# dylandreimerink/gobpfld

Measured on AMD Instinct MI355X. Metric: Mpkt/s device-resident XDP-emulator verdicts, 64B and 1500B batches, higher is better.
Workload: dtype int64

## Files before the change

### gobpfld_amd/_native.py

```python
from __future__ import annotations

import ctypes as C
from pathlib import Path

ROOT = Path(__file__).resolve().parent.parent
PRODUCT_LIB = ROOT / "gobpfld_amd" / "libxdpemu.so"
TUNING_LIB = ROOT / "gobpfld_amd" / "libxdpemu_tuning.so"


def product_path() -> Path:
    import os
    env = os.environ.get("XE_LIB")
    if not env:
        return PRODUCT_LIB
    p = Path(env).resolve()
    if p not in (PRODUCT_LIB.resolve(), TUNING_LIB.resolve()):
        raise RuntimeError(f"XE_LIB={env}: only {PRODUCT_LIB.name} or {TUNING_LIB.name} may serve as the product library")
    return p


class Desc(C.Structure):
    _fields_ = [("addr", C.c_uint64), ("len", C.c_uint32), ("options", C.c_uint32)]


# ... 45 lines not shown
class BatchStats(C.Structure):
    _fields_ = [("packets", C.c_uint64), ("steps", C.c_uint64), ("status_count", C.c_uint64 * 8),
                ("mode_used", C.c_uint32), ("conflict", C.c_uint32), ("kernel_ms", C.c_float),
                ("total_ms", C.c_float), ("engine_used", C.c_uint32), ("grid_blocks", C.c_uint32)]


def np_dtypes():
    import numpy as np
    desc = np.dtype([("addr", "<u8"), ("len", "<u4"), ("options", "<u4")])
    result = np.dtype([("status", "u1"), ("r0_kind", "u1"), ("code", "<u2"), ("pc", "<u4"), ("r0", "<i8")])
    regs = np.dtype([("val", "<i8", (10,)), ("kind", "u1", (10,)), ("region", "u1", (10,)),
                     ("map", "u1", (10,)), ("pad", "u1", (2,)), ("steps", "<u4")], align=True)
    assert desc.itemsize == 16 and result.itemsize == 16 and regs.itemsize == C.sizeof(Regs)
    return desc, result, regs


def np_trace_dtype():
    import numpy as np
    t = np.dtype([("packet", "<u4"), ("step", "<u4"), ("pc", "<i4"), ("pi", "<i4"), ("sf", "<u4"),
                  ("kind", "u1", (11,)), ("pad", "u1"), ("val", "<i8", (11,))], align=True)
    assert t.itemsize == C.sizeof(TraceRec) == 120
    return t


P = C.c_void_p
_SIGS = {
    "default_settings": (C.c_int, [P]),
    "create": (C.c_int, [P, C.POINTER(P)]),
    "destroy": (None, [P]),
    "last_error": (C.c_char_p, [P]),
    "add_raw_program": (C.c_int, [P, P, C.c_uint32, C.POINTER(C.c_int32)]),
    "set_entrypoint": (C.c_int, [P, C.c_int32]),
    "add_map": (C.c_int, [P, P, P, C.c_size_t, C.POINTER(C.c_int32)]),
    "map_lookup": (C.c_int, [P, C.c_int32, P, P]),
    "map_update": (C.c_int, [P, C.c_int32, P, P]),
    "map_delete": (C.c_int, [P, C.c_int32, P]),
    "map_update_batch": (C.c_int, [P, C.c_int32, P, P, C.c_uint64]),
    "map_count": (C.c_int, [P, C.c_int32, C.POINTER(C.c_uint64)]),
    "map_dump": (C.c_int, [P, C.c_int32, P, P, C.c_uint64, C.POINTER(C.c_uint64)]),
    "map_dump_list": (C.c_int, [P, C.c_int32, P, C.c_uint64, P, C.c_uint64, C.POINTER(C.c_uint64), C.POINTER(C.c_uint64)]),
    "map_lru_order": (C.c_int, [P, C.c_int32, P, C.c_uint64, C.POINTER(C.c_uint64)]),
    "map_push": (C.c_int, [P, C.c_int32, P]),
    "run_batch": (C.c_int, [P, P, C.c_uint64, P, C.c_uint32, P, P, P, P]),
    "run_batch_host": (C.c_int, [P, P, C.c_uint64, P, C.c_uint32, P, P, P, P]),
    "run_batch_device": (C.c_int, [P, P, C.c_uint64, P, C.c_uint32, P, P, P, P, P]),
    "run_batch_device_async": (C.c_int, [P, P, C.c_uint64, P, C.c_uint32, P, P, P, P, P]),
    "sync": (C.c_int, [P]),
    "cancel": (C.c_int, [P, C.POINTER(C.c_uint32)]),
    "trace_config": (C.c_int, [P, P, C.c_uint32, C.c_uint32]),
    "trace_read": (C.c_int, [P, C.c_uint32, P, C.c_uint32, C.POINTER(C.c_uint32)]),
    "set_helper": (C.c_int, [P, C.c_uint32, HELPER_FN, P]),
    "reset_helper": (C.c_int, [P, C.c_uint32]),
    "prepare": (C.c_int, [P]),
    "debug_set_schedule": (C.c_int, [P, C.c_uint32]),
    "debug_set_lru_epoch": (C.c_int, [P, C.c_uint64]),
    "debug_map_pool": (C.c_int, [P, C.c_int32, C.POINTER(C.c_uint64), C.POINTER(C.c_uint64)]),
    "set_kernel_cache": (C.c_int, [C.c_char_p]),
    "kernel_source": (C.c_int, [P, C.c_int, C.c_char_p, C.c_size_t, C.POINTER(C.c_size_t)]),
    "compile_kernel_source": (C.c_int, [C.c_char_p, C.c_char_p, C.c_char_p, C.c_char_p, C.c_size_t]),
    "kernel_object_name": (C.c_int, [C.c_char_p, C.c_char_p, C.c_char_p, C.c_size_t]),
    "kernel_cache_stats": (C.c_int, [C.POINTER(C.c_uint64), C.POINTER(C.c_uint64), C.POINTER(C.c_double)]),
    "map_values_bytes": (C.c_int, [P, C.c_int32, C.POINTER(C.c_uint64)]),
    "map_delta": (C.c_int, [P, C.c_int32, C.c_uint32, P, P]),
    "map_apply_delta": (C.c_int, [P, C.c_int32, C.c_uint32, P, P]),
    "map_delta_lane": (C.c_int, [P, C.c_int32, C.POINTER(C.c_uint32)]),
    "footprint": (C.c_int, [P, C.POINTER(C.c_uint64), C.c_uint32, C.POINTER(C.c_uint32)]),
    "shard_check": (C.c_int, [P, C.c_uint32, C.c_uint32, P]),
    "epoch_begin": (C.c_int, [P, P]),
    "epoch_end": (C.c_int, [P]),
    "map_state_bytes": (C.c_int, [P, C.c_int32, C.POINTER(C.c_uint64)]),
    "map_state_export": (C.c_int, [P, C.c_int32, P, P]),
    "map_state_import": (C.c_int, [P, C.c_int32, P, P]),
    "map_lookup_batch_device": (C.c_int, [P, C.c_int32, P, C.c_uint64, P, P, P]),
    "map_update_batch_device": (C.c_int, [P, C.c_int32, P, P, C.c_uint64, P]),
    "map_delete_batch_device": (C.c_int, [P, C.c_int32, P, C.c_uint64, P, P]),
    "map_lookup_batch": (C.c_int, [P, C.c_int32, P, C.c_uint64, P, P]),
    "map_update_batch_staged": (C.c_int, [P, C.c_int32, P, P, C.c_uint64]),
    "map_delete_batch": (C.c_int, [P, C.c_int32, P, C.c_uint64, P]),
    "map_scan_device": (C.c_int, [P, C.c_int32, P, P, P, C.c_uint64, C.POINTER(C.c_uint64), P]),
    "map_expire_device": (C.c_int, [P, C.c_int32, P, P, P, C.c_uint64, C.POINTER(C.c_uint64), P]),
    "map_scan": (C.c_int, [P, C.c_int32, P, P, P, C.c_uint64, C.POINTER(C.c_uint64)]),
    "map_expire": (C.c_int, [P, C.c_int32, P, P, P, C.c_uint64, C.POINTER(C.c_uint64)]),
    "debug_map_traffic": (C.c_int, [P, C.c_int32, C.POINTER(C.c_uint64), C.POINTER(C.c_uint64)]),
    "multi_create": (C.c_int, [P, C.c_uint32, C.POINTER(P)]),
    "multi_destroy": (None, [P]),
    "multi_last_error": (C.c_char_p, [P]),
    "run_batch_multi": (C.c_int, [P, P, P, P, P, P, P, P, P]),
    "version": (C.c_char_p, []),
    "device_count": (C.c_int, [C.POINTER(C.c_int)]),
    "decode_names": (C.c_int, [P, C.c_uint32, C.c_char_p, C.c_size_t]),
    "pcap_header": (C.c_int, [P, C.c_uint64, P]),
    "pcap_count": (C.c_int, [P, C.c_uint64, P, C.c_uint64, C.POINTER(C.c_uint64), C.POINTER(C.c_uint64)]),
    "pcap_fill": (C.c_int, [P, C.c_uint64, P, C.POINTER(C.c_uint64), P, C.c_uint64, C.c_uint32, C.c_uint32, P,
                            C.c_uint64, C.c_uint32, P, P, P, C.POINTER(C.c_uint32)]),
    "pcap_pack": (C.c_int, [P, C.c_uint64, P, C.POINTER(C.c_uint64), P, C.c_uint64, C.c_uint32, C.c_uint32,
                            C.c_uint32, P, P, P, C.POINTER(C.c_uint32), C.POINTER(C.c_uint64)]),
    "dispatch_scratch_bytes": (C.c_int, [C.c_uint32, C.POINTER(C.c_uint64)]),
    "dispatch_device": (C.c_int, [P, P, P, C.c_uint32, P, P, P, P, C.c_uint64, P]),
    "gather_device": (C.c_int, [P, C.c_uint64, P, P, C.c_uint32, C.c_uint32, P, C.c_uint32, P, C.c_uint64, P, P, P]),
}

HEADER_SYMBOLS = [
    "xe_default_settings", "xe_create", "xe_destroy", "xe_last_error", "xe_add_raw_program",
    "xe_set_entrypoint", "xe_add_map", "xe_map_lookup", "xe_map_update", "xe_map_delete",
    "xe_map_count", "xe_map_dump", "xe_map_dump_list", "xe_map_lru_order", "xe_map_push", "xe_map_update_batch", "xe_run_batch_device", "xe_run_batch_host",
    "xe_run_batch_device_async", "xe_sync", "xe_prepare", "xe_map_values_bytes", "xe_map_delta", "xe_map_apply_delta", "xe_map_delta_lane", "xe_footprint", "xe_version",
    "xe_device_count", "xe_shard_check", "xe_epoch_begin", "xe_epoch_end", "xe_map_state_bytes", "xe_map_state_export",
    "xe_map_state_import",
    "xe_multi_create", "xe_multi_destroy", "xe_run_batch_multi", "xe_multi_last_error", "xe_debug_set_schedule",
    "xe_debug_set_lru_epoch", "xe_debug_map_pool",
    "xe_map_lookup_batch_device", "xe_map_update_batch_device", "xe_map_delete_batch_device",
    "xe_map_lookup_batch", "xe_map_update_batch_staged", "xe_map_delete_batch", "xe_debug_map_traffic",
    "xe_map_scan_device", "xe_map_expire_device", "xe_map_scan", "xe_map_expire",
    "xe_set_kernel_cache", "xe_kernel_source", "xe_compile_kernel_source", "xe_kernel_object_name",
    "xe_kernel_cache_stats",
    "xe_cancel", "xe_trace_config", "xe_trace_read", "xe_set_helper", "xe_reset_helper",
]
IO_HEADER_SYMBOLS = ["xe_pcap_header", "xe_pcap_count", "xe_pcap_fill", "xe_pcap_pack",
                     "xe_dispatch_scratch_bytes", "xe_dispatch_device", "xe_gather_device"]
ACT_ABORTED, ACT_DROP, ACT_PASS, ACT_TX, ACT_REDIRECT, ACT_COUNT = 0, 1, 2, 3, 4, 5
XE_DISPATCH_TILE = 2048


class Lib:

    def __init__(self, path: Path | str, prefix: str = "xe_"):
        self.path = Path(path)
        if not self.path.exists():
            raise FileNotFoundError(
                f"{self.path} is missing: build it with `python -c 'import __graft_entry__ as g; g.build()'`")
        self.dll = C.CDLL(str(self.path))
        self.prefix = prefix
        for name, (res, args) in _SIGS.items():
            fn = getattr(self.dll, prefix + name, None)
            if fn is None:
                continue
            fn.restype = res
            fn.argtypes = args
            setattr(self, name, fn)

    def has(self, name: str) -> bool:
        return hasattr(self, name)


_product: Lib | None = None


def product() -> Lib:
    global _product
    if _product is None:
        try:
            import torch
        except ImportError:
            pass
        _product = Lib(product_path(), "xe_")
        kdir = ROOT / "gobpfld_amd" / "kernels"
        if kdir.is_dir() and _product.has("set_kernel_cache"):
            _product.set_kernel_cache(str(kdir).encode())
    return _product
```

### gobpfld_amd/csrc/xe_internal.h

```cpp
#pragma once
#if !defined(__HIPCC_RTC__)
#include <stdint.h>
#endif
#include "../../include/xdpemu.h"

#if defined(__HIPCC_RTC__)
#define XE_HD __host__ __device__ __forceinline__
#elif defined(__HIPCC__)
#include <hip/hip_runtime.h>
#define XE_HD __host__ __device__ __forceinline__
#else
#define XE_HD static inline
#endif

#if !defined(__HIPCC_RTC__)
#if defined(XE_TUNING)
#include <stdlib.h>
static inline const char* xe_tuning_env(const char* name) { return getenv(name); }
#else
static inline const char* xe_tuning_env(const char*) { return nullptr; }
#endif
#endif

enum XeUopClass : uint8_t {
// ... 151 lines not shown
  x ^= x >> 33;
  x *= 0xff51afd7ed558ccdull;
  x ^= x >> 33;
  x *= 0xc4ceb9fe1a85ec53ull;
  x ^= x >> 33;
  return x;
}
XE_HD uint64_t xe_kid(uint32_t m, uint64_t h) {
  return (uint64_t(m & 63u) << 58) | (xe_kid_mix(h) & ((1ull << 58) - 16ull)) | 2ull;
}
#define XE_KLOG_W 1ull
#define XE_KLOG_INS 4ull
#define XE_KLOG_FLAGS 0xDull
#define XE_KINS 2u
enum : uint32_t { XE_KS_DSET = 0, XE_KS_UNION, XE_KS_COMPRESS, XE_KS_ASSIGN, XE_KS_IOTA, XE_KS_NCHAIN, XE_KS_RESERVE,
                  XE_KS_COUNT, XE_KS_CSTART, XE_KS_CLONG, XE_KS_UNNEW, XE_KS_CFLAG, XE_KS_CLIST,
                  XE_KS_LRUID, XE_KS_FIRST, XE_KS_EKEY, XE_KS_EVICT, XE_KS_EMARK };
#define XE_KSTRIPES 32
#define XE_KS_DCOUNT 0
#define XE_KS_ERR 64
#define XE_KS_CHANGED 65
#define XE_KS_NO 66
#define XE_KS_LONG 67
#define XE_KS_NCH 68
#define XE_KS_CNEXT 69
#define XE_KS_DINS 128
#define XE_KS_CINS 192
#define XE_KS_WORDS (192 + 64 * XE_KSTRIPES)
#define XE_KEY_VALID 0x200ull
#define XE_KID_ARRAY_TAG 0xA7A7A7A700000000ull
#define XE_KID_NIL_KEY 0x6e696c6b65790001ull

struct XeKeyed {
  uint64_t* klog;
  uint32_t* kcnt;
  uint32_t dcap;
  uint32_t kw;
  uint64_t* dkid;
  uint32_t* dcomp;
  uint32_t* cstart;
  uint64_t* dkey;
  uint64_t* ikey;
  uint32_t* dcount;
  uint32_t* dins;
  uint32_t* cins;
  uint32_t* err;
  uint32_t* changed;
  uint32_t* ckey;
  uint32_t* okey;
  uint32_t* order;
  uint32_t* iota;
  uint32_t* counts;
  const uint8_t* skip;
  uint32_t n;
  uint32_t nO;
  uint32_t* dfirst;
  uint32_t* dvict;
  uint64_t* ekey;
  uint64_t* ekey2;
  uint32_t* eval;
  uint32_t* eval2;
  const uint64_t* etsnap;
  const uint32_t* vorder;
  uint32_t em, eoff, efree, ecnt0;
};

struct XeGen {
  uint8_t* base;
  uint32_t nl;
  uint32_t nobj;
  uint32_t nframes;
  uint32_t nvc;
  uint32_t nbm;
  uint32_t nkey;
  uint64_t nbytes;
  uint64_t o_ov, o_oh, o_ot, o_ofree, o_mark, o_frm, o_ctx, o_vc, o_vcinfo, o_vfree, o_bm, o_bfree, o_pres, o_key;
  uint64_t o_bytes;
  uint32_t mark_words;
  uint32_t pad;
};

#define XE_TAIL_MAPS 4
#define XE_TAIL_MAP_WORDS 2048
struct XeTailMap {
  unsigned long long* vals;
  unsigned long long* rep;
  unsigned long long* snap;
  uint64_t words;
  uint64_t stride_words;
  uint32_t nrep;
  uint32_t pad;
};
struct XeTailArgs {
  unsigned long long* aux;
  unsigned long long* host_aux;
  uint32_t* poison;
  uint32_t aux_words, nrep, rep_words, nmaps, mode, ntail;
  XeTailMap tail[XE_TAIL_MAPS];
};

struct XeListRun {
  uint32_t cnt0[64];
  uint32_t sens[64];
  uint32_t push[64];
  uint32_t senslo[64];
  unsigned long long popmask;
  unsigned long long newlist;
};
#define XE_POP_SLOTS 4u
struct XePopSlots {
  uint8_t slot[64];
};

struct XeParams {
  const XeUop* prog;
  int32_t prog_len;
  uint32_t mode;
  uint8_t* umem;
  uint64_t umem_len;
  const xe_desc* desc;
  uint32_t n;
  uint32_t nmaps;
  uint8_t bigmap[XE_H_BIG_FIELDS];
  uint8_t bigoff[XE_H_BIG_FIELDS];
  xe_result* results;
  uint32_t* verdicts;
  xe_regs* regs;
  const XeDevMap* maps;
  uint64_t max_steps;
  uint32_t ingress;
  uint32_t rxq;
  uint32_t* flags;
  unsigned long long* rep;
  uint32_t nrep;
  uint32_t rep_words;
  const XeUop* progs;
  const int32_t* prog_off;
  const int32_t* prog_lens;
  uint32_t nprogs;
  int32_t entry;
  XeGen gen;
  const uint32_t* poison;
  uint32_t seq_prefetch;
  XeKeyed K;
  uint32_t sched;
  const uint32_t* trace_pk;
  xe_trace_rec* trace;
  uint32_t* trace_cnt;
  uint32_t trace_npk, trace_max;
  XeListRun* list;
  uint32_t pop_mode;
  uint32_t pop_stride;
  uint8_t pop_slot[64];
  uint32_t* popflag;
  const uint32_t* popbase;
  uint64_t host_helpers[3];
  uint64_t nil_helpers[3];
  struct XeHostCall* hostcall;
};

#define XE_HOSTCALL_TIMEOUT_TICKS (100ull * 1000 * 1000 * 30)
struct XeHostCall {
  uint32_t req;
  uint32_t ack;
  uint32_t id;
  uint32_t packet;
  int64_t args[5];
  uint8_t kinds[5];
  uint8_t pad[3];
  int32_t err;
  int64_t r0;
  xe_helper_fn fn[192];
  void* user[192];
};

#define XE_AUX_DECISION 1

template <class Words>
XE_HD bool xe_replay_decision(uint32_t flags, Words orw, uint32_t rep_words, uint32_t nmaps, uint32_t mode) {
  bool conflict = (flags & (XE_FLAG_ORDERED | XE_FLAG_CAPACITY)) != 0;
  for (uint32_t m = 1; m <= nmaps && m < 64 && 17 + 2 * m < rep_words; m++) {
    if (orw[16 + 2 * m] & orw[16 + 2 * m + 1]) conflict = true;
    const unsigned wc = unsigned(orw[XE_REC_WIDTH0 + m / 16] >> (4 * (m % 16))) & 15u;
    if (wc & (wc - 1)) conflict = true;
  }
  return conflict && (mode == XE_MODE_AUTO || (flags & XE_FLAG_CAPACITY));
}
```

### gobpfld_amd/csrc/xe_interp.h

```cpp
#pragma once
#include "xe_internal.h"

#ifndef XE_UNIFORM
#define XE_UNIFORM 0
#endif

#if defined(__HIPCC__)
#define XE_DEV __device__ __forceinline__
#define XE_WAVE 64
typedef unsigned int xe_u4 __attribute__((ext_vector_type(4)));
XE_DEV unsigned long long xe_ballot(bool p) { return __ballot(p); }
XE_DEV int xe_readfirst(int v) { return __builtin_amdgcn_readfirstlane(v); }
XE_DEV int xe_readlane(int v, int l) { return __builtin_amdgcn_readlane(v, l); }
XE_DEV uint64_t xe_readlane64(uint64_t v, int l) {
  return uint64_t(uint32_t(__builtin_amdgcn_readlane(int(uint32_t(v)), l))) |
         (uint64_t(uint32_t(__builtin_amdgcn_readlane(int(uint32_t(v >> 32)), l))) << 32);
}
XE_DEV int xe_lane() { return __lane_id(); }
XE_DEV void xe_pin(uint64_t& x) { asm volatile("" : "+v"(x)); }
#define XE_GP(T) __attribute__((address_space(1))) T*
#define XE_LP(T) __attribute__((address_space(3))) T*
XE_DEV uint32_t xe_uni32(uint32_t v) { return XE_UNIFORM ? uint32_t(__builtin_amdgcn_readfirstlane(int(v))) : v; }
XE_DEV uint64_t xe_uni64(uint64_t v) {
  if (!XE_UNIFORM) return v;
// ... 3490 lines not shown

  for (;;) {
    int key = 0x7fffffff;
    if (status == -1) {
      if (steps >= P.max_steps) {
        status = XE_ST_BUDGET; res_pc = pc;
      } else if (XE_LANE_PI(L) < 1 || XE_LANE_PI(L) > int32_t(P.nprogs)) {
        status = XE_ST_VMERR; code = XE_E_NO_PROGRAM; res_pc = pc;
      } else if (pc < 0 || pc >= P.prog_lens[XE_LANE_PI(L)]) {
        status = XE_ST_PANIC; code = XE_P_INDEX; res_pc = pc;
      } else {
        key = P.prog_off[XE_LANE_PI(L)] + pc;
      }
    }
    const int sel = wave_min(key);
    if (sel == 0x7fffffff) break;
    if (key == sel) {
      const XeUop u = P.progs[sel];
      const int32_t plen = P.prog_lens[XE_LANE_PI(L)];
      steps++;
      int32_t tgt;
      int e = exec_uop(L, P, u, pc, tgt);
      res_pc = pc;
#if XE_TRACE
      if (tslot >= 0 && (e == 0 || e == XE_EV_EXIT)) {
        if (tdone < P.trace_max) trace_put(L, P, tslot, i, tdone, pc);
        tdone++;
      }
#endif
      if (e == 0) {
        if (int64_t(plen) <= int64_t(tgt) + 1) {
          status = XE_ST_VMERR; code = XE_E_BAD_PC;
        } else {
          pc = tgt + 1;
        }
      } else {
        status_from_error(e, status, code);
      }
    }
  }
#if XE_TRACE
  if (tslot >= 0) P.trace_cnt[tslot] = uint32_t(tdone < P.trace_max ? tdone : P.trace_max);
#endif
  if (finish) lane_finish(L, P, i, valid, status, code, res_pc, steps);
}

XE_DEV void run_packet(XeLane& L, const XeParams& P, uint32_t i, bool valid) {
  lane_reset(L, P, i, valid);
  run_staged(L, P, i, valid);
}

XE_DEV void flush_wave_state(XeLane& L, const XeParams& P) {
  acc_flush(L);
  unsigned long long steps = L.acc_steps;
  unsigned int aw = L.awidth;
#if defined(__HIPCC__)
  for (int o = 32; o > 0; o >>= 1) aw |= __shfl_xor(aw, o);
#endif
  if (xe_lane() == 0 && aw) xe_atomic_or64(&L.rep[XE_REC_WIDTH0], aw);
#if XE_KEYED
  if (xe_lane() == 0 && L.kany) xe_atomic_or32(P.flags, XE_FLAG_KEYED);
#endif
#if defined(__HIPCC__)
  for (int o = 32; o > 0; o >>= 1) steps += __shfl_xor(steps, o);
#endif
  if (xe_lane() == 0) {
    if (steps) xe_atomic_add64(&L.rep[0], steps);
#pragma unroll
    for (int st = 0; st < 8; st++)
      if (L.acc_status[st]) xe_atomic_add64(&L.rep[1 + st], L.acc_status[st]);
  }
#pragma unroll
  for (int k = 0; k < XE_FP_MAPS; k++) {
    unsigned long long r = L.fpr[k], a = L.fpa[k];
#if defined(__HIPCC__)
    for (int o = 32; o > 0; o >>= 1) { r |= __shfl_xor(r, o); a |= __shfl_xor(a, o); }
#endif
    if (xe_lane() == 0) {
      if (r) xe_atomic_or64(&L.rep[16 + (k + 1) * 2], r);
      if (a) xe_atomic_or64(&L.rep[16 + (k + 1) * 2 + 1], a);
    }
  }
}
```

### gobpfld_amd/csrc/xe_jit.cpp

```cpp
#ifndef XE_HOSTSIM
#include <hip/hip_runtime_api.h>
#include <hip/hiprtc.h>
#endif

#include <algorithm>
#include <array>
#include <atomic>
#include <chrono>
#include <climits>
#include <cstdint>
#include <cstdio>
#include <cstdlib>
#include <cstring>
#include <fstream>
#include <future>
#include <map>
#include <memory>
#include <set>
#include <mutex>
#include <sstream>
#include <string>
#include <vector>

#include <unistd.h>
// ... 880 lines not shown
          o << "    if (uop_jmp(L, " << U << ")) ";
          emit_goto_bb(o, size_t(k), u.tgt, n, cyclic ? "steps" : "(steps + st)");
          o << "\n";
          break;
        case U_MOVI: case U_MOVR:
          o << "    " << handler_call(u, cms[size_t(k)]) << "\n";
          break;
        case U_ALU: case U_NEG: case U_END: case U_LDIMM64: case U_LDX: case U_ST: case U_STX: case U_ATOMIC:
        case U_HELPER: case U_CALLX: {
          auto ks = kshadow.find(k);
          if (!dead.count(k))
            o << "    " << (ks != kshadow.end() ? key_call(p, u, cms[size_t(k)], ks->second, captured) : handler_call(u, cms[size_t(k)]))
              << "\n" << on_err;
          const std::string cap = key_capture(u, k, captured, alias_caps);
          if (!cap.empty()) o << "    " << cap << "\n";
          break;
        }
        default: o << "    e = exec_uop(L, P, " << U << ", " << k << ", tgt);\n" << on_err; break;
      }
    }
    if (!terminated) {
      if (e + 1 >= n) o << "    status = XE_ST_VMERR; code = XE_E_BAD_PC; res_pc = " << e << "; bb = XE_BB_DONE;\n";
      else o << "    bb = " << e + 1 << ";\n";
    }
    o << "  } while (0);\n";
    if (ifconv) o << "#endif\n";
    b = rules ? rci->second.end : (chain.empty() ? e : chain.back()) + 1;
  }
  if (cyclic) o << "  }\n";
  else o << "  steps += st;\n";
}

bool fields_model(const std::vector<XeUop>& p, bool cyclic) { return !cyclic && 7 + max_stores_on_path(p) <= 64; }

void emit_kernel(std::ostringstream& o) {
  o << R"(#ifndef XE_MIN_WAVES_PER_EU
#define XE_MIN_WAVES_PER_EU 4  // 4 waves per SIMD: VGPRs <= 128 (16 waves per CU)
#endif
extern "C" __global__ void __launch_bounds__(256, XE_MIN_WAVES_PER_EU) xe_jit_kernel(XeParams P) {
  __shared__ __attribute__((aligned(16))) uint8_t hdr_lds[XE_HDR_LDS_BYTES];
  __shared__ XePend pend_lds[4];
  extern __shared__ __attribute__((aligned(16))) uint8_t xe_dyn_lds[];  // (nmaps + 1) map descriptors
  XeLane L;
#if !XE_GEN
  XeMem M;
  L.mem = &M;
#endif
  L.hdrbuf = (XE_LP(uint8_t))(hdr_lds + (threadIdx.x >> 6) * XE_HDR_WAVE_BYTES);
  const int lane = xe_lane();
#if XE_COMMITTER
  __shared__ XeRing xe_rings[3];  // waves 0..2 -> the committer (wave 3), parallel mode
  if (threadIdx.x < 3) { xe_rings[threadIdx.x].head = 0; xe_rings[threadIdx.x].tail = 0; xe_rings[threadIdx.x].done = 0; }
#endif
  stage_maps(L, P, (XE_LP(XeDevMap))xe_dyn_lds);
  wave_state_init(L, P, (blockIdx.x * blockDim.x + threadIdx.x) >> 6, &pend_lds[threadIdx.x >> 6]);
#if XE_UNIFORM
  {  // the scalar replay: the sequential driver alone
#else
  if (P.mode == XE_MODE_SEQUENTIAL) {
#endif
    if (blockIdx.x != 0 || threadIdx.x >= 64) return;
    seq_packets(L, P, [&](uint32_t i, bool valid) __attribute__((always_inline)) {
      int status = XE_ST_OK, code = 0; int32_t res_pc = 0; uint64_t steps = 0;
      if (valid) xe_jit_body(L, P, status, code, res_pc, steps);
      lane_finish(L, P, i, valid, status, code, res_pc, steps);
    }, [&](bool valid) __attribute__((always_inline)) {  // the runahead: results dropped
      int status = XE_ST_OK, code = 0; int32_t res_pc = 0; uint64_t steps = 0;
      if (valid) xe_jit_body(L, P, status, code, res_pc, steps);
    });
#if XE_UNIFORM
  }
#else
#if XE_KEYED
  } else if (P.mode == XE_MODE_CHAIN) {
    chain_packets(L, P, blockIdx.x * blockDim.x + threadIdx.x, gridDim.x * blockDim.x, [&](uint32_t i, bool valid) __attribute__((always_inline)) {
      int status = XE_ST_OK, code = 0; int32_t res_pc = 0; uint64_t steps = 0;
      if (valid) xe_jit_body(L, P, status, code, res_pc, steps);
      lane_finish(L, P, i, valid, status, code, res_pc, steps);
    });
#endif
  } else {
    uint32_t wave = (blockIdx.x * blockDim.x + threadIdx.x) >> 6;
    uint32_t nwaves = (gridDim.x * blockDim.x) >> 6;
#if XE_COMMITTER
    if (P.mode == XE_MODE_PARALLEL && blockDim.x == 256) {
      const uint32_t wib = threadIdx.x >> 6;
      if (wib == 3) { committer_loop(L, P, (XE_LP(XeRing))xe_rings, 3); return; }
      L.ring = (XE_LP(XeRing))&xe_rings[wib];
      wave = blockIdx.x * 3 + wib;
      nwaves = gridDim.x * 3;
    }
#endif
    parallel_packets(L, P, wave, nwaves, [&](uint32_t i, bool valid) __attribute__((always_inline)) {
      int status = XE_ST_OK, code = 0; int32_t res_pc = 0; uint64_t steps = 0;
      if (valid) xe_jit_body(L, P, status, code, res_pc, steps);
      lane_finish(L, P, i, valid, status, code, res_pc, steps);
    });
#if XE_COMMITTER
    if (L.ring) ring_done(L.ring);
#endif
  }
#endif  // !XE_UNIFORM
  flush_wave_state(L, P);
}
)";
}

enum { XE_JV_PLAIN = 0, XE_JV_KEYED = 1, XE_JV_LEAN = 2, XE_JV_SEQ = 3 };
void emit_variant(std::ostringstream& o, int variant) {
  o << "#define XE_KEYED " << (variant == XE_JV_KEYED ? 1 : 0) << "\n";
  if (variant == XE_JV_LEAN) o << "#define XE_RECORDS 0\n";
  if (variant == XE_JV_SEQ) o << "#define XE_UNIFORM 1\n#define XE_MIN_WAVES_PER_EU 1\n#define xe_jit_kernel xe_jit_seq_kernel\n";
}

bool has_lru(const std::vector<XeDevMap>& geom);

std::string generate(const std::vector<XeUop>& p, bool cyclic, const std::vector<XeDevMap>& geom, int variant = XE_JV_PLAIN) {
  std::ostringstream o;
  const int64_t n = int64_t(p.size());
  unsigned mapkinds = 0;
  for (size_t i = 1; i < geom.size(); i++)
    mapkinds |= geom[i].kind == XE_DM_ARRAY ? 1u : (geom[i].kind == XE_DM_HASH || geom[i].kind == XE_DM_LRU) ? 2u : 0u;
  const bool lru = has_lru(geom);
  o << "#define XE_REGS_FIELDS 1\n";
  o << "#define XE_HAS_ARRAY " << ((mapkinds & 1u) ? 1 : 0) << "\n";
  o << "#define XE_HAS_HASH " << ((mapkinds & 2u) ? 1 : 0) << "\n";
  o << "#define XE_FP_MAPS " << std::max<size_t>(1, std::min<size_t>(4, geom.size() - 1)) << "\n";
  o << "#define XE_HAS_ORDERED " << (lru ? 1 : 0) << "\n";
  if (lru) o << "#define XE_FIELDS_LRU 1\n";
  if (lru && variant == XE_JV_KEYED) o << "#define XE_MIN_WAVES_PER_EU 2\n";
  emit_variant(o, variant);
  if (variant != XE_JV_KEYED && fields_model(p, cyclic)) o << "#ifndef XE_SEQ_PEEK\n#define XE_SEQ_PEEK 1\n#endif\n";
  o << "#ifndef XE_IFCONV\n#define XE_IFCONV 1  // if-converted jump blocks (emit_body_blocks; -D overrides: A/B)\n#endif\n";
  int add_sites = 0;
  for (const XeUop& u : p)
    add_sites += (u.cls == U_ATOMIC || (u.cls == U_STX && (u.fl & UF_LIFT))) && uop_size(u) == 8 ? 1 : 0;
  o << "#define XE_PAIR_ADDS " << (add_sites >= 2 ? 1 : 0) << "\n";
  if (fields_model(p, cyclic)) emit_mem_fields(o, 7 + max_stores_on_path(p));
  emit_geom(o, geom);
  std::vector<RegMasks> cms = class_masks(p);
  emit_window(o, p, cyclic, cms, geom);
  o << "#include \"xe_interp.h\"\n";
  o << "__device__ __forceinline__ void xe_jit_geom(unsigned m, XeDevMap& M) { XE_JIT_GEOM_BODY }\n\n";
  int cond = 0;
  for (const XeUop& u : p) cond += u.cls == U_JMP;
  const bool blocks = n > 0 && cond > 32;
  const std::map<int64_t, RuleChain> rchains = blocks ? rule_chains(p, cyclic) : std::map<int64_t, RuleChain>{};
  {
    int id = 0;
    for (const auto& rc : rchains) emit_rule_tables(o, rc.second, id++);
  }
  o << "XE_DEV void xe_jit_body(XeLane& L, const XeParams& P, int& status, int& code, int32_t& res_pc, uint64_t& steps) {\n";
  o << "  int e = 0; int32_t tgt = 0; (void)e; (void)tgt;\n";
  std::map<int64_t, int64_t> store_off;
  AliasCaps alias_caps;
  const KeyShadows kshadow = key_shadows(p, cms, geom, &store_off, &alias_caps);
  const std::set<int64_t> dead = fields_model(p, cyclic) ? dead_frame_stores(p, cms, kshadow, store_off) : std::set<int64_t>{};
  std::set<int64_t> modified;
  for (const auto& a : alias_caps)
    for (const auto& sr : a.second) modified.insert(sr.first);
  std::set<int64_t> captured;
  for (const auto& site : kshadow)
    for (const KeyPart& q : site.second)
      if (p[size_t(q.store)].cls == U_STX || modified.count(q.store)) captured.insert(q.store);
  for (int64_t s : captured) o << "  int64_t ksv" << s << " = 0;\n";
  if (n == 0) o << "  status = XE_ST_PANIC; code = XE_P_INDEX; res_pc = 0; return;\n";
  if (blocks) {
    o << "#define XE_BB_DONE 0x7fffffff\n";
    emit_body_blocks(o, p, cyclic, cms, kshadow, captured, dead, alias_caps, rchains);
  } else {
  for (int64_t k = 0; k < n; k++) {
    const XeUop& u = p[k];
    o << "L" << k << ":\n";
    if (cyclic) o << "  if (steps >= P.max_steps) { status = XE_ST_BUDGET; res_pc = " << k << "; return; }\n";
    o << "  steps++;\n";
    const std::string U = uop_literal(u);
    const std::string on_err = "  if (e) { res_pc = " + std::to_string(k) + "; status_from_error(e, status, code); return; }\n";
    switch (u.cls) {
      case U_EXIT:
        o << "  status = XE_ST_OK; res_pc = " << k << "; return;\n";
        continue;
      case U_NOP:
        break;
// ... 799 lines not shown
```

### gobpfld_amd/csrc/xe_kernel.hip

```cpp
#include "xe_interp.h"
#include "xe_kernels.h"

#include <hipcub/device/device_radix_sort.hpp>
#include <hipcub/device/device_scan.hpp>

extern "C" __global__ void __launch_bounds__(256) xe_interp_kernel(XeParams P) {
  __shared__ __attribute__((aligned(16))) uint8_t hdr_lds[XE_HDR_LDS_BYTES];
  __shared__ XePend pend_lds[4];
  extern __shared__ __attribute__((aligned(16))) uint8_t xe_dyn_lds[];
  XeLane L;
  L.hdrbuf = (XE_LP(uint8_t))(hdr_lds + (threadIdx.x >> 6) * XE_HDR_WAVE_BYTES);
  const int lane = xe_lane();
  stage_maps(L, P, (XE_LP(XeDevMap))xe_dyn_lds);
  wave_state_init(L, P, (blockIdx.x * blockDim.x + threadIdx.x) >> 6, &pend_lds[threadIdx.x >> 6]);
  if (P.mode == XE_MODE_SEQUENTIAL) {
    if (blockIdx.x != 0 || threadIdx.x >= 64) return;
    seq_packets(L, P, [&](uint32_t i, bool valid) { run_staged(L, P, i, valid); }, [](bool) {});
  } else if (P.mode == XE_MODE_CHAIN) {
    chain_packets(L, P, blockIdx.x * blockDim.x + threadIdx.x, gridDim.x * blockDim.x,
                  [&](uint32_t i, bool valid) { run_staged(L, P, i, valid); });
  } else {
    const uint32_t wave = (blockIdx.x * blockDim.x + threadIdx.x) >> 6;
    const uint32_t nwaves = (gridDim.x * blockDim.x) >> 6;
    parallel_packets(L, P, wave, nwaves, [&](uint32_t i, bool valid) { run_staged(L, P, i, valid); });
  }
  flush_wave_state(L, P);
}

template <class T, class C>
__global__ void xe_delta_kernel(const T* cur, const T* snap, C* out, uint64_t n) {
  for (uint64_t i = blockIdx.x * uint64_t(blockDim.x) + threadIdx.x; i < n; i += uint64_t(gridDim.x) * blockDim.x)
    out[i] = C(T(cur[i] - snap[i]));
}
template <class T, class C>
__global__ void xe_apply_delta_kernel(T* cur, const T* snap, const C* delta, uint64_t n) {
  for (uint64_t i = blockIdx.x * uint64_t(blockDim.x) + threadIdx.x; i < n; i += uint64_t(gridDim.x) * blockDim.x)
    cur[i] = T(snap[i] + T(delta[i]));
}
template <class C>
__global__ void xe_sum_kernel(C* acc, const C* in, uint64_t n) {
  for (uint64_t i = blockIdx.x * uint64_t(blockDim.x) + threadIdx.x; i < n; i += uint64_t(gridDim.x) * blockDim.x)
    acc[i] = C(acc[i] + in[i]);
}

extern "C" __global__ void xe_rep_fold_kernel(unsigned long long* __restrict__ vals, unsigned long long* __restrict__ rep,
                                              uint64_t stride_words, uint32_t nrep, uint64_t nwords,
                                              const unsigned long long* __restrict__ recs, uint32_t rwords, uint32_t vsize,
                                              uint32_t cap, const unsigned long long* __restrict__ lim) {
  if (lim) nwords = nwords < (lim[3] * vsize + 7) / 8 ? nwords : (lim[3] * vsize + 7) / 8;
  for (uint64_t i = blockIdx.x * uint64_t(blockDim.x) + threadIdx.x; i < nwords; i += uint64_t(gridDim.x) * blockDim.x) {
    if (recs) {
      const uint64_t s0 = 8 * i / vsize, s1 = (8 * i + 7) / vsize;
      const bool live = (s0 <= cap && recs[s0 * rwords] != 0) || (s1 != s0 && s1 <= cap && recs[s1 * rwords] != 0);
      if (!live) continue;
    }
    unsigned long long v[16];
#pragma unroll
    for (uint32_t k = 0; k < 16; k++) v[k] = k < nrep ? rep[k * stride_words + i] : 0ull;
    unsigned long long s = 0;
#pragma unroll
    for (uint32_t k = 0; k < 16; k++) {
      s += v[k];
      if (v[k]) rep[k * stride_words + i] = 0;
    }
    if (s) vals[i] += s;
  }
}

#define XE_PRO_SEGS 8
struct XeProlog {
  const unsigned long long* src[XE_PRO_SEGS];
  unsigned long long* dst[XE_PRO_SEGS];
  uint64_t words[XE_PRO_SEGS];
  uint32_t nseg;
  unsigned long long* zero;
  uint64_t zero_words;
};
extern "C" __global__ void xe_prologue_kernel(XeProlog A) {
  const uint64_t tid = blockIdx.x * uint64_t(blockDim.x) + threadIdx.x, nth = uint64_t(gridDim.x) * blockDim.x;
  for (uint64_t i = tid; i < A.zero_words; i += nth) A.zero[i] = 0;
  for (uint32_t g = 0; g < A.nseg; g++)
    for (uint64_t i = tid; i < A.words[g]; i += nth) A.dst[g][i] = A.src[g][i];
}

extern "C" __global__ void __launch_bounds__(1024) xe_tail_kernel(XeTailArgs A) {
  __shared__ unsigned long long orw[257];
  const uint32_t t = threadIdx.x, nt = blockDim.x;
  for (uint32_t w = t; w <= 256; w += nt) orw[w] = 0;
  const bool poisoned = *(volatile uint32_t*)A.poison != 0;
  __syncthreads();
  for (uint32_t i = t; i < A.aux_words; i += nt) {
    const unsigned long long v = A.aux[i];
    if (v) A.aux[i] = 0;
    A.host_aux[i] = v;
    if (i == 0) orw[256] = v;
    else if (i >= 16 && v) atomicOr(&orw[(i - 16) % A.rep_words], v);
  }
  __syncthreads();
  if (t == 0) {
    const bool replay = !poisoned && xe_replay_decision(uint32_t(orw[256]), orw, A.rep_words, A.nmaps, A.mode);
    A.host_aux[XE_AUX_DECISION] = replay ? 1ull : 0ull;
    if (replay) *A.poison = 1u;
  }
  if (poisoned) return;
  for (uint32_t f = 0; f < A.ntail; f++) {
    const XeTailMap& T = A.tail[f];
    for (uint64_t i = t; i < T.words; i += nt) {
      unsigned long long r[16];
#pragma unroll
      for (uint32_t k = 0; k < 16; k++) r[k] = k < T.nrep ? T.rep[k * T.stride_words + i] : 0ull;
      unsigned long long s = 0;
#pragma unroll
      for (uint32_t k = 0; k < 16; k++) {
        s += r[k];
        if (r[k]) T.rep[k * T.stride_words + i] = 0;
      }
      const unsigned long long v = T.vals[i] + s;
      if (s) T.vals[i] = v;
      T.snap[i] = v;
    }
  }
}
extern "C" int xe_launch_tail(const XeTailArgs* A, hipStream_t s) {
  if (A->rep_words > 256) return -1;
  hipLaunchKernelGGL(xe_tail_kernel, dim3(1), dim3(1024), 0, s, *A);
  return hipGetLastError() == hipSuccess ? 0 : -1;
}

__global__ void xe_desc_split_kernel(const xe_desc* d, uint32_t n, uint64_t umem_len, unsigned long long* key,
                                     uint32_t* len) {
  for (uint64_t i = blockIdx.x * uint64_t(blockDim.x) + threadIdx.x; i < n; i += uint64_t(gridDim.x) * blockDim.x) {
    const uint64_t a = d[i].addr;
    uint32_t l = d[i].len;
    if (a > umem_len || uint64_t(l) > umem_len - a) l = 0;
    key[i] = l ? a : ~0ull;
    len[i] = l;
  }
}
__global__ void xe_desc_overlap_kernel(const unsigned long long* key, const uint32_t* len, uint32_t n, uint32_t* flag) {
  for (uint64_t i = blockIdx.x * uint64_t(blockDim.x) + threadIdx.x; i + 1 < n; i += uint64_t(gridDim.x) * blockDim.x)
    if (len[i] && len[i + 1] && key[i] + len[i] > key[i + 1]) *flag = 1u;
}
extern "C" int xe_launch_desc_overlap(const void* desc, uint32_t n, uint64_t umem_len, void* scratch, size_t* scratch_bytes,
                                      uint32_t* flag, hipStream_t s) {
  const size_t arr = ((size_t(n) * 8 + 255) & ~size_t(255)) * 2 + ((size_t(n) * 4 + 255) & ~size_t(255)) * 2;
  size_t tmp = 0;
  if (hipcub::DeviceRadixSort::SortPairs(nullptr, tmp, (unsigned long long*)nullptr, (unsigned long long*)nullptr,
                                         (uint32_t*)nullptr, (uint32_t*)nullptr, int(n), 0, 64, s) != hipSuccess)
    return -1;
  if (!scratch) {
    *scratch_bytes = arr + tmp;
    return 0;
  }
  if (*scratch_bytes < arr + tmp) return -1;
  uint8_t* p = (uint8_t*)scratch;
  auto take = [&](size_t bytes) { uint8_t* q = p; p += (bytes + 255) & ~size_t(255); return q; };
  unsigned long long* k0 = (unsigned long long*)take(size_t(n) * 8);
  unsigned long long* k1 = (unsigned long long*)take(size_t(n) * 8);
  uint32_t* l0 = (uint32_t*)take(size_t(n) * 4);
  uint32_t* l1 = (uint32_t*)take(size_t(n) * 4);
  const uint32_t blocks = n / 256 + 1 < 4096 ? n / 256 + 1 : 4096;
  if (hipMemsetAsync(flag, 0, 4, s) != hipSuccess) return -1;
  hipLaunchKernelGGL(xe_desc_split_kernel, dim3(blocks), dim3(256), 0, s, (const xe_desc*)desc, n, umem_len, k0, l0);
  if (hipcub::DeviceRadixSort::SortPairs(p, tmp, k0, k1, l0, l1, int(n), 0, 64, s) != hipSuccess) return -1;
  hipLaunchKernelGGL(xe_desc_overlap_kernel, dim3(blocks), dim3(256), 0, s, k1, l1, n, flag);
  return hipGetLastError() == hipSuccess ? 0 : -1;
}

extern "C" __global__ void xe_keyed_kernel(XeKeyed K, const XeDevMap* maps, uint8_t* skip, uint32_t step, uint32_t items) {
  for (uint64_t i = blockIdx.x * uint64_t(blockDim.x) + threadIdx.x; i < items; i += uint64_t(gridDim.x) * blockDim.x)
    keyed_step(K, maps, skip, step, uint32_t(i));
}
extern "C" __global__ void xe_keyed_count_kernel(XeKeyed K) {
  __shared__ unsigned int hist[64], ins[64];
  if (threadIdx.x < 64) hist[threadIdx.x] = ins[threadIdx.x] = 0;
  __syncthreads();
  for (uint64_t x = blockIdx.x * uint64_t(blockDim.x) + threadIdx.x; x < K.dcap; x += uint64_t(gridDim.x) * blockDim.x) {
    const uint64_t kid = K.dkid[x];
    if (kid) {
      atomicAdd(&hist[kid >> 58], 1u);
      if (K.dkey[x * K.kw] & XE_KEY_VALID) atomicAdd(&ins[kid >> 58], 1u);
    }
  }
  __syncthreads();
  if (threadIdx.x < 64 && hist[threadIdx.x]) atomicAdd(K.dcount + threadIdx.x, hist[threadIdx.x]);
  if (threadIdx.x < 64 && ins[threadIdx.x]) atomicAdd(K.dins + threadIdx.x, ins[threadIdx.x]);
}
extern "C" int xe_launch_keyed(const XeKeyed* K, const XeDevMap* maps, uint8_t* skip, uint32_t step, uint32_t items,
                               hipStream_t s) {
  if (!items) return 0;
  if (step == XE_KS_COUNT) {
    hipLaunchKernelGGL(xe_keyed_count_kernel, dim3(1024), dim3(256), 0, s, *K);
    return hipGetLastError() == hipSuccess ? 0 : -1;
  }
  const uint32_t blocks = items / 256 + 1 < 8192 ? items / 256 + 1 : 8192;
  hipLaunchKernelGGL(xe_keyed_kernel, dim3(blocks), dim3(256), 0, s, *K, maps, skip, step, items);
  return hipGetLastError() == hipSuccess ? 0 : -1;
}
extern "C" int xe_launch_keyed_sort(const XeKeyed* K, uint32_t n, uint32_t end_bit, void* scratch, size_t* bytes, hipStream_t s) {
  size_t tmp = 0;
  if (hipcub::DeviceRadixSort::SortPairs(nullptr, tmp, (const uint32_t*)nullptr, (uint32_t*)nullptr, (const uint32_t*)nullptr,
                                         (uint32_t*)nullptr, int(n), 0, int(end_bit), s) != hipSuccess)
    return -1;
  if (!scratch) {
    *bytes = tmp;
    return 0;
  }
  if (*bytes < tmp) return -1;
  return hipcub::DeviceRadixSort::SortPairs(scratch, tmp, K->ckey, K->okey, K->iota, K->order, int(n), 0, int(end_bit), s) ==
                 hipSuccess
             ? 0
// ... 263 lines not shown
```

### gobpfld_amd/csrc/xe_kernels.h

```cpp
#ifndef XE_KERNELS_H_
#define XE_KERNELS_H_

#include "xe_internal.h"

#ifndef XE_HOSTSIM
#include <hip/hip_runtime_api.h>
#endif

extern "C" {

int xe_jit_may_write_entries(const XeUop* prog, size_t n);
size_t xe_jit_source_for(const XeUop* const* progs, const uint32_t* lens, uint32_t nprogs, int32_t entry,
                         const XeDevMap* maps, uint32_t nmaps, int variant, char* buf, size_t buflen);

#ifndef XE_HOSTSIM
void* xe_jit_get(const XeUop* const* progs, const uint32_t* lens, uint32_t nprogs, int32_t entry, int device,
                 const XeDevMap* maps, uint32_t nmaps, bool* cyclic, bool* general, const char** err, int variant,
                 uint64_t* maxpath);
int xe_jit_launch(void* fn, const XeParams* P, uint32_t blocks, uint32_t threads, hipStream_t s);
int xe_jit_occupancy(void* fn, uint32_t nmaps);

int xe_launch_interp(const XeParams* P, uint32_t blocks, uint32_t threads, hipStream_t s);
int xe_interp_occupancy(uint32_t nmaps);
int xe_launch_delta(const void* cur, const void* snap, void* out, uint64_t bytes, uint32_t lane, hipStream_t s);
int xe_launch_apply_delta(void* cur, const void* snap, const void* delta, uint64_t bytes, uint32_t lane, hipStream_t s);
int xe_launch_delta_sum(void* acc, const void* in, uint64_t bytes, uint32_t lane, hipStream_t s);
int xe_launch_rep_fold(void* vals, void* rep, uint64_t stride_words, uint32_t nrep, uint64_t nwords, const void* recs,
                       uint32_t rwords, uint32_t vsize, uint32_t cap, const void* lim, hipStream_t s);
int xe_launch_prologue(const void* const* src, void* const* dst, const uint64_t* words, uint32_t nseg, void* zero,
                       uint64_t zero_words, hipStream_t s);
int xe_launch_tail(const XeTailArgs* A, hipStream_t s);
int xe_launch_desc_overlap(const void* desc, uint32_t n, uint64_t umem_len, void* scratch, size_t* scratch_bytes,
                           uint32_t* flag, hipStream_t s);
int xe_launch_keyed(const XeKeyed* K, const XeDevMap* maps, uint8_t* skip, uint32_t step, uint32_t items, hipStream_t s);
int xe_launch_keyed_sort(const XeKeyed* K, uint32_t n, uint32_t end_bit, void* scratch, size_t* bytes, hipStream_t s);
int xe_launch_keyed_esort(const XeKeyed* K, void* scratch, size_t* bytes, hipStream_t s);
int xe_launch_keyed_scan(const XeKeyed* K, uint32_t n, void* scratch, size_t* bytes, hipStream_t s);
int xe_launch_append(const XeAppendArgs* A, uint32_t end_bit, void* scratch, size_t* bytes, hipStream_t s);
int xe_launch_pop(const uint32_t* src, uint32_t* dst, uint32_t n, uint32_t mode, uint32_t arg, XePopSlots sl, uint32_t* flag,
                  hipStream_t s);
int xe_launch_lru_relink(uint64_t* tag, uint32_t pool, uint32_t cnt, uint32_t* link, uint64_t* hdr, void* scratch,
                         size_t* bytes, int renumber, hipStream_t s);
int xe_launch_lru_tag_fold(uint64_t* tag, uint64_t* rep, uint32_t pool, uint32_t r, const uint64_t* hdr, hipStream_t s);
int xe_launch_lru_log(const uint64_t* tag, uint32_t pool, const uint32_t* order, const uint64_t* hdr, uint64_t* log,
                      hipStream_t s);
#endif

int xe_internal_vm_device(const xe_vm* vm);
void* xe_internal_vm_stream(xe_vm* vm);
int xe_internal_nmaps(const xe_vm* vm);
int xe_internal_may_write_packet(const xe_vm* vm);
int xe_internal_delta_sum(xe_vm* vm, void* acc, const void* in, uint64_t bytes, uint32_t lane);
int xe_internal_alloc(xe_vm* vm, void** p, uint64_t bytes);
void xe_internal_free(xe_vm* vm, void* p);
int xe_internal_copy(xe_vm* vm, void* dst, const void* src, uint64_t bytes);

}

#endif
```

### gobpfld_amd/csrc/xe_runtime.cpp

```cpp
#include "xe_internal.h"
#include "xe_mapops.h"

#include <algorithm>
#include <map>
#include <chrono>
#include <cstdio>
#include <cstdlib>
#include <cstring>
#include <string>
#include <array>
#include <thread>
#include <vector>

#ifdef XE_HOSTSIM
#define XE_SEQ_PEEK 1
#include "xe_interp.h"
typedef void* xe_stream_t;
#else
#include <hip/hip_runtime_api.h>
typedef hipStream_t xe_stream_t;
#endif
#include "xe_kernels.h"

#define XE_FRAME_SIZE 256

namespace {

#ifdef XE_HOSTSIM
#ifdef XE_HOSTSIM_POISON
int dev_alloc(void** p, size_t n) {
  n = n ? n : 8;
  *p = malloc(n);
  if (*p) memset(*p, 0xA5, n);
  return *p ? 0 : -1;
}
#else
int dev_alloc(void** p, size_t n) { *p = calloc(n ? n : 8, 1); return *p ? 0 : -1; }
#endif
void dev_free(void* p) { free(p); }
int h2d(void* d, const void* h, size_t n, xe_stream_t) { memcpy(d, h, n); return 0; }
int d2h(void* h, const void* d, size_t n, xe_stream_t) { memcpy(h, d, n); return 0; }
int d2d(void* d, const void* s, size_t n, xe_stream_t) { memmove(d, s, n); return 0; }
int dmemset(void* d, int v, size_t n, xe_stream_t) { memset(d, v, n); return 0; }
int dsync(xe_stream_t) { return 0; }
int launch_interp(const XeParams* P, uint32_t, uint32_t, xe_stream_t) {
  XeLane L;
#ifdef XE_HOSTSIM_POISON
  memset(static_cast<void*>(&L), 0, sizeof L);
#endif
  static thread_local uint8_t hdrbuf[XE_HDR_WAVE_BYTES + 16];
  L.hdrbuf = hdrbuf;
  XePend pend;
  stage_maps(L, *P, nullptr);
  wave_state_init(L, *P, 0, &pend);
  if (P->mode == XE_MODE_PARALLEL || P->mode == XE_MODE_SPEC) {
    parallel_packets(L, *P, 0, 1, [&](uint32_t i, bool valid) { run_staged(L, *P, i, valid); });
  } else if (P->mode == XE_MODE_CHAIN) {
    chain_packets(L, *P, 0, 1, [&](uint32_t i, bool valid) { run_staged(L, *P, i, valid); });
  } else {
    seq_packets(L, *P, [&](uint32_t i, bool valid) { run_staged(L, *P, i, valid); },
                [&](bool valid) { run_staged(L, *P, 0, valid, false); });
  }
  flush_wave_state(L, *P);
  return 0;
}
int launch_jit(void*, const XeParams* P, uint32_t b, uint32_t t, xe_stream_t s) { return launch_interp(P, b, t, s); }
template <class T, class C = T>
void lanes_sub(const void* a, const void* b, void* o, uint64_t n) {
  for (uint64_t i = 0; i < n; i++) ((C*)o)[i] = C(T(((const T*)a)[i] - ((const T*)b)[i]));
}
template <class T, class C = T>
void lanes_add(const void* snap, const void* d, void* o, uint64_t n) {
  for (uint64_t i = 0; i < n; i++) ((T*)o)[i] = T(((const T*)snap)[i] + T(((const C*)d)[i]));
}
template <class C>
void lanes_acc(void* acc, const void* in, uint64_t n) {
  for (uint64_t i = 0; i < n; i++) ((C*)acc)[i] = C(((C*)acc)[i] + ((const C*)in)[i]);
}
int launch_delta(const void* cur, const void* snap, void* out, uint64_t bytes, uint32_t lane, xe_stream_t) {
  switch (lane) {
    case 1: lanes_sub<uint8_t>(cur, snap, out, bytes); break;
    case 2: lanes_sub<uint16_t, uint32_t>(cur, snap, out, bytes / 2); break;
    case 4: lanes_sub<uint32_t>(cur, snap, out, bytes / 4); break;
    default: lanes_sub<uint64_t>(cur, snap, out, bytes / 8); break;
  }
  return 0;
}
int launch_apply_delta(void* cur, const void* snap, const void* delta, uint64_t bytes, uint32_t lane, xe_stream_t) {
  switch (lane) {
    case 1: lanes_add<uint8_t>(snap, delta, cur, bytes); break;
    case 2: lanes_add<uint16_t, uint32_t>(snap, delta, cur, bytes / 2); break;
    case 4: lanes_add<uint32_t>(snap, delta, cur, bytes / 4); break;
    default: lanes_add<uint64_t>(snap, delta, cur, bytes / 8); break;
  }
  return 0;
}
int launch_delta_sum(void* acc, const void* in, uint64_t bytes, uint32_t lane, xe_stream_t) {
  switch (lane) {
    case 1: lanes_acc<uint8_t>(acc, in, bytes); break;
    case 2: case 4: lanes_acc<uint32_t>(acc, in, bytes / lane); break;
    default: lanes_acc<uint64_t>(acc, in, bytes / 8); break;
  }
  return 0;
}
int launch_prologue(const void* const* src, void* const* dst, const uint64_t* words, uint32_t nseg, void* zero, uint64_t zw,
                    xe_stream_t) {
  if (zw) memset(zero, 0, zw * 8);
  for (uint32_t g = 0; g < nseg; g++) memcpy(dst[g], src[g], words[g] * 8);
  return 0;
}
int launch_rep_fold(void* vals, void* rep, uint64_t sw, uint32_t nrep, uint64_t nw, const void* recs, uint32_t rwords,
                    uint32_t vsize, uint32_t cap, const void* lim, xe_stream_t) {
  uint64_t* v = (uint64_t*)vals;
  uint64_t* r = (uint64_t*)rep;
  const uint64_t* rc = (const uint64_t*)recs;
  if (lim) nw = std::min<uint64_t>(nw, (((const uint64_t*)lim)[3] * vsize + 7) / 8);
  for (uint64_t i = 0; i < nw; i++) {
    if (rc) {
      const uint64_t s0 = 8 * i / vsize, s1 = (8 * i + 7) / vsize;
      if (!((s0 <= cap && rc[s0 * rwords]) || (s1 != s0 && s1 <= cap && rc[s1 * rwords]))) continue;
    }
    for (uint32_t k = 0; k < nrep; k++) { v[i] += r[k * sw + i]; r[k * sw + i] = 0; }
  }
  return 0;
}
int launch_tail(const XeTailArgs* A, xe_stream_t) {
  unsigned long long orw[257] = {};
  const bool poisoned = *A->poison != 0;
  for (uint32_t i = 0; i < A->aux_words; i++) {
    const unsigned long long v = A->aux[i];
    A->aux[i] = 0;
    A->host_aux[i] = v;
    if (i == 0) orw[256] = v;
    else if (i >= 16) orw[(i - 16) % A->rep_words] |= v;
  }
  const bool replay = !poisoned && xe_replay_decision(uint32_t(orw[256]), orw, A->rep_words, A->nmaps, A->mode);
  A->host_aux[XE_AUX_DECISION] = replay ? 1ull : 0ull;
  if (replay) *A->poison = 1u;
  if (poisoned) return 0;
  for (uint32_t f = 0; f < A->ntail; f++) {
    const XeTailMap& T = A->tail[f];
    for (uint64_t i = 0; i < T.words; i++) {
      unsigned long long s = 0;
      for (uint32_t k = 0; k < T.nrep; k++) { s += T.rep[k * T.stride_words + i]; T.rep[k * T.stride_words + i] = 0; }
      T.vals[i] += s;
      T.snap[i] = T.vals[i];
    }
  }
  return 0;
}
int host_alloc(void** p, size_t n) { *p = calloc(n ? n : 8, 1); return *p ? 0 : -1; }
void host_free(void* p) { free(p); }
int host_device_ptr(void** d, void* h) { *d = h; return 0; }
int host_alloc_coherent(void** p, size_t n) { return host_alloc(p, n); }
int serve_hostcalls(XeHostCall*, xe_stream_t) { return 0; }
int poison_async(uint32_t* d, xe_stream_t*) { *d = 2; return 0; }
void stream_destroy(xe_stream_t) {}
int launch_desc_overlap(const void* desc, uint32_t n, uint64_t umem_len, void* scratch, size_t* bytes, uint32_t* flag,
                        xe_stream_t) {
  if (!scratch) { *bytes = 8; return 0; }
  std::vector<std::pair<uint64_t, uint32_t>> r;
  const xe_desc* d = (const xe_desc*)desc;
  for (uint32_t i = 0; i < n; i++) {
    uint32_t l = d[i].len;
    if (d[i].addr > umem_len || uint64_t(l) > umem_len - d[i].addr) l = 0;
    if (l) r.emplace_back(d[i].addr, l);
  }
  std::sort(r.begin(), r.end());
  *flag = 0;
  for (size_t i = 0; i + 1 < r.size(); i++)
    if (r[i].first + r[i].second > r[i + 1].first) *flag = 1;
  return 0;
}
int launch_keyed(const XeKeyed* K, const XeDevMap* maps, uint8_t* skip, uint32_t step, uint32_t items, xe_stream_t) {
  if (step == XE_KS_COUNT) {
    for (uint32_t x = 0; x < K->dcap; x++)
      if (K->dkid[x]) {
        K->dcount[K->dkid[x] >> 58]++;
        if (K->dkey[uint64_t(x) * K->kw] & XE_KEY_VALID) K->dins[K->dkid[x] >> 58]++;
      }
    return 0;
  }
  for (uint32_t i = 0; i < items; i++) keyed_step(*K, maps, skip, step, i);
  if (step == XE_KS_DSET && getenv("XE_HOSTSIM_DCYCLE")) {
    uint32_t a = K->dcap, b = K->dcap;
    for (uint32_t x = 0; x < K->dcap && b == K->dcap; x++)
      if (K->dkid[x]) (a == K->dcap ? a : b) = x;
    if (b != K->dcap) { K->dcomp[a] = b; K->dcomp[b] = a; }
  }
  return 0;
}
int launch_keyed_sort(const XeKeyed* K, uint32_t n, uint32_t, void* scratch, size_t* bytes, xe_stream_t) {
  if (!scratch) { *bytes = 8; return 0; }
  std::vector<std::pair<uint32_t, uint32_t>> v(n);
  for (uint32_t i = 0; i < n; i++) v[i] = {K->ckey[i], K->iota[i]};
  std::stable_sort(v.begin(), v.end(), [](const auto& a, const auto& b) { return a.first < b.first; });
  for (uint32_t i = 0; i < n; i++) { K->okey[i] = v[i].first; K->order[i] = v[i].second; }
  return 0;
}
int launch_keyed_esort(const XeKeyed* K, void* scratch, size_t* bytes, xe_stream_t) {
  if (!scratch) { *bytes = 8; return 0; }
  std::vector<std::pair<uint64_t, uint32_t>> v(K->dcap);
  for (uint32_t i = 0; i < K->dcap; i++) v[i] = {K->ekey[i], K->eval[i]};
  std::stable_sort(v.begin(), v.end(), [](const auto& a, const auto& b) { return a.first < b.first; });
  for (uint32_t i = 0; i < K->dcap; i++) { K->ekey2[i] = v[i].first; K->eval2[i] = v[i].second; }
  return 0;
}
int launch_lru_relink(uint64_t* tag, uint32_t pool, uint32_t cnt, uint32_t* link, uint64_t* hdr, void* scratch,
                      size_t* bytes, int renumber, xe_stream_t) {
  if (!scratch) { *bytes = size_t(pool) * 16 + 256; return 0; }
  std::vector<uint32_t> v(pool);
  for (uint32_t i = 0; i < pool; i++) v[i] = i;
  std::stable_sort(v.begin(), v.end(), [&](uint32_t a, uint32_t b) { return tag[a] > tag[b]; });
  uint32_t* vout = (uint32_t*)((uint8_t*)scratch + size_t(pool) * 8) + pool;
  for (uint32_t i = 0; i < pool; i++) vout[i] = v[i];
  if (renumber == 2) return 0;
  for (uint32_t i = 0; i < cnt && i < pool; i++) {
    if (renumber) tag[v[i]] = cnt - i;
    link[4 * uint64_t(v[i])] = i ? v[i - 1] : XE_NONE;
    link[4 * uint64_t(v[i]) + 1] = i + 1 < cnt ? v[i + 1] : XE_NONE;
  }
  hdr[0] = cnt ? v[0] : XE_NONE;
  hdr[1] = cnt ? v[cnt - 1] : XE_NONE;
  return 0;
}
int launch_lru_tag_fold(uint64_t* tag, uint64_t* rep, uint32_t pool, uint32_t r, const uint64_t* hdr, xe_stream_t) {
  for (uint64_t v = 0; v < std::min<uint64_t>(pool, hdr[3]); v++)
    for (uint32_t k = 0; k < r; k++) {
      uint64_t& x = rep[k * uint64_t(pool) + v];
      if (x > tag[v]) tag[v] = x;
// ... 36 lines not shown
  std::stable_sort(v.begin(), v.end(), [](const auto& a, const auto& b) { return a.first < b.first; });
  std::vector<uint64_t> rec;
  if (A->perf) rec.assign(A->rec + 2 * A->base, A->rec + 2 * (A->base + A->k));
  for (uint32_t j = 0; j < A->k; j++) {
    const uint32_t id = v[j].second;
    if (A->perf) {
      A->rec[2 * (A->base + j)] = rec[2 * (id - A->base)];
      A->rec[2 * (A->base + j) + 1] = rec[2 * (id - A->base) + 1];
    } else {
      A->link[A->stack ? A->cnt0 + j : (A->head + A->cnt0 + j) % A->list_cap] = id;
    }
  }
  return 0;
}
struct Timer {
  std::chrono::steady_clock::time_point t;
  void rec(xe_stream_t) { t = std::chrono::steady_clock::now(); }
  static float ms(const Timer& a, const Timer& b) { return std::chrono::duration<float, std::milli>(b.t - a.t).count(); }
  int wait() { return 0; }
  void init() {}
  void fini() {}
};
int set_device(int) { return 0; }
int blocks_per_cu(void*, uint32_t) { return 1; }
int cu_count(int) { return 1; }
#else
int dev_alloc(void** p, size_t n) { return hipMalloc(p, n ? n : 8) == hipSuccess ? 0 : -1; }
void dev_free(void* p) { if (p) (void)hipFree(p); }
int h2d(void* d, const void* h, size_t n, xe_stream_t s) { return hipMemcpyAsync(d, h, n, hipMemcpyHostToDevice, s) == hipSuccess ? 0 : -1; }
int d2h(void* h, const void* d, size_t n, xe_stream_t s) { return hipMemcpyAsync(h, d, n, hipMemcpyDeviceToHost, s) == hipSuccess ? 0 : -1; }
int d2d(void* d, const void* src, size_t n, xe_stream_t s) { return hipMemcpyAsync(d, src, n, hipMemcpyDeviceToDevice, s) == hipSuccess ? 0 : -1; }
int dmemset(void* d, int v, size_t n, xe_stream_t s) { return hipMemsetAsync(d, v, n, s) == hipSuccess ? 0 : -1; }
int dsync(xe_stream_t s) { return hipStreamSynchronize(s) == hipSuccess ? 0 : -1; }
int launch_interp(const XeParams* P, uint32_t b, uint32_t t, xe_stream_t s) { return xe_launch_interp(P, b, t, s); }
int launch_jit(void* fn, const XeParams* P, uint32_t b, uint32_t t, xe_stream_t s) { return xe_jit_launch(fn, P, b, t, s); }
int launch_delta(const void* c, const void* sn, void* o, uint64_t b, uint32_t lane, xe_stream_t s) {
  return xe_launch_delta(c, sn, o, b, lane, s);
}
int launch_apply_delta(void* c, const void* sn, const void* d, uint64_t b, uint32_t lane, xe_stream_t s) {
  return xe_launch_apply_delta(c, sn, d, b, lane, s);
}
int launch_rep_fold(void* v, void* r, uint64_t sw, uint32_t nrep, uint64_t nw, const void* recs, uint32_t rwords, uint32_t vsize,
                    uint32_t cap, const void* lim, xe_stream_t s) {
  return xe_launch_rep_fold(v, r, sw, nrep, nw, recs, rwords, vsize, cap, lim, s);
}
int launch_delta_sum(void* acc, const void* in, uint64_t bytes, uint32_t lane, xe_stream_t s) {
  return xe_launch_delta_sum(acc, in, bytes, lane, s);
}
int launch_prologue(const void* const* src, void* const* dst, const uint64_t* words, uint32_t nseg, void* zero, uint64_t zw,
                    xe_stream_t s) {
  return xe_launch_prologue(src, dst, words, nseg, zero, zw, s);
}
int host_alloc(void** p, size_t n) { return hipHostMalloc(p, n ? n : 8, hipHostMallocDefault) == hipSuccess ? 0 : -1; }
int launch_keyed(const XeKeyed* K, const XeDevMap* maps, uint8_t* skip, uint32_t step, uint32_t items, xe_stream_t s) {
  return xe_launch_keyed(K, maps, skip, step, items, s);
}
int launch_keyed_esort(const XeKeyed* K, void* scratch, size_t* bytes, xe_stream_t s) {
  return xe_launch_keyed_esort(K, scratch, bytes, s);
}
int launch_keyed_sort(const XeKeyed* K, uint32_t n, uint32_t end_bit, void* scratch, size_t* bytes, xe_stream_t s) {
  return xe_launch_keyed_sort(K, n, end_bit, scratch, bytes, s);
}
int launch_append(const XeAppendArgs* A, uint32_t end_bit, void* scratch, size_t* bytes, xe_stream_t s) {
  return xe_launch_append(A, end_bit, scratch, bytes, s);
}
int launch_pop(const uint32_t* src, uint32_t* dst, uint32_t n, uint32_t mode, uint32_t arg, XePopSlots sl, uint32_t* flag,
               xe_stream_t s) {
  return xe_launch_pop(src, dst, n, mode, arg, sl, flag, s);
}
int launch_keyed_scan(const XeKeyed* K, uint32_t n, void* scratch, size_t* bytes, xe_stream_t s) {
  return xe_launch_keyed_scan(K, n, scratch, bytes, s);
}
void host_free(void* p) { if (p) (void)hipHostFree(p); }
int launch_lru_relink(uint64_t* tag, uint32_t pool, uint32_t cnt, uint32_t* link, uint64_t* hdr, void* scratch,
                      size_t* bytes, int renumber, xe_stream_t s) {
  return xe_launch_lru_relink(tag, pool, cnt, link, hdr, scratch, bytes, renumber, s);
}
int launch_lru_tag_fold(uint64_t* tag, uint64_t* rep, uint32_t pool, uint32_t r, const uint64_t* hdr, xe_stream_t s) {
  return xe_launch_lru_tag_fold(tag, rep, pool, r, hdr, s);
}
int launch_lru_log(const uint64_t* tag, uint32_t pool, const uint32_t* order, const uint64_t* hdr, uint64_t* log, xe_stream_t s) {
  return xe_launch_lru_log(tag, pool, order, hdr, log, s);
}
int launch_tail(const XeTailArgs* A, xe_stream_t s) { return xe_launch_tail(A, s); }
int launch_desc_overlap(const void* desc, uint32_t n, uint64_t umem_len, void* scratch, size_t* bytes, uint32_t* flag,
                        xe_stream_t s) {
  return xe_launch_desc_overlap(desc, n, umem_len, scratch, bytes, flag, s);
}
int host_device_ptr(void** d, void* h) { return hipHostGetDevicePointer(d, h, 0) == hipSuccess ? 0 : -1; }
int host_alloc_coherent(void** p, size_t n) {
  if (hipHostMalloc(p, n ? n : 8, hipHostMallocCoherent | hipHostMallocMapped) != hipSuccess) return -1;
  memset(*p, 0, n);
  return 0;
}
int serve_hostcalls(XeHostCall* H, xe_stream_t s) {
  for (;;) {
    const uint32_t req = __atomic_load_n(&H->req, __ATOMIC_ACQUIRE);
    if (req != __atomic_load_n(&H->ack, __ATOMIC_RELAXED)) {
      const uint32_t id = H->id;
      int64_t a[5];
      uint8_t k[5];
      for (int r = 0; r < 5; r++) { a[r] = H->args[r]; k[r] = H->kinds[r]; }
      int64_t r0 = 0;
      const int err = (id < 192 && H->fn[id]) ? H->fn[id](H->user[id], H->packet, a, k, &r0) : 1;
      H->r0 = r0;
      H->err = err ? 1 : 0;
      __atomic_store_n(&H->ack, req, __ATOMIC_RELEASE);
      continue;
    }
    const hipError_t q = hipStreamQuery(s);
    if (q == hipSuccess) return 0;
    if (q != hipErrorNotReady) return -1;
    std::this_thread::sleep_for(std::chrono::microseconds(20));
  }
}
int poison_async(uint32_t* d, xe_stream_t* cs) {
  if (!*cs && hipStreamCreateWithFlags(cs, hipStreamNonBlocking) != hipSuccess) return -1;
  if (hipMemsetD32Async(reinterpret_cast<hipDeviceptr_t>(d), 2u, 1, *cs) != hipSuccess) return -1;
  return hipStreamSynchronize(*cs) == hipSuccess ? 0 : -1;
}
void stream_destroy(xe_stream_t s) { if (s) (void)hipStreamDestroy(s); }
struct Timer {
  hipEvent_t e = nullptr;
  void init() { if (!e) (void)hipEventCreate(&e); }
  void fini() { if (e) (void)hipEventDestroy(e); e = nullptr; }
  void rec(xe_stream_t s) { init(); (void)hipEventRecord(e, s); }
  int wait() { return hipEventSynchronize(e) == hipSuccess ? 0 : -1; }
  static float ms(const Timer& a, const Timer& b) { float m = 0; (void)hipEventElapsedTime(&m, a.e, b.e); return m; }
};
int set_device(int d) { return hipSetDevice(d) == hipSuccess ? 0 : -1; }
int blocks_per_cu(void* jit, uint32_t nmaps) { return jit ? xe_jit_occupancy(jit, nmaps) : xe_interp_occupancy(nmaps); }
int cu_count(int dev) {
  int n = 0;
  if (hipDeviceGetAttribute(&n, hipDeviceAttributeMultiprocessorCount, dev) != hipSuccess) return 0;
  return n;
}
#endif
int launch_emulator(void* fn, const XeParams* P, uint32_t blocks, uint32_t threads, xe_stream_t s) {
  return fn ? launch_jit(fn, P, blocks, threads, s) : launch_interp(P, blocks, threads, s);
}

int size_log2(uint8_t sizecode) {
  switch (sizecode) { case 0x00: return 2; case 0x08: return 1; case 0x10: return 0; default: return 3; }
}

XeUop fail_uop(int code) { XeUop u{}; u.cls = U_FAIL; u.imm = code; return u; }

int translate(const uint64_t* raw, uint32_t n, std::vector<XeUop>& out, std::string& err) {
  out.assign(n, XeUop{});
  for (uint32_t i = 0; i < n; i++) {
    const uint64_t r = raw[i];
    const uint8_t op = uint8_t(r);
    const uint8_t dst = uint8_t(r >> 8) & 0x0f, src = uint8_t(r >> 12) & 0x0f;
    const int16_t off = int16_t(uint16_t(r >> 16));
    const int32_t imm = int32_t(uint32_t(r >> 32));
    const uint8_t cls = op & 7;
    XeUop u{};
    bool decoded = true, translated = true;

    if (op == 0x18) {
      if (i + 1 >= n) { err = "decode: load double word imm op code found but not enough instructions"; return XE_ERR_DECODE; }
      if (dst > 9) u = fail_uop(XE_E_BAD_REG);
      else { u.cls = U_LDIMM64; u.dst = dst; u.src = src; u.imm = imm; u.x = uint32_t(raw[i + 1] >> 32); }
      out[i] = u;
      out[i + 1] = XeUop{}; out[i + 1].cls = U_NOP;
      i++;
      continue;
    }
    switch (op) {
      case 0x20: case 0x28: case 0x30: case 0x38:
      case 0x40: case 0x48: case 0x50: case 0x58:
        u = fail_uop(XE_E_NOT_IMPL);
        break;
      case 0x61: case 0x69: case 0x71: case 0x79:
        if (src > 10) { u = fail_uop(XE_E_BAD_REG); break; }
        u.cls = U_LDX; u.src = src; u.tgt = off; u.fl = uint8_t(size_log2(op ^ 0x61) << 4);
        if (dst > 9) u.fl |= UF_BADDST; else u.dst = dst;
        break;
      case 0x62: case 0x6a: case 0x72: case 0x7a:
        if (dst > 10) { u = fail_uop(XE_E_BAD_REG); break; }
        u.cls = U_ST; u.dst = dst; u.imm = imm; u.tgt = off; u.fl = uint8_t(size_log2(op ^ 0x62) << 4);
        break;
      case 0x63: case 0x6b: case 0x73: case 0x7b:
        if (src > 9 || dst > 10) { u = fail_uop(XE_E_BAD_REG); break; }
        u.cls = U_STX; u.dst = dst; u.src = src; u.tgt = off; u.fl = uint8_t(size_log2(op ^ 0x63) << 4);
        break;
      case 0xc3: case 0xcb: case 0xd3: case 0xdb: {
        bool known = imm == 0x00 || imm == 0x01 || imm == 0x10 || imm == 0x11 || imm == 0x50 || imm == 0x51 ||
                     imm == 0x40 || imm == 0x41 || imm == 0xa0 || imm == 0xa1 || imm == 0xe1 || imm == 0xf1;
        if (!known) { decoded = false; break; }
        if (imm != 0x00 && imm != 0x01) { translated = false; break; }
        if (dst > 10) { u = fail_uop(XE_E_BAD_REG); break; }
        u.cls = U_ATOMIC; u.dst = dst; u.tgt = off; u.fl = uint8_t(size_log2(op ^ 0xc3) << 4);
        if (src > 9) u.fl |= UF_BADSRC; else u.src = src;
        break;
      }
      default:
        if (cls == 0x04 || cls == 0x07) {
          const uint8_t aop = op & 0xf0;
          const bool x = op & 0x08, wide = cls == 0x07;
          if (aop == 0x80) {
            if (x) { decoded = false; break; }
            if (dst > 9) { u = fail_uop(XE_E_BAD_REG); break; }
            u.cls = U_NEG; u.dst = dst; u.fl = wide ? UF_WIDE : 0;
          } else if (aop == 0xd0) {
            if (wide || !(imm == 16 || imm == 32 || imm == 64)) { decoded = false; break; }
            if (dst > 9) { u = fail_uop(XE_E_BAD_REG); break; }
            u.cls = U_END; u.dst = dst; u.imm = imm; u.x = x ? 8 : 0;
          } else if (aop == 0xe0 || aop == 0xf0) {
            decoded = false;
          } else if (aop == 0xb0) {
            if (!x) {
              if (dst > 9) { u = fail_uop(XE_E_ASSIGN_REG); break; }
              u.cls = U_MOVI; u.dst = dst; u.imm = imm;
            } else {
              if (src > 10) { u = fail_uop(XE_E_BAD_REG); break; }
              if (dst > 9) { u = fail_uop(XE_E_ASSIGN_REG); break; }
              u.cls = U_MOVR; u.dst = dst; u.src = src;
            }
            u.fl = wide ? UF_WIDE : 0;
          } else {
// ... 257 lines not shown
    state[i] = 0;
    count--;
    uint32_t j = i;
    for (;;) {
      j = (j + 1) & mask;
      if (!(state[j] & XE_SLOT_FULL)) break;
      uint32_t k = uint32_t(xe_hash_words(key_at(j), kwords, def.key_size)) & mask;
      bool move = (j > i) ? (k <= i || k > j) : (k <= i && k > j);
      if (move) {
        memcpy(key_at(i), key_at(j), kwords * 8);
        memcpy(vals.data() + uint64_t(i) * def.value_size, vals.data() + uint64_t(j) * def.value_size, def.value_size);
        state[i] = state[j];
        state[j] = 0;
        i = j;
      }
    }
  }
};

}

struct xe_vm {
  xe_settings settings{};
  std::vector<std::vector<XeUop>> programs{std::vector<XeUop>()};
  int32_t entry = 0;
  std::vector<HostMap> maps{HostMap()};
  std::string last_error;
  xe_stream_t stream = nullptr;
  XeUop* d_progs = nullptr;
  int32_t* d_prog_off = nullptr;
  size_t d_progs_n = 0;
  size_t d_prog_len = 0;
  std::vector<int32_t> prog_off;
  uint8_t* d_arena_par = nullptr;
  uint64_t arena_par_bytes = 0;
  uint8_t* d_arena_seq = nullptr;
  uint64_t arena_seq_bytes = 0;
  uint32_t seq_scale = 1;
  uint64_t* d_ksnap = nullptr;
  size_t d_ksnap_bytes = 0;
  XeDevMap* d_maps = nullptr;
  size_t d_maps_n = 0;
  std::vector<XeDevMap> dm_uploaded;
  unsigned long long* d_aux = nullptr;
  int cus = -1, occ_interp = -1, occ_jit = -1;
  void* occ_jit_fn = nullptr;
  uint32_t occ_nmaps = 0;
  uint32_t last_grid = 0;
  void* d_umem = nullptr; size_t d_umem_cap = 0;
  void* d_usnap = nullptr; size_t d_usnap_cap = 0;
  void* d_ovl = nullptr; size_t d_ovl_cap = 0;
  void* d_desc = nullptr; size_t d_desc_cap = 0;
  void* d_res = nullptr; size_t d_res_cap = 0;
  void* d_ver = nullptr; size_t d_ver_cap = 0;
  void* d_regs = nullptr; size_t d_regs_cap = 0;
  std::vector<unsigned long long> last_fp;
  uint32_t last_flags = 0;
  uint32_t last_mode = 0;
  int32_t jit_idx = -1;
  size_t jit_nmaps = 0;
  size_t jit_nprogs = 0;
  void* jit_fn = nullptr;
  bool jit_cyclic = false;
  uint64_t jit_maxpath = 0;
  bool jit_general = false;
  std::string jit_error;
  struct Variant {
    bool ready = false;
    void* fn = nullptr;
  };
  std::array<Variant, 4> jit_variants{};
  Timer t0, t1, t2;
  uint64_t ord_slack = 4096, ord_slack_bytes = 1 << 20;
  struct Batch {
    void* d_umem = nullptr; uint64_t umem_len = 0; const void* d_desc = nullptr; uint32_t n = 0;
    void* d_results = nullptr; void* d_verdicts = nullptr; void* d_regs = nullptr;
    xe_stream_t s = nullptr; xe_batch_stats* stats = nullptr;
  };
  struct Slot {
    unsigned long long* d_aux = nullptr;
    unsigned long long* h_aux = nullptr;
    unsigned long long* h_aux_dev = nullptr;
    Timer t0, t1, done;
    Batch b;
    size_t aux_used = 0;
    uint32_t nmaps = 0, grid = 0, engine = 0;
    uint32_t snap = 0;
  };
  std::array<Slot, kAsyncDepth> slots;
  std::vector<uint32_t> pending;
  uint32_t next_slot = 0;
  uint32_t next_snap = 0;
  uint32_t* d_poison = nullptr;
  xe_stream_t cancel_stream = nullptr;
  int32_t staged_slot = -1;
  bool draining = false;
  bool delta_base = true;
  bool epoch_open = false;
  std::vector<unsigned long long> epoch_fp;
  uint32_t epoch_flags = 0;
  bool epoch_seq = false;
  XeKeyed kd{};
  uint8_t* d_skip = nullptr;
  uint32_t* d_ksmall = nullptr;
  uint64_t keyed_n = 0;
  uint32_t keyed_dcap = 0, keyed_kw = 0;
  uint32_t keyed_dnext = 0;
  void* d_ksort = nullptr;
  size_t d_ksort_cap = 0;
  bool keyed_hint = false;
  bool keyed_hint_set = false;
  uint32_t keyed_backoff = 0;
  XeListRun* d_listrun = nullptr;
  uint32_t* d_popflag = nullptr;
  uint32_t* d_popbase = nullptr;
  uint32_t* d_popused = nullptr;
  size_t pop_n = 0;
  uint32_t seg_depth = 0;
  std::vector<uint32_t> trace_pk;
  uint32_t trace_max = 0;
  uint32_t* d_trace_pk = nullptr;
  xe_trace_rec* d_trace = nullptr;
  uint32_t* d_trace_cnt = nullptr;
  uint64_t host_helpers[3] = {0, 0, 0};
  uint64_t nil_helpers[3] = {0, 0, 0};
  XeHostCall* h_hostcall = nullptr;
  XeHostCall* d_hostcall = nullptr;
  uint32_t ord_backoff = 0;
  void* d_app = nullptr; size_t d_app_cap = 0;
  void* d_app_sort = nullptr; size_t d_app_sort_cap = 0;
  void* d_relink = nullptr; size_t d_relink_cap = 0;
  uint64_t lru_epoch = 0;
  uint32_t sched = 0;
  void* d_mo = nullptr; size_t d_mo_cap = 0;
  void* d_mo_keys = nullptr; size_t d_mo_keys_cap = 0;
  void* d_mo_vals = nullptr; size_t d_mo_vals_cap = 0;
  void* d_mo_found = nullptr; size_t d_mo_found_cap = 0;
  void* d_ms = nullptr; size_t d_ms_cap = 0;
};
static void keyed_free(xe_vm* vm) {
  XeKeyed& K = vm->kd;
  dev_free(K.klog); dev_free(K.kcnt); dev_free(K.dkey); dev_free(K.dkid); dev_free(K.dcomp); dev_free(K.ikey);
  dev_free(K.cstart);
  dev_free(K.dfirst); dev_free(K.dvict); dev_free(K.ekey); dev_free(K.ekey2); dev_free(K.eval); dev_free(K.eval2);
  dev_free(K.ckey); dev_free(K.okey); dev_free(K.order); dev_free(K.iota);
  dev_free(vm->d_skip); dev_free(vm->d_ksmall); dev_free(vm->d_ksort);
  K = XeKeyed{};
  vm->d_skip = nullptr; vm->d_ksmall = nullptr; vm->d_ksort = nullptr;
  vm->d_ksort_cap = 0;
  vm->keyed_n = 0;
  vm->keyed_dcap = vm->keyed_kw = 0;
}
static int keyed_alloc(xe_vm* vm, uint32_t n, uint32_t dcap) {
  uint32_t kw = 1;
  for (size_t i = 1; i < vm->maps.size(); i++)
    if (vm->maps[i].dkind == XE_DM_HASH || vm->maps[i].dkind == XE_DM_LRU) kw = std::max(kw, 1 + vm->maps[i].kwords);
  XeKeyed& K = vm->kd;
  if (vm->keyed_n < n || !vm->d_ksmall || vm->keyed_kw < kw) {
    dev_free(K.klog); dev_free(K.kcnt); dev_free(K.ckey); dev_free(K.okey); dev_free(K.order); dev_free(K.iota);
    dev_free(K.ikey); dev_free(vm->d_skip); dev_free(vm->d_ksmall);
    K.klog = K.ikey = nullptr; K.kcnt = K.ckey = K.okey = K.order = K.iota = nullptr;
    vm->d_skip = nullptr; vm->d_ksmall = nullptr;
    vm->keyed_n = 0;
    vm->keyed_dcap = 0;
    const uint64_t np = std::max<uint64_t>(n, 64);
    if (dev_alloc((void**)&K.klog, np * XE_KLOG * 8) || dev_alloc((void**)&K.kcnt, np * 4) ||
        dev_alloc((void**)&K.ikey, np * XE_KINS * kw * 8) ||
        dev_alloc((void**)&K.ckey, np * 4) || dev_alloc((void**)&K.okey, np * 4) || dev_alloc((void**)&K.order, np * 4) ||
        dev_alloc((void**)&K.iota, np * 4) || dev_alloc((void**)&vm->d_skip, np) ||
        dev_alloc((void**)&vm->d_ksmall, XE_KS_WORDS * 4)) {
      keyed_free(vm);
      return -1;
    }
    vm->keyed_n = np;
    K.dcount = vm->d_ksmall + XE_KS_DCOUNT;
    K.dins = vm->d_ksmall + XE_KS_DINS;
    K.err = vm->d_ksmall + XE_KS_ERR;
    K.changed = vm->d_ksmall + XE_KS_CHANGED;
    K.counts = vm->d_ksmall + XE_KS_NO;
    K.cins = vm->d_ksmall + XE_KS_CINS;
  }
  if (vm->keyed_dcap < dcap || vm->keyed_kw < kw) {
    dev_free(K.dkey); dev_free(K.dkid); dev_free(K.dcomp); dev_free(K.cstart);
    dev_free(K.dfirst); dev_free(K.dvict); dev_free(K.ekey); dev_free(K.ekey2); dev_free(K.eval); dev_free(K.eval2);
    K.dkey = nullptr; K.dkid = nullptr; K.dcomp = K.cstart = nullptr;
    K.dfirst = K.dvict = K.eval = K.eval2 = nullptr; K.ekey = K.ekey2 = nullptr;
    vm->keyed_dcap = 0;
    if (dev_alloc((void**)&K.dkey, uint64_t(dcap) * kw * 8) || dev_alloc((void**)&K.dkid, uint64_t(dcap) * 8) ||
        dev_alloc((void**)&K.dcomp, uint64_t(dcap) * 4) || dev_alloc((void**)&K.cstart, uint64_t(dcap) * 4) ||
        dev_alloc((void**)&K.dfirst, uint64_t(dcap) * 4) || dev_alloc((void**)&K.dvict, uint64_t(dcap) * 4) ||
        dev_alloc((void**)&K.ekey, uint64_t(dcap) * 8) || dev_alloc((void**)&K.ekey2, uint64_t(dcap) * 8) ||
        dev_alloc((void**)&K.eval, uint64_t(dcap) * 4) || dev_alloc((void**)&K.eval2, uint64_t(dcap) * 4)) {
      keyed_free(vm);
      return -1;
    }
    vm->keyed_dcap = dcap;
    vm->keyed_kw = kw;
  }
  K.kw = vm->keyed_kw;
  K.dcap = dcap;
  return 0;
}

namespace {

constexpr uint32_t kRep = 64;
constexpr uint32_t kRepWords = 16 + 2 * 64;
constexpr size_t kAuxWords = 16 + size_t(kRep) * kRepWords;
constexpr uint64_t kTailMapBytes = 8 * XE_TAIL_MAP_WORDS;

int fail(xe_vm* vm, int rc, const std::string& msg) {
  if (vm) vm->last_error = msg;
  return rc;
}

int ensure_buf(void** p, size_t* cap, size_t need) {
  if (*cap >= need && *p) return 0;
  dev_free(*p);
  *p = nullptr;
  size_t c = std::max<size_t>(need, 256);
  if (dev_alloc(p, c)) { *cap = 0; return -1; }
  *cap = c;
  return 0;
}

bool nrep_bounded(uint32_t want, uint64_t live, uint64_t vals_alloc, bool hash) {
  return uint64_t(want) * (hash ? live : vals_alloc) <= (160ull << 20) && uint64_t(want) * vals_alloc <= (1ull << 30);
}

uint32_t choose_nrep(uint64_t live, uint64_t vals_alloc, bool hash) {
  if (const char* e = xe_tuning_env("XE_NREP")) return uint32_t(std::min(16, std::max(1, atoi(e))));
  uint32_t want = live <= (2ull << 20) ? 16u : live <= (8ull << 20) ? 4u : 1u;
  while (want > 1 && !nrep_bounded(want, live, vals_alloc, hash)) want >>= 1;
  return want;
}

int fold_map(HostMap& m, xe_stream_t s) {
  const bool hash = m.dkind == XE_DM_HASH && m.def.value_size > 0;
  const bool lru = m.dkind == XE_DM_LRU;
  const uint64_t words = lru ? (uint64_t(m.pool_cap) * m.def.value_size + 7) / 8 : m.vals_alloc / 8;
  return launch_rep_fold(m.d_vals, m.d_rep, m.rep_stride / 8, m.nrep, words, hash ? m.d_keys : nullptr,
                         hash ? xe_hash_rwords(m.kwords) : 0, hash || lru ? m.def.value_size : 8, m.cap,
                         lru ? (const void*)m.d_hdr : nullptr, s);
}

int map_alloc_device(HostMap& m) {
  if (m.ordered()) return 0;
  if (dev_alloc((void**)&m.d_vals, m.vals_alloc)) return -1;
  if (dev_alloc((void**)&m.d_snap, m.vals_alloc)) return -1;
  m.nrep = 1;
  m.nrep_fixed = false;
  m.rep_stride = (m.vals_alloc + 255) & ~uint64_t(255);
  if (const char* e = xe_tuning_env("XE_REP_SKEW")) m.rep_stride = ((m.vals_alloc + 4095) & ~uint64_t(4095)) + uint64_t(atoll(e));
  if (m.dkind == XE_DM_HASH) {
    if (dev_alloc((void**)&m.d_keys, size_t(m.cap + 1) * xe_hash_rwords(m.kwords) * 8)) return -1;
    if (dev_alloc((void**)&m.d_count, 8)) return -1;
  }
  return 0;
}

void map_free_device(HostMap& m) {
  for (auto& p : m.d_asnap) { dev_free(p); p = nullptr; }
  dev_free(m.d_ebase);
  m.d_ebase = nullptr;
  dev_free(m.d_win);
  m.d_win = nullptr;
  dev_free(m.d_vals); dev_free(m.d_snap); dev_free(m.d_keys); dev_free(m.d_state); dev_free(m.d_count); dev_free(m.d_rep);
  m.d_vals = m.d_snap = nullptr; m.d_keys = nullptr; m.d_state = m.d_count = nullptr; m.d_rep = nullptr;
  dev_free(m.d_hdr); dev_free(m.d_link); dev_free(m.d_elen); dev_free(m.d_rec);
  m.d_hdr = nullptr; m.d_link = nullptr; m.d_elen = nullptr; m.d_rec = nullptr;
  m.pool_cap = m.list_cap = 0;
  m.data_cap = 0;
  m.n_vals = m.n_elen = m.n_link = m.n_rec = 0;
  dev_free(m.d_tag);
  m.d_tag = nullptr;
  m.n_tag = 0;
  dev_free(m.d_trep);
  m.d_trep = nullptr;
  m.n_trep = 0;
  m.trep_r = 0;
  dev_free(m.d_vsnap);
  m.d_vsnap = nullptr;
  m.n_vsnap = 0;
  dev_free(m.d_tsnap);
  m.d_tsnap = nullptr;
  m.n_tsnap = 0;
  dev_free(m.d_rsnap); dev_free(m.d_lsnap); dev_free(m.d_esnap); dev_free(m.d_vsnap2); dev_free(m.d_tsnap2);
  m.d_rsnap = nullptr; m.d_lsnap = nullptr; m.d_esnap = nullptr; m.d_vsnap2 = nullptr; m.d_tsnap2 = nullptr;
  m.n_rsnap = m.n_lsnap = m.n_esnap = m.n_vsnap2 = m.n_tsnap2 = 0;
  m.dsnap = false;
  m.links_stale = false;
}

int ordered_upload(xe_vm* vm, HostMap& m, uint64_t slack, uint64_t slack_bytes);
int ordered_download(xe_vm* vm, HostMap& m);

int upload_map_table(xe_vm* vm, xe_stream_t s) {
  std::vector<XeDevMap> dm(vm->maps.size());
  memset(dm.data(), 0, dm.size() * sizeof(XeDevMap));
  for (size_t i = 1; i < vm->maps.size(); i++) {
    HostMap& m = vm->maps[i];
    XeDevMap& d = dm[i];
    d.kind = m.dkind;
    d.btype = m.def.type;
    d.key_size = m.def.key_size;
    d.value_size = m.def.value_size;
    d.max_entries = m.def.max_entries;
    d.big = m.big;
    d.vals_bytes = m.vals_bytes;
    d.vals = m.d_vals;
    d.keys = m.d_keys;
    d.state = m.d_state;
    d.count = m.d_count;
    d.cap = m.cap;
    d.kwords = m.kwords;
    d.rwords = (m.dkind == XE_DM_HASH || m.dkind == XE_DM_LRU) ? xe_hash_rwords(m.kwords) : 0;
    d.rep = m.d_rep;
    d.rep_stride = m.rep_stride;
    d.nrep = m.nrep;
    d.hdr = m.d_hdr;
// ... 399 lines not shown
  if (int rc = upload_map_table(vm, s)) return rc;
  if (!vm->d_aux && dev_alloc((void**)&vm->d_aux, kAuxWords * 8)) return fail(vm, XE_ERR_DEVICE, "device alloc (aux)");
  return XE_OK;
}

XeGen gen_layout(uint32_t nl, uint32_t nobj, uint32_t nframes, uint32_t nvc, uint32_t nbm, uint64_t nbytes, uint64_t* total) {
  XeGen g{};
  g.nl = nl; g.nobj = nobj; g.nframes = nframes; g.nvc = nvc; g.nbm = nbm; g.nbytes = nbytes;
  g.mark_words = (((nobj + 31) & ~31u) + ((nvc + 31) & ~31u) + ((nbm + 31) & ~31u)) / 32;
  uint64_t at = 0;
  auto field = [&](uint64_t& off, uint64_t bytes_per_lane) {
    off = at;
    at = (at + bytes_per_lane * nl + 255) & ~uint64_t(255);
  };
  field(g.o_ov, 8ull * nobj);
  field(g.o_oh, 4ull * nobj);
  field(g.o_ot, 4ull * nobj);
  field(g.o_ofree, 4ull * nobj);
  field(g.o_mark, 4ull * g.mark_words);
  field(g.o_frm, 2ull * XE_FRAME_SIZE * nframes);
  field(g.o_ctx, 2ull * 24);
  field(g.o_vc, 2ull * XE_FRAME_SIZE * nvc);
  field(g.o_vcinfo, 4ull * nvc);
  field(g.o_vfree, 4ull * nvc);
  field(g.o_bm, 16ull * nbm);
  field(g.o_bfree, 4ull * nbm);
  field(g.o_pres, 4ull * 17 * 8);
  g.o_key = at;
  field(g.o_bytes, nbytes);
  *total = at;
  return g;
}

constexpr int kMaxBlocksPerCu = 4;
uint32_t grid_blocks(uint32_t n, int per_cu, int cus) {
  uint64_t chunks = (uint64_t(n) + 63) / 64;
  uint64_t blocks = (chunks + 3) / 4;
  if (per_cu > kMaxBlocksPerCu) per_cu = kMaxBlocksPerCu;
  uint64_t maxb = (per_cu > 0 && cus > 0) ? uint64_t(per_cu) * uint64_t(cus) : 256ull * 4;
  if (const char* e = xe_tuning_env("XE_MAX_BLOCKS")) maxb = std::max(1ll, atoll(e));
  return uint32_t(std::max<uint64_t>(1, std::min(blocks, maxb)));
}

}

extern "C" {

int xe_default_settings(xe_settings* s) {
  if (!s) return XE_ERR_INVAL;
  memset(s, 0, sizeof *s);
  s->stack_frame_size = 256;
  s->max_stack_frames = 8;
  s->max_steps = 1u << 20;
  s->ingress_ifindex = 1;
  s->rx_queue_index = 0;
  s->device = 0;
  s->mode = XE_MODE_AUTO;
  return XE_OK;
}

int xe_create(const xe_settings* s, xe_vm** out) {
  if (!out) return XE_ERR_INVAL;
  xe_vm* vm = new xe_vm();
  if (s) vm->settings = *s;
  else xe_default_settings(&vm->settings);
  if (vm->settings.stack_frame_size == 0) vm->settings.stack_frame_size = 256;
  if (vm->settings.max_stack_frames == 0) vm->settings.max_stack_frames = 8;
  if (vm->settings.max_steps == 0) vm->settings.max_steps = 1u << 20;
  if (vm->settings.stack_frame_size != 256 || vm->settings.max_stack_frames != 8) {
    delete vm;
    return XE_ERR_UNSUPPORTED;
  }
  if (set_device(vm->settings.device)) { delete vm; return XE_ERR_DEVICE; }
#ifndef XE_HOSTSIM
  if (hipStreamCreateWithFlags(&vm->stream, hipStreamNonBlocking) != hipSuccess) { delete vm; return XE_ERR_DEVICE; }
#endif
  *out = vm;
  return XE_OK;
}

void xe_destroy(xe_vm* vm) {
  if (!vm) return;
  set_device(vm->settings.device);
  for (uint32_t si : vm->pending) (void)vm->slots[si].done.wait();
  vm->pending.clear();
  for (auto& sl : vm->slots) {
    dev_free(sl.d_aux); host_free(sl.h_aux);
    sl.t0.fini(); sl.t1.fini(); sl.done.fini();
  }
  dev_free(vm->d_poison);
  stream_destroy(vm->cancel_stream);
  dev_free(vm->d_trace_pk); dev_free(vm->d_trace); dev_free(vm->d_trace_cnt);
  dev_free(vm->d_listrun); dev_free(vm->d_popflag); dev_free(vm->d_popbase); dev_free(vm->d_popused);
  host_free(vm->h_hostcall);
  for (auto& m : vm->maps) map_free_device(m);
  dev_free(vm->d_progs); dev_free(vm->d_prog_off); dev_free(vm->d_maps); dev_free(vm->d_aux);
  dev_free(vm->d_arena_par); dev_free(vm->d_arena_seq); dev_free(vm->d_ksnap);
  dev_free(vm->d_umem); dev_free(vm->d_desc); dev_free(vm->d_res); dev_free(vm->d_ver); dev_free(vm->d_regs);
  dev_free(vm->d_usnap); dev_free(vm->d_ovl); dev_free(vm->d_app); dev_free(vm->d_app_sort); dev_free(vm->d_relink);
  dev_free(vm->d_mo); dev_free(vm->d_mo_keys); dev_free(vm->d_mo_vals); dev_free(vm->d_mo_found); dev_free(vm->d_ms);
  keyed_free(vm);
  vm->t0.fini(); vm->t1.fini(); vm->t2.fini();
#ifndef XE_HOSTSIM
  if (vm->stream) (void)hipStreamDestroy(vm->stream);
#endif
  delete vm;
}

const char* xe_last_error(const xe_vm* vm) { return vm ? vm->last_error.c_str() : "null vm"; }

int xe_add_raw_program(xe_vm* vm, const uint64_t* insns, uint32_t n, int32_t* idx) {
  if (!vm || (!insns && n)) return XE_ERR_INVAL;
  if (int rc = xe_sync(vm)) return rc;
  std::vector<XeUop> prog;
  std::string err;
  int rc = translate(insns, n, prog, err);
  if (rc) return fail(vm, rc, err);
  lift_rmw(prog);
  vm->programs.push_back(std::move(prog));
  if (idx) *idx = int32_t(vm->programs.size() - 1);
  return XE_OK;
}

int xe_set_entrypoint(xe_vm* vm, int32_t idx) {
  if (!vm) return XE_ERR_INVAL;
  if (int rc = xe_sync(vm)) return rc;
  if (idx < 1 || int32_t(vm->programs.size()) <= idx) return fail(vm, XE_ERR_INVAL, "program index out of bounds");
  vm->entry = idx;
  return XE_OK;
}

int xe_add_map(xe_vm* vm, const xe_map_def* def, const void* init, size_t init_len, int32_t* idx) {
  if (!vm || !def) return XE_ERR_INVAL;
  vm->staged_slot = -1;
  if (int rc = xe_sync(vm)) return rc;
  if (vm->maps.size() > XE_H_MAX_MAPS) return fail(vm, XE_ERR_UNSUPPORTED, "at most 63 maps");
  HostMap m;
  m.def = *def;
  switch (def->type) {
    case XE_MAP_ARRAY: case XE_MAP_PERCPU_ARRAY: case XE_MAP_PROG_ARRAY: case XE_MAP_ARRAY_OF_MAPS:
      m.dkind = XE_DM_ARRAY;
      m.vals_bytes = uint64_t(def->value_size) * def->max_entries;
      break;
    case XE_MAP_HASH: case XE_MAP_PERCPU_HASH: case XE_MAP_HASH_OF_MAPS:
      if (def->key_size > XE_MAX_KEY) return fail(vm, XE_ERR_UNSUPPORTED, "device hash maps support keys up to 64 bytes");
      m.dkind = XE_DM_HASH;
      if (def->max_entries > kHashCapMax) return fail(vm, XE_ERR_UNSUPPORTED, "hash map max_entries too large (<= 2^27)");
      m.cap = uint32_t(hash_cap(def->max_entries));
      m.kwords = (def->key_size + 7) / 8;
      m.vals_bytes = uint64_t(m.cap + 1) * def->value_size;
      m.keys.assign(size_t(m.cap + 1) * m.kwords, 0);
      m.state.assign(size_t(m.cap) + 1, 0);
      break;
    case XE_MAP_LRU_HASH: case XE_MAP_LRU_PERCPU_HASH:
      if (def->key_size > XE_MAX_KEY) return fail(vm, XE_ERR_UNSUPPORTED, "device hash maps support keys up to 64 bytes");
      m.dkind = XE_DM_LRU;
      if (def->max_entries > (kHashCapMax >> 1)) return fail(vm, XE_ERR_UNSUPPORTED, "LRU hash map max_entries too large (<= 2^26)");
      m.cap = uint32_t(hash_cap(def->max_entries));
      if (def->max_entries >= (1u << (XE_H_SLOT_BITS - 2)))
        m.pool_limit = std::min<uint64_t>(kHashCapMax, uint64_t(big_fields(2ull * def->max_entries + (1u << 20))) << XE_H_SLOT_BITS);
      m.kwords = (def->key_size + 7) / 8;
      break;
    case XE_MAP_QUEUE: case XE_MAP_STACK:
      m.dkind = XE_DM_LIST;
      m.stack = def->type == XE_MAP_STACK;
      break;
    case XE_MAP_PERF_EVENT_ARRAY:
      m.dkind = XE_DM_PERF;
      break;
    default:
      return fail(vm, XE_ERR_MAPTYPE, "map type not yet implemented");
  }
  {
// ... 811 lines not shown
              std::chrono::duration<double, std::milli>(std::chrono::steady_clock::now() - tm0).count(), n);
  }
  void keyed_trace(const char* why) const {
    if (xe_tuning_env("XE_KEYED_TRACE")) fprintf(stderr, "keyed: %s (n=%u)\n", why, n);
  }

  int prepare();
  int read_aux();
  int rollback(bool hash_records);
  int snap_records();
  int fold();
  int sequential();
  int replay_in_order() { used = XE_MODE_SEQUENTIAL; return sequential(); }

  KeyedResult kfail(int rc, const char* msg) { err = fail(vm, rc, msg); return KeyedResult::Error; }
  KeyedResult kerror() { err = -1; return KeyedResult::Error; }
  KeyedResult kreplay(const char* why, bool hash_records = false);
  int krollback();
  int kstep(uint32_t st, uint32_t items) { return launch_keyed(&K, vm->d_maps, vm->d_skip, st, items, s); }
  int read_small() { return d2h(small.data(), vm->d_ksmall, XE_KS_WORDS * 4, s) || dsync(s); }
  KeyedResult keyed_spec(bool& finished);
  KeyedResult keyed_build();
  KeyedResult keyed_capacity();
  KeyedResult keyed_evictions();
  KeyedResult keyed_order();
  KeyedResult keyed_reserve();
  KeyedResult keyed_remainder();
  KeyedResult keyed_chains();
  KeyedResult keyed();
  KeyedResult keyed_with_retries();
  int keyed_first();

  int list_setup();
  int list_init();
  int list_read() { return d2h(&lr, vm->d_listrun, sizeof lr, s) || dsync(s); }
  int pass();
  int ranked_passes();
  int list_sensitivity();
  int parallel();
  int after_conflict();
  int results_stand();
  int publish();
};

int BatchRun::prepare() {
  vm->staged_slot = -1;
  for (size_t i = 1; i < vm->maps.size(); i++) vm->maps[i].dsnap = false;
  if (stats) memset(stats, 0, sizeof *stats);
  if (int rc = xe_sync(vm)) return rc;
  s = stream ? (xe_stream_t)stream : vm->stream;
  if (int rc = prepare_run(vm, s)) return rc;
  tmark("prepare_run");
  if (n && (!d_umem || !d_desc)) return fail(vm, XE_ERR_INVAL, "null umem/desc");
  vm->delta_base = true;

  P = batch_params(vm, d_umem, umem_len, d_desc, n, d_results, d_verdicts, d_regs, vm->d_aux);
  aux_used = 16 + size_t(kRep) * P.rep_words;
  {
    bool lru = false;
    for (size_t i = 1; i < vm->maps.size(); i++) lru = lru || vm->maps[i].dkind == XE_DM_LRU;
    if (lru && vm->lru_epoch >= kLruEpochMax && lru_renumber(vm, s)) return fail(vm, XE_ERR_DEVICE, "LRU renumber");
    const uint64_t e[2] = {lru ? (++vm->lru_epoch) << 48 : 0, 0};
    for (size_t i = 1; i < vm->maps.size(); i++)
      if (vm->maps[i].dkind == XE_DM_LRU && (h2d(vm->maps[i].d_hdr + 5, e, 16, s) || dsync(s)))
        return fail(vm, XE_ERR_DEVICE, "LRU epoch");
  }
  if (P.trace && dmemset(vm->d_trace_cnt, 0, vm->trace_pk.size() * 4, s)) return fail(vm, XE_ERR_DEVICE, "trace reset");
  hostcalls = calls_host_helper(vm);

  mode = vm->settings.mode;
  if (int rc = select_engine(vm, jit, jit_general)) return rc;
  general = !jit || jit_general;
  {
    std::vector<const void*> src;
    std::vector<void*> dst;
    std::vector<uint64_t> words;
    for (size_t i = 1; i < vm->maps.size(); i++) {
      HostMap& m = vm->maps[i];
      if (m.ordered()) continue;
      src.push_back(m.d_vals);
      dst.push_back(m.d_snap);
      words.push_back(m.vals_alloc / 8);
    }
    if (launch_prologue(src.data(), dst.data(), words.data(), uint32_t(src.size()), vm->d_aux, aux_used, s))
      return fail(vm, XE_ERR_DEVICE, "prologue");
  }
  keep_pkts = mode == XE_MODE_AUTO && umem_len && may_write_packet(vm->programs[vm->entry]);
  if (keep_pkts && (ensure_buf(&vm->d_usnap, &vm->d_usnap_cap, umem_len) || d2d(vm->d_usnap, d_umem, umem_len, s)))
    return fail(vm, XE_ERR_DEVICE, "packet snapshot");
  if (keep_pkts && n > 1) {
    size_t need = 0;
    uint32_t flag = 0;
    if (launch_desc_overlap(d_desc, n, umem_len, nullptr, &need, nullptr, s) ||
        ensure_buf(&vm->d_ovl, &vm->d_ovl_cap, need + 256))
      return fail(vm, XE_ERR_DEVICE, "device alloc (descriptor overlap check)");
    uint32_t* d_flag = (uint32_t*)((uint8_t*)vm->d_ovl + ((need + 255) & ~size_t(255)));
    if (launch_desc_overlap(d_desc, n, umem_len, vm->d_ovl, &need, d_flag, s) || d2h(&flag, d_flag, 4, s) || dsync(s))
      return fail(vm, XE_ERR_DEVICE, "descriptor overlap check");
    overlap = flag != 0;
  }
  aux.resize(aux_used);
  ordmaps = has_ordered_maps(vm);
  if (jit && keyed_candidate(vm)) variant_kernel(vm, jit, kKeyedVariant);
  vm->t0.rec(s);
  tmark("setup");
  if (!vm->keyed_hint_set && n > 0) {
    vm->keyed_hint_set = true;
    if (lru_update_sites(vm)) vm->keyed_hint = true;
  }
  return XE_OK;
}

int BatchRun::read_aux() {
  if (d2h(aux.data(), vm->d_aux, aux_used * 8, s) || dsync(s)) return -1;
  reduce_aux(aux.data(), P.nmaps, P.rep_words, red);
  return 0;
}

struct HashSnap {
  HostMap* m;
  uint64_t off, rb;
};
uint64_t hash_snapshot_layout(xe_vm* vm, std::vector<HashSnap>& out) {
  uint64_t off = 0;
  for (size_t i = 1; i < vm->maps.size(); i++) {
    HostMap& m = vm->maps[i];
    if (m.dkind != XE_DM_HASH) continue;
    out.push_back({&m, off, hash_record_bytes(m)});
    off += out.back().rb + 8;
  }
  return off;
}

int BatchRun::rollback(bool hash_records) {
  for (size_t i = 1; i < vm->maps.size(); i++) {
    HostMap& m = vm->maps[i];
    if (!m.ordered() && d2d(m.d_vals, m.d_snap, m.vals_alloc, s)) return -1;
  }
  if (hash_records) {
    std::vector<HashSnap> snaps;
    hash_snapshot_layout(vm, snaps);
    for (const HashSnap& h : snaps) {
      uint8_t* at = (uint8_t*)vm->d_ksnap + h.off;
      if (d2d(h.m->d_keys, at, h.rb, s) || d2d(h.m->d_count, at + h.rb, 4, s)) return -1;
    }
    for (size_t i = 1; i < vm->maps.size(); i++) {
      HostMap& m = vm->maps[i];
      if (m.dkind == XE_DM_LRU && m.dsnap) {
        if (lru_dev_restore(m, s)) return -1;
      } else if (m.ordered() && ordered_upload(vm, m, vm->ord_slack, vm->ord_slack_bytes)) {
        return -1;
      }
    }
  }
  if (keep_pkts && d2d(d_umem, vm->d_usnap, umem_len, s)) return -1;
  return dmemset(vm->d_aux, 0, aux_used * 8, s);
}

int BatchRun::snap_records() {
  std::vector<HashSnap> snaps;
  const uint64_t kb = hash_snapshot_layout(vm, snaps);
  if (kb && ensure_buf((void**)&vm->d_ksnap, &vm->d_ksnap_bytes, kb)) return fail(vm, XE_ERR_DEVICE, "device alloc (snapshot)");
  for (const HashSnap& h : snaps) {
    uint8_t* at = (uint8_t*)vm->d_ksnap + h.off;
    if (d2d(at, h.m->d_keys, h.rb, s) || d2d(at + h.rb, h.m->d_count, 4, s)) return fail(vm, XE_ERR_DEVICE, "snapshot");
  }
  return XE_OK;
}

int BatchRun::fold() {
  for (size_t i = 1; i < vm->maps.size(); i++) {
    HostMap& m = vm->maps[i];
    if (m.nrep > 1 && fold_map(m, s)) return -1;
    if (m.dkind == XE_DM_LRU && m.trep_r > 1 && launch_lru_tag_fold(m.d_tag, m.d_trep, m.pool_cap, m.trep_r, m.d_hdr, s)) return -1;
  }
  return 0;
}

int BatchRun::sequential() {
  if (int rc = snap_records()) return rc;
  if (int rc = ordered_rollback_point(vm, s)) return rc;
  P.seq_prefetch = may_write_packet(vm->programs[vm->entry]) ? 0u : 1u;
  if (P.seq_prefetch) {
    const char* pk = xe_tuning_env("XE_SEQ_PEEK");
    if (!pk || atoi(pk)) P.seq_prefetch |= 2u;
  }
  for (int attempt = 0;; attempt++) {
    P.mode = XE_MODE_SEQUENTIAL;
    if (general && ensure_arena(vm, true, 1, P.gen)) return fail(vm, XE_ERR_NOMEM, "device alloc (replay arena)");
    bool table = false;
    for (size_t i = 1; i < vm->maps.size(); i++) {
      if (vm->maps[i].dkind != XE_DM_LRU) continue;
      const int r = lru_log_build(vm, vm->maps[i], s);
      if (r < 0) return fail(vm, XE_ERR_DEVICE, "LRU order log");
      table = table || r > 0;
    }
    if (table) {
      if (int rc = upload_map_table(vm, s)) return rc;
      P.maps = vm->d_maps;
    }
    vm->t1.rec(s);
    void* sj = (jit && !jit_general && n >= kSeqScalarMin) ? variant_kernel(vm, jit, kSeqVariant) : nullptr;
    if (launch_emulator(sj ? sj : jit, &P, 1, 64, s)) return fail(vm, XE_ERR_DEVICE, "kernel launch");
    vm->t2.rec(s);
    if (hostcalls && serve_hostcalls(vm->h_hostcall, s)) return fail(vm, XE_ERR_DEVICE, "kernel failed (host helpers)");
    if (read_aux()) return fail(vm, XE_ERR_DEVICE, "kernel failed");
    kms += Timer::ms(vm->t1, vm->t2);
    if (!(red[0] & XE_FLAG_CAPACITY)) {
      for (size_t i = 1; i < vm->maps.size(); i++)
        if (vm->maps[i].dkind == XE_DM_LRU) vm->maps[i].links_stale = true;
      return XE_OK;
    }
    if (attempt >= 6) return fail(vm, XE_ERR_NOMEM, "the ordered replay outgrew its device arena");
    vm->seq_scale *= 4;
    vm->ord_slack *= 4;
    vm->ord_slack_bytes *= 4;
    if (rollback(true)) return fail(vm, XE_ERR_DEVICE, "rollback");
    for (size_t i = 1; i < vm->maps.size(); i++) {
      HostMap& m = vm->maps[i];
      if (m.dkind != XE_DM_LRU) continue;
      m.dev_dirty = true;
      if (map_download(vm, m)) return fail(vm, XE_ERR_DEVICE, "map download");
      m.host_dirty = true;
    }
    if (prepare_run(vm, s)) return fail(vm, XE_ERR_DEVICE, "rollback");
    for (size_t i = 1; i < vm->maps.size(); i++)
      if (vm->maps[i].dkind == XE_DM_LRU && lru_dev_snapshot(vm->maps[i], s)) return fail(vm, XE_ERR_DEVICE, "LRU snapshot");
    P.maps = vm->d_maps;
  }
}


int BatchRun::krollback() {
  if (rollback(false)) return -1;
  return ordmaps ? ordered_hdr_restore(vm, kh0, s) : 0;
}

KeyedResult BatchRun::kreplay(const char* why, bool hash_records) {
  keyed_trace(why);
  if (hash_records ? rollback(true) : krollback()) return kerror();
  return KeyedResult::Replay;
}

KeyedResult BatchRun::keyed_spec(bool& finished) {
  finished = false;
  kjit = variant_kernel(vm, jit, kKeyedVariant);
  if (jit && !kjit) return KeyedResult::Replay;
  dmax = 4096, dcap = 4096;
  while (dmax < 2ull * n && dmax < (1u << 30)) dmax <<= 1;
  const uint64_t dwant = vm->keyed_dnext ? vm->keyed_dnext : std::max<uint64_t>(4096, n / 4);
  while (dcap < dwant && dcap < dmax) dcap <<= 1;
  tmark("keyed start");
  if (keyed_alloc(vm, n, dcap)) return kfail(XE_ERR_NOMEM, "device alloc (keyed execution)");
  tmark("keyed alloc");
  kh0.clear();
  if (ordmaps) {
    if ((err = ordered_rollback_point(vm, s))) return KeyedResult::Error;
    tmark("map snapshot");
    if (ordered_hdr_read(vm, kh0, s)) return kfail(XE_ERR_DEVICE, "ordered map header");
    tmark("hdr read");
  }
  K = vm->kd;
  K.n = n;
  if (dmemset(K.dkid, 0, uint64_t(K.dcap) * 8, s) || dmemset(vm->d_ksmall, 0, XE_KS_WORDS * 4, s) ||
      dmemset(K.dfirst, 0xff, uint64_t(K.dcap) * 4, s) || dmemset(K.dvict, 0xff, uint64_t(K.dcap) * 4, s))
    return kfail(XE_ERR_DEVICE, "keyed reset");
  kgrid = parallel_grid(vm, kjit, general, n, P.nmaps);
  X = P;
  if (general && ensure_arena(vm, false, kgrid * 256, X.gen)) return kfail(XE_ERR_NOMEM, "device alloc (arena)");
  tmark("arena");
  X.mode = XE_MODE_SPEC;
  X.K = K;
  if (launch_emulator(kjit, &X, kgrid, 256, s) || fold()) return kfail(XE_ERR_DEVICE, "kernel launch (keyed spec)");
  if (read_aux()) return kfail(XE_ERR_DEVICE, "kernel failed (keyed spec)");
  const uint32_t sflags = uint32_t(red[0]);
  if (ordmaps && (sflags & XE_FLAG_CAPACITY) && !(sflags & XE_FLAG_ORDERED)) {
    const int g = ordered_grow(vm, kh0, s);
    if (g < 0) return kfail(XE_ERR_DEVICE, "ordered map room");
    if (g == 1) {
      if (rollback(false) || prepare_run(vm, s)) return kfail(XE_ERR_DEVICE, "rollback");
      P.maps = vm->d_maps;
      keyed_trace("spec capacity: grown");
      return KeyedResult::Retry;
    }
  }
  if (sflags & (XE_FLAG_ORDERED | XE_FLAG_CAPACITY)) return kreplay("spec ordered/capacity");
  if (!(sflags & XE_FLAG_KEYED)) {
    if (run_conflict(red, P.nmaps)) return kreplay("spec conflict");
    if (ordmaps && ordered_finalize(vm, kh0, n, s)) return kfail(XE_ERR_DEVICE, "ordered map appends");
    used = XE_MODE_PARALLEL;
    finished = true;
  }
  return KeyedResult::Done;
}

KeyedResult BatchRun::keyed_build() {
  small.assign(XE_KS_WORDS, 0);
  if (kstep(XE_KS_DSET, n)) return kfail(XE_ERR_DEVICE, "keyed build");
  for (int round = 0;; round++) {
    if (round >= 64) return kreplay("union rounds");
    if (dmemset(K.changed, 0, 4, s) || kstep(XE_KS_UNION, n) || read_small()) return kfail(XE_ERR_DEVICE, "keyed build");
    if (!small[XE_KS_CHANGED]) break;
  }
  if (kstep(XE_KS_COMPRESS, K.dcap) || kstep(XE_KS_ASSIGN, n) || kstep(XE_KS_COUNT, K.dcap) || read_small())
    return kfail(XE_ERR_DEVICE, "keyed build");
  if (small[XE_KS_ERR] & 8u) {
    vm->keyed_dnext = dmax;
    if (dcap < dmax) {
      keyed_trace("D full");
      if (krollback()) return kerror();
      return KeyedResult::Retry;
    }
  }
  if (small[XE_KS_ERR]) return kreplay(small[XE_KS_ERR] & 16u ? "root walk" : "key log overflow");
  uint64_t nd = 0;
  for (uint32_t i = 0; i < 64; i++) nd += small[XE_KS_DCOUNT + i];
  uint64_t next = 4096;
  while (next < 4 * nd && next < dmax) next <<= 1;
  vm->keyed_dnext = uint32_t(next);
  return KeyedResult::Done;
}

KeyedResult BatchRun::keyed_capacity() {
  evict.clear();
  for (size_t i = 1; i < vm->maps.size() && i < 64; i++) {
    HostMap& m = vm->maps[i];
    const uint64_t nd = small[XE_KS_DINS + i];
    if ((m.dkind != XE_DM_HASH && m.dkind != XE_DM_LRU) || !nd) continue;
    uint64_t cnt = 0;
    if (m.dkind == XE_DM_HASH) {
      uint32_t c32 = 0;
      if (d2h(&c32, m.d_count, 4, s) || dsync(s)) return kfail(XE_ERR_DEVICE, "count");
      cnt = c32;
    } else {
      cnt = kh0[i * 8 + 2];
      const uint64_t ev = cnt + nd > m.def.max_entries ? cnt + nd - m.def.max_entries : 0;
      if (kh0[i * 8 + 3] + (nd - ev) > m.pool_cap) {
        if (krollback() || map_download(vm, m)) return kerror();
        vm->ord_slack = std::max<uint64_t>(vm->ord_slack, 2 * nd + 4096);
        m.host_dirty = true;
        if (prepare_run(vm, s)) return kfail(XE_ERR_DEVICE, "ordered map room");
        P.maps = vm->d_maps;
        keyed_trace("LRU pool grown");
        return KeyedResult::Retry;
      }
    }
    if (cnt + nd > m.def.max_entries) {
      if (m.dkind != XE_DM_LRU) return kreplay("capacity");
      evict[i] = cnt + nd - m.def.max_entries;
    }
  }
  return KeyedResult::Done;
}

KeyedResult BatchRun::keyed_evictions() {
  if (evict.empty()) return KeyedResult::Done;
  size_t eb = 0;
  if (kstep(XE_KS_FIRST, n) || kstep(XE_KS_EKEY, K.dcap) || launch_keyed_esort(&K, nullptr, &eb, s) ||
      ensure_buf(&vm->d_ksort, &vm->d_ksort_cap, eb) || launch_keyed_esort(&K, vm->d_ksort, &eb, s))
    return kfail(XE_ERR_DEVICE, "keyed evictions");
  uint64_t off = 0;
  for (size_t i = 1; i < vm->maps.size() && i < 64; i++) {
    HostMap& m = vm->maps[i];
    if (m.dkind != XE_DM_LRU) continue;
    const uint32_t nd = small[XE_KS_DINS + i];
    if (evict.count(i)) {
      const uint64_t cnt = kh0[i * 8 + 2];
      size_t rb = 0;
      if (launch_lru_relink(m.d_tsnap, m.pool_cap, uint32_t(cnt), m.d_link, m.d_hdr, nullptr, &rb, 2, s) ||
          ensure_buf(&vm->d_relink, &vm->d_relink_cap, rb) ||
          launch_lru_relink(m.d_tsnap, m.pool_cap, uint32_t(cnt), m.d_link, m.d_hdr, vm->d_relink, &rb, 2, s))
        return kfail(XE_ERR_DEVICE, "keyed evictions (order)");
      K.em = uint32_t(i);
      K.eoff = uint32_t(off);
      K.efree = uint32_t(m.def.max_entries - cnt);
      K.ecnt0 = uint32_t(cnt);
      K.etsnap = m.d_tsnap;
      K.vorder = lru_sorted_ids(vm->d_relink, m.pool_cap);
      if (kstep(XE_KS_EVICT, nd) || kstep(XE_KS_EMARK, nd)) return kfail(XE_ERR_DEVICE, "keyed evictions");
    }
    off += nd;
  }
  if (read_small()) return kfail(XE_ERR_DEVICE, "keyed evictions");
  if (small[XE_KS_ERR] & 8u) {
    vm->keyed_dnext = dmax;
    if (dcap < dmax) {
      keyed_trace("D full (victims)");
      if (krollback()) return kerror();
      return KeyedResult::Retry;
    }
  }
  if (small[XE_KS_ERR]) return kreplay("eviction seen by the batch");
  K.em = 0;
  return KeyedResult::Done;
}

KeyedResult BatchRun::keyed_order() {
  uint32_t end_bit = 1;
  while ((1ull << end_bit) <= K.dcap) end_bit++;
  size_t sb = 0;
  if (kstep(XE_KS_IOTA, n) || launch_keyed_sort(&K, n, end_bit, nullptr, &sb, s) ||
      ensure_buf(&vm->d_ksort, &vm->d_ksort_cap, sb) || launch_keyed_sort(&K, n, end_bit, vm->d_ksort, &sb, s))
    return kfail(XE_ERR_DEVICE, "keyed sort");
  if (kstep(XE_KS_NCHAIN, n) || read_small()) return kfail(XE_ERR_DEVICE, "keyed build");
  K.nO = small[XE_KS_NO];
  if (kstep(XE_KS_CSTART, K.nO) || kstep(XE_KS_CLONG, K.nO) || read_small()) return kfail(XE_ERR_DEVICE, "keyed build");
  if (small[XE_KS_LONG]) return kreplay("long chain");
  return KeyedResult::Done;
}

KeyedResult BatchRun::keyed_reserve() {
  if (krollback() || snap_records()) return kfail(XE_ERR_DEVICE, "rollback");
  if (ordmaps && kstep(XE_KS_LRUID, K.dcap)) return kfail(XE_ERR_DEVICE, "keyed value ids");
  if (kstep(XE_KS_RESERVE, K.dcap) || read_small()) return kfail(XE_ERR_DEVICE, "keyed reserve");
  if (small[XE_KS_ERR]) return kreplay("reserve", true);
  return KeyedResult::Done;
}

KeyedResult BatchRun::keyed_remainder() {
  X.mode = XE_MODE_PARALLEL;
  X.K = K;
  X.K.skip = vm->d_skip;
  if (K.nO < n) {
    XeParams Y = X;
    const uint32_t pgrid = parallel_grid(vm, jit, general, n, P.nmaps);
    if (general && ensure_arena(vm, false, pgrid * 256, Y.gen)) return kfail(XE_ERR_NOMEM, "device alloc (arena)");
    if (launch_emulator(jit, &Y, pgrid, 256, s) || fold()) return kfail(XE_ERR_DEVICE, "kernel launch (keyed parallel)");
  }
  return KeyedResult::Done;
}

KeyedResult BatchRun::keyed_chains() {
  {
    size_t sb2 = 0;
    if (kstep(XE_KS_CFLAG, K.nO) || launch_keyed_scan(&K, K.nO, nullptr, &sb2, s) ||
        ensure_buf(&vm->d_ksort, &vm->d_ksort_cap, sb2) || launch_keyed_scan(&K, K.nO, vm->d_ksort, &sb2, s) ||
        kstep(XE_KS_CLIST, K.nO) || dmemset(vm->d_ksmall + XE_KS_CNEXT, 0, 4, s))
      return kfail(XE_ERR_DEVICE, "keyed chain list");
  }
  X.mode = XE_MODE_CHAIN;
  X.K.skip = nullptr;
  const uint32_t cgrid = std::max<uint32_t>(1, std::min<uint32_t>(kgrid, (K.nO + 255) / 256));
  if (general && ensure_arena(vm, false, cgrid * 256, X.gen)) return kfail(XE_ERR_NOMEM, "device alloc (arena)");
  if (launch_emulator(kjit, &X, cgrid, 256, s) || kstep(XE_KS_UNNEW, K.dcap)) return kfail(XE_ERR_DEVICE, "kernel launch (keyed chains)");
  if (read_aux() || read_small()) return kfail(XE_ERR_DEVICE, "kernel failed (keyed chains)");
  if (run_conflict(red, P.nmaps)) return kreplay("chain conflict", true);
  auto inserts = [&](size_t i) {
    uint32_t add = 0;
    for (uint32_t k = 0; k < XE_KSTRIPES; k++) add += small[XE_KS_CINS + i * XE_KSTRIPES + k];
    return add;
  };
  for (const auto& [i, ev] : evict)
    if (inserts(i) != small[XE_KS_DINS + i]) return kreplay("eviction ranks", true);
  for (size_t i = 1; i < vm->maps.size() && i < 64; i++) {
    HostMap& m = vm->maps[i];
    const uint32_t add = inserts(i);
    if (!add) continue;
    if (m.dkind == XE_DM_HASH) {
      uint32_t cnt = 0;
      if (d2h(&cnt, m.d_count, 4, s) || dsync(s)) return kfail(XE_ERR_DEVICE, "count");
      cnt += add;
      if (h2d(m.d_count, &cnt, 4, s) || dsync(s)) return kfail(XE_ERR_DEVICE, "count");
    } else if (m.dkind == XE_DM_LRU) {
      uint64_t cnt = 0;
      if (d2h(&cnt, m.d_hdr + 2, 8, s) || dsync(s)) return kfail(XE_ERR_DEVICE, "count");
      cnt += add;
      if (evict.count(i)) cnt -= evict[i];
      if (h2d(m.d_hdr + 2, &cnt, 8, s) || dsync(s)) return kfail(XE_ERR_DEVICE, "count");
    }
  }
  if (ordmaps && ordered_finalize(vm, kh0, n, s)) return kfail(XE_ERR_DEVICE, "ordered map appends");
  vm->last_grid = kgrid;
  used = XE_MODE_KEYED;
  return KeyedResult::Done;
}

KeyedResult BatchRun::keyed() {
  bool finished = false;
  KeyedResult r = keyed_spec(finished);
  if (r != KeyedResult::Done || finished) return r;
  if ((r = keyed_build()) != KeyedResult::Done) return r;
  if ((r = keyed_capacity()) != KeyedResult::Done) return r;
  if ((r = keyed_evictions()) != KeyedResult::Done) return r;
  if ((r = keyed_order()) != KeyedResult::Done) return r;
  if ((r = keyed_reserve()) != KeyedResult::Done) return r;
  if ((r = keyed_remainder()) != KeyedResult::Done) return r;
  return keyed_chains();
}

KeyedResult BatchRun::keyed_with_retries() {
  KeyedResult r = keyed();
  for (int t = 0; r == KeyedResult::Retry && t < 3; t++) r = keyed();
  return r == KeyedResult::Retry ? KeyedResult::Replay : r;
}

int BatchRun::keyed_first() {
  const KeyedResult r = keyed_with_retries();
  if (r == KeyedResult::Error) return err;
  if (r == KeyedResult::Replay) {
    vm->keyed_backoff = kKeyedBackoff;
    if (ordmaps) vm->ord_backoff = kKeyedBackoff;
    if (int rc = replay_in_order()) return rc;
  }
  conflict = used != XE_MODE_PARALLEL;
  vm->t1.rec(s);
  if (dsync(s)) return fail(vm, XE_ERR_DEVICE, "sync");
  kms += Timer::ms(vm->t0, vm->t1);
  return XE_OK;
}


int BatchRun::list_setup() {
  lists = ordmaps && n > 0 && has_list_maps(vm);
  pops = lists && may_pop(vm);
  if (!lists) return XE_OK;
  if (!vm->d_listrun && dev_alloc((void**)&vm->d_listrun, sizeof(XeListRun))) return fail(vm, XE_ERR_NOMEM, "device alloc (lists)");
  P.list = vm->d_listrun;
  if (pops && vm->pop_n < n) {
    dev_free(vm->d_popflag); dev_free(vm->d_popbase); dev_free(vm->d_popused);
    vm->d_popflag = vm->d_popbase = vm->d_popused = nullptr;
    vm->pop_n = 0;
    if (dev_alloc((void**)&vm->d_popflag, size_t(n) * 4) || dev_alloc((void**)&vm->d_popbase, size_t(n) * 4 * XE_POP_SLOTS) ||
        dev_alloc((void**)&vm->d_popused, size_t(n) * 4))
      return fail(vm, XE_ERR_NOMEM, "device alloc (pop ranks)");
    vm->pop_n = n;
  }
  return XE_OK;
}

int BatchRun::list_init() {
  memset(&lr, 0, sizeof lr);
  for (size_t i = 1; i < vm->maps.size() && i < 64; i++)
    if (vm->maps[i].dkind == XE_DM_LIST) lr.cnt0[i] = uint32_t(ord_h0[i * 8 + 1]);
  for (int i = 0; i < 64; i++) lr.push[i] = lr.senslo[i] = 0xffffffffu;
  return h2d(vm->d_listrun, &lr, sizeof lr, s);
}

int BatchRun::pass() {
  if (launch_emulator(pj, &P, vm->last_grid, 256, s)) return fail(vm, XE_ERR_DEVICE, "kernel launch");
  vm->t1.rec(s);
  if (fold()) return fail(vm, XE_ERR_DEVICE, "replica fold");
  if (read_aux()) return fail(vm, XE_ERR_DEVICE, "kernel failed");
  kms = Timer::ms(vm->t0, vm->t1);
  flags = uint32_t(red[0]);
  conflict = run_conflict(red, P.nmaps);
  return XE_OK;
}

int BatchRun::ranked_passes() {
  P.pop_mode = 1;
  P.popflag = vm->d_popflag;
  P.popbase = nullptr;
  if (dmemset(vm->d_popflag, 0, size_t(n) * 4, s)) return fail(vm, XE_ERR_DEVICE, "pop flags");
  if (int rc = pass()) return rc;
  tmark("count pass");
  if (conflict) return XE_OK;
  if (list_read()) return fail(vm, XE_ERR_DEVICE, "list run");
  uint64_t mask = lr.popmask;
  bool ranked = false;
  for (int it = 0; it < 4 && !conflict; it++) {
    if (__builtin_popcountll(mask) > int(XE_POP_SLOTS)) break;
    XePopSlots sl;
    memset(sl.slot, 0xff, sizeof sl.slot);
    uint32_t ns = 0;
    for (uint32_t m = 0; m < 64; m++)
      if ((mask >> m) & 1) sl.slot[m] = uint8_t(ns++);
    memcpy(P.pop_slot, sl.slot, sizeof sl.slot);
    P.pop_stride = n;
    if (it == 0 ? launch_pop(vm->d_popflag, vm->d_popused, n, 0, 0, sl, nullptr, s)
                : d2d(vm->d_popused, vm->d_popflag, size_t(n) * 4, s))
      return fail(vm, XE_ERR_DEVICE, "pop ranks");
    for (uint32_t j = 0; j < ns; j++) {
      XeKeyed S{};
      S.iota = vm->d_popflag;
      S.ckey = vm->d_popbase + size_t(j) * n;
      size_t sb = 0;
      if (launch_pop(vm->d_popused, vm->d_popflag, n, 1, j, sl, nullptr, s) ||
          launch_keyed_scan(&S, n, nullptr, &sb, s) || ensure_buf(&vm->d_ksort, &vm->d_ksort_cap, sb) ||
          launch_keyed_scan(&S, n, vm->d_ksort, &sb, s))
        return fail(vm, XE_ERR_DEVICE, "pop ranks");
    }
    if (rollback(false) || ordered_hdr_restore(vm, ord_h0, s) || list_init()) return fail(vm, XE_ERR_DEVICE, "pop ranks");
    tmark("ranks");
    P.pop_mode = 2;
    P.popbase = vm->d_popbase;
    if (int rc = pass()) return rc;
    tmark("ranked pass");
    if (conflict) break;
    if (list_read()) return fail(vm, XE_ERR_DEVICE, "list run");
    if (lr.newlist) {
      mask |= lr.popmask;
      continue;
    }
    if (ensure_buf(&vm->d_ksort, &vm->d_ksort_cap, 256)) return fail(vm, XE_ERR_NOMEM, "pop ranks");
    uint32_t* d_flag = (uint32_t*)vm->d_ksort;
    uint32_t mismatch = 0;
    if (dmemset(d_flag, 0, 4, s) || launch_pop(vm->d_popflag, vm->d_popused, n, 2, 0, sl, d_flag, s) ||
        d2h(&mismatch, d_flag, 4, s) || dsync(s))
      return fail(vm, XE_ERR_DEVICE, "pop ranks");
    if (!mismatch) {
      ranked = true;
      popped = mask;
      break;
    }
  }
  if (!ranked && !conflict) {
    list_conflict = conflict = true;
    flags |= XE_FLAG_ORDERED;
  }
  return XE_OK;
}

int BatchRun::list_sensitivity() {
  if (list_read()) return fail(vm, XE_ERR_DEVICE, "list run");
  for (int i = 0; i < 64; i++)
    if (lr.sens[i] > lr.push[i]) list_conflict = true;
  if (!list_conflict) return XE_OK;
  conflict = true;
  if (!(flags & XE_FLAG_ORDERED)) {
    seg_cut = n;
    for (int i = 0; i < 64; i++)
      if (lr.sens[i] > lr.push[i]) seg_cut = std::min(seg_cut, lr.senslo[i] >= lr.push[i] ? lr.senslo[i] : lr.push[i]);
// ... 76 lines not shown
    uint32_t j = 0;
    for (uint32_t mi = 0; mi < 64; mi++) {
      if (!((popped >> mi) & 1)) continue;
      uint32_t base = 0;
      if (d2h(&base, vm->d_popbase + size_t(j) * n + (n - 1), 4, s) || dsync(s)) return fail(vm, XE_ERR_DEVICE, "pop count");
      const uint64_t k = std::min<uint64_t>(uint64_t(base) + ((last_used >> (8 * j)) & 0xffu), ord_h0[mi * 8 + 1]);
      if (vm->maps[mi].stack) h0[mi * 8 + 1] -= k;
      if (k) took.push_back({mi, k});
      j++;
    }
  }
  tmark("before finalize");
  if (ordered_finalize(vm, h0, n, s)) return fail(vm, XE_ERR_DEVICE, "ordered map appends");
  tmark("finalize");
  for (const auto& t : took) {
    HostMap& m = vm->maps[t.first];
    const uint64_t k = t.second;
    uint64_t hdr[8];
    if (d2h(hdr, m.d_hdr, 64, s) || dsync(s)) return fail(vm, XE_ERR_DEVICE, "pops");
    if (!m.stack) hdr[0] = (hdr[0] + k) % m.list_cap;
    hdr[1] -= k;
    if (h2d(m.d_hdr, hdr, 64, s) || dsync(s)) return fail(vm, XE_ERR_DEVICE, "pops");
  }
  return XE_OK;
}

int BatchRun::publish() {
  if (n > 0) vm->keyed_hint = used == XE_MODE_KEYED;
  if (used == XE_MODE_KEYED) red[0] |= XE_FLAG_ORDERED;
  record_widths(vm, red, P.nmaps);
  if (used == XE_MODE_SEQUENTIAL || used == XE_MODE_KEYED) {
    std::vector<uint32_t> counts(vm->maps.size(), 0);
    for (size_t i = 1; i < vm->maps.size(); i++)
      if (vm->maps[i].dkind == XE_DM_HASH && d2h(&counts[i], vm->maps[i].d_count, 4, s)) return fail(vm, XE_ERR_DEVICE, "count");
    if (dsync(s)) return fail(vm, XE_ERR_DEVICE, "sync");
    for (size_t i = 1; i < vm->maps.size(); i++)
      if (vm->maps[i].dkind == XE_DM_HASH) vm->maps[i].live = counts[i];
  }
  note_run(vm, red, used);
  tmark("done");
  if (n > 0)
    for (size_t i = 1; i < vm->maps.size(); i++) vm->maps[i].dev_dirty = true;
  publish_stats(stats, red, n, used, conflict, kms, jit ? XE_ENGINE_JIT : XE_ENGINE_INTERP,
                used == XE_MODE_SEQUENTIAL ? 1 : vm->last_grid);
  return XE_OK;
}

}

extern "C" {

int xe_run_batch_device(xe_vm* vm, void* d_umem, uint64_t umem_len, const void* d_desc, uint32_t n,
                        void* d_results, void* d_verdicts, void* d_regs, void* stream, xe_batch_stats* stats) {
  if (!vm) return XE_ERR_INVAL;
  BatchRun b{vm, d_umem, umem_len, d_desc, n, d_results, d_verdicts, d_regs, stream, stats};
  if (int rc = b.prepare()) return rc;
  const bool automatic = b.mode == XE_MODE_AUTO;
  const bool ord_par = !b.ordmaps || ordered_parallel_ok(vm);
  b.keyed_ok = automatic && n > 0 && !b.overlap && ord_par;
  const bool ord_seq = automatic && b.ordmaps && (!ord_par || vm->ord_backoff);
  if (ord_seq && vm->ord_backoff) vm->ord_backoff--;
  int rc = XE_OK;
  if (b.mode == XE_MODE_SEQUENTIAL || ord_seq || b.overlap || b.hostcalls) {
    rc = b.replay_in_order();
  } else if (b.keyed_ok && vm->keyed_hint) {
    rc = b.keyed_first();
  } else {
    if ((rc = b.parallel())) return rc;
    if (b.conflict && automatic && b.seg_cut >= kSegMin && b.seg_cut < n && segments_ok(vm, b.P)) {
      if (b.rollback(false) || (b.ordmaps && ordered_hdr_restore(vm, b.ord_h0, b.s))) return fail(vm, XE_ERR_DEVICE, "rollback");
      return run_segments(vm, d_umem, umem_len, d_desc, n, b.seg_cut, d_results, d_verdicts, d_regs, stream, stats);
    }
    if (b.conflict && (automatic || (b.flags & XE_FLAG_CAPACITY))) rc = b.after_conflict();
    else if (!b.conflict) rc = b.results_stand();
  }
  return rc ? rc : b.publish();
}

namespace {

int complete_oldest(xe_vm* vm) {
  const uint32_t si = vm->pending.front();
  xe_vm::Slot& sl = vm->slots[si];
  if (sl.done.wait()) {
    vm->pending.clear();
    return fail(vm, XE_ERR_DEVICE, "kernel failed (pipelined batch)");
  }
  const unsigned long long* aux = sl.h_aux;
  if (aux[XE_AUX_DECISION]) {
    vm->staged_slot = -1;
    const xe_stream_t s = sl.b.s;
    for (size_t i = 1; i < vm->maps.size(); i++) {
      HostMap& m = vm->maps[i];
      if (!m.ordered() && d2d(m.d_vals, m.d_asnap[sl.snap], m.vals_alloc, s)) return fail(vm, XE_ERR_DEVICE, "rollback");
    }
    if (dmemset(vm->d_poison, 0, 4, s)) return fail(vm, XE_ERR_DEVICE, "rollback");
    std::vector<xe_vm::Batch> redo;
    for (uint32_t k : vm->pending) redo.push_back(vm->slots[k].b);
    vm->pending.clear();
    for (const xe_vm::Batch& b : redo)
      if (int rc = xe_run_batch_device(vm, b.d_umem, b.umem_len, b.d_desc, b.n, b.d_results, b.d_verdicts, b.d_regs, b.s,
                                       b.stats))
        return rc;
    return XE_OK;
  }
  std::vector<unsigned long long> red;
  reduce_aux(aux, sl.nmaps, 16 + 2 * (sl.nmaps + 1), red);
  record_widths(vm, red, sl.nmaps);
  note_run(vm, red, XE_MODE_PARALLEL);
  if (sl.b.stats)
    publish_stats(sl.b.stats, red, sl.b.n, XE_MODE_PARALLEL, run_conflict(red, sl.nmaps), Timer::ms(sl.t0, sl.t1), sl.engine,
                  sl.grid);
  vm->pending.erase(vm->pending.begin());
  return XE_OK;
}

}

int xe_prepare(xe_vm* vm) {
  if (!vm) return XE_ERR_INVAL;
  if (int rc = xe_sync(vm)) return rc;
  if (int rc = prepare_run(vm, vm->stream)) return rc;
  void* jit = nullptr;
  bool jit_general = false;
  if (int rc = select_engine(vm, jit, jit_general)) return rc;
  if (jit && keyed_candidate(vm)) variant_kernel(vm, jit, kKeyedVariant);
  if (jit) variant_kernel(vm, jit, kLeanVariant);
  return dsync(vm->stream) ? fail(vm, XE_ERR_DEVICE, "sync") : XE_OK;
}

int xe_kernel_source(xe_vm* vm, int variant, char* buf, size_t cap, size_t* len) {
  if (!vm || variant < 0 || variant > 3) return XE_ERR_INVAL;
  if (int rc = xe_sync(vm)) return rc;
  if (int rc = prepare_run(vm, vm->stream)) return rc;
  if (vm->settings.engine == XE_ENGINE_INTERP || !jit_possible(vm))
    return fail(vm, XE_ERR_UNSUPPORTED, "the program runs on the interpreter");
  if (variant == 1 && !keyed_candidate(vm)) return fail(vm, XE_ERR_UNSUPPORTED, "no keyed variant for this program");
  const ProgTab t = prog_tab(vm);
  const size_t n = xe_jit_source_for(t.p.data(), t.n.data(), uint32_t(vm->programs.size() - 1), vm->entry,
                                     vm->dm_uploaded.data(), uint32_t(vm->dm_uploaded.size() - 1), variant, buf, cap);
  if (len) *len = n;
  if (n == 0) return fail(vm, XE_ERR_UNSUPPORTED, "no such kernel variant for this program");
  return XE_OK;
}

#ifdef XE_HOSTSIM
int xe_set_kernel_cache(const char*) { return XE_OK; }
int xe_compile_kernel_source(const char*, const char*, const char*, char* err, size_t errlen) {
  if (err && errlen) err[0] = 0;
  return XE_ERR_UNSUPPORTED;
}
int xe_kernel_object_name(const char*, const char*, char*, size_t) { return XE_ERR_UNSUPPORTED; }
int xe_kernel_cache_stats(uint64_t* hits, uint64_t* compiles, double* compile_s) {
  if (hits) *hits = 0;
  if (compiles) *compiles = 0;
  if (compile_s) *compile_s = 0;
  return XE_OK;
}
#endif

int xe_sync(xe_vm* vm) {
  if (!vm) return XE_ERR_INVAL;
  while (!vm->pending.empty())
    if (int rc = complete_oldest(vm)) {
      vm->pending.clear();
      return rc;
    }
// ... 64 lines not shown
  if (it == vm->trace_pk.end() || *it != packet) return fail(vm, XE_ERR_INVAL, "packet is not traced");
  const size_t slot = size_t(it - vm->trace_pk.begin());
  set_device(vm->settings.device);
  uint32_t cnt = 0;
  if (d2h(&cnt, vm->d_trace_cnt + slot, 4, vm->stream) || dsync(vm->stream)) return fail(vm, XE_ERR_DEVICE, "trace read");
  *nsteps = cnt;
  if (!out || !cap) return XE_OK;
  const uint32_t c = std::min(cap, cnt);
  if (c && (d2h(out, vm->d_trace + slot * vm->trace_max, size_t(c) * sizeof(xe_trace_rec), vm->stream) || dsync(vm->stream)))
    return fail(vm, XE_ERR_DEVICE, "trace read");
  return XE_OK;
}

int xe_set_helper(xe_vm* vm, uint32_t id, xe_helper_fn fn, void* user) {
  if (!vm || id >= 192) return XE_ERR_INVAL;
  if (int rc = xe_sync(vm)) return rc;
  const uint64_t b = 1ull << (id & 63);
  if (fn) {
    if (!vm->h_hostcall) {
      set_device(vm->settings.device);
      void* h = nullptr;
      void* d = nullptr;
      if (host_alloc_coherent(&h, sizeof(XeHostCall)) || host_device_ptr(&d, h)) return fail(vm, XE_ERR_NOMEM, "host helper mailbox");
      vm->h_hostcall = (XeHostCall*)h;
      vm->d_hostcall = (XeHostCall*)d;
    }
    vm->h_hostcall->fn[id] = fn;
    vm->h_hostcall->user[id] = user;
    vm->host_helpers[id >> 6] |= b;
    vm->nil_helpers[id >> 6] &= ~b;
  } else {
    vm->host_helpers[id >> 6] &= ~b;
    vm->nil_helpers[id >> 6] |= b;
  }
  return XE_OK;
}

int xe_reset_helper(xe_vm* vm, uint32_t id) {
  if (!vm || id >= 192) return XE_ERR_INVAL;
  if (int rc = xe_sync(vm)) return rc;
  const uint64_t b = 1ull << (id & 63);
  vm->host_helpers[id >> 6] &= ~b;
  vm->nil_helpers[id >> 6] &= ~b;
  return XE_OK;
}

int xe_run_batch_device_async(xe_vm* vm, void* d_umem, uint64_t umem_len, const void* d_desc, uint32_t n,
                              void* d_results, void* d_verdicts, void* d_regs, void* stream, xe_batch_stats* stats) {
  if (!vm) return XE_ERR_INVAL;
  if (stats) memset(stats, 0, sizeof *stats);
  xe_stream_t s = stream ? (xe_stream_t)stream : vm->stream;
  const bool entry_ok = vm->entry >= 1 && vm->entry < int32_t(vm->programs.size());
  if (!entry_ok || vm->settings.mode == XE_MODE_SEQUENTIAL || has_ordered_maps(vm) || vm->keyed_hint ||
      (umem_len && may_write_packet(vm->programs[vm->entry])) || !vm->trace_pk.empty() || calls_host_helper(vm))
    return xe_run_batch_device(vm, d_umem, umem_len, d_desc, n, d_results, d_verdicts, d_regs, stream, stats);
  if (n && (!d_umem || !d_desc)) return fail(vm, XE_ERR_INVAL, "null umem/desc");
  if (!vm->pending.empty() && vm->slots[vm->pending.back()].b.s != s)
    if (int rc = xe_sync(vm)) return rc;
  while (vm->pending.size() >= kAsyncDepth)
    if (int rc = complete_oldest(vm)) {
      vm->pending.clear();
      return rc;
    }
  if (int rc = prepare_run(vm, s)) return rc;
  void* jit = nullptr;
  bool jit_general = false;
  if (int rc = select_engine(vm, jit, jit_general)) return rc;
  const bool general = !jit || jit_general;

  const uint32_t si = vm->next_slot;
  const uint32_t ai = vm->next_snap, nai = (ai + 1) % (kAsyncDepth + 1);
  xe_vm::Slot& sl = vm->slots[si];
  if (!sl.d_aux) {
    if (dev_alloc((void**)&sl.d_aux, kAuxWords * 8) || dmemset(sl.d_aux, 0, kAuxWords * 8, s))
      return fail(vm, XE_ERR_DEVICE, "alloc (pipelined batch records)");
  }
  if (!sl.h_aux) {
    if (host_alloc((void**)&sl.h_aux, kAuxWords * 8) || host_device_ptr((void**)&sl.h_aux_dev, sl.h_aux))
      return fail(vm, XE_ERR_DEVICE, "alloc (pipelined batch records)");
  }
  if (!vm->d_poison) {
    if (dev_alloc((void**)&vm->d_poison, 8) || dmemset(vm->d_poison, 0, 8, s)) return fail(vm, XE_ERR_DEVICE, "alloc (poison)");
  }
  XeParams P = batch_params(vm, d_umem, umem_len, d_desc, n, d_results, d_verdicts, d_regs, sl.d_aux);
  P.mode = XE_MODE_PARALLEL;
  P.poison = vm->d_poison;
  const size_t aux_used = 16 + size_t(kRep) * P.rep_words;
  const bool staged = vm->staged_slot == int32_t(ai) && !vm->pending.empty() && vm->slots[vm->pending.back()].b.s == s;
  XeTailArgs A{};
  A.aux = sl.d_aux;
  A.host_aux = sl.h_aux_dev;
  A.poison = vm->d_poison;
  A.aux_words = uint32_t(aux_used);
  A.nrep = kRep;
  A.rep_words = P.rep_words;
  A.nmaps = P.nmaps;
  A.mode = vm->settings.mode;
  std::vector<const void*> src;
  std::vector<void*> dst;
  std::vector<uint64_t> words;
  std::vector<size_t> big;
  for (size_t i = 1; i < vm->maps.size(); i++) {
    HostMap& m = vm->maps[i];
    for (uint32_t k : {ai, nai})
      if (!m.d_asnap[k] && dev_alloc((void**)&m.d_asnap[k], m.vals_alloc))
        return fail(vm, XE_ERR_DEVICE, "device alloc (batch snapshot)");
    const bool small = m.vals_alloc <= kTailMapBytes && A.ntail < XE_TAIL_MAPS;
    if (small) {
      XeTailMap& T = A.tail[A.ntail++];
      T.vals = (unsigned long long*)m.d_vals;
      T.rep = (unsigned long long*)m.d_rep;
      T.snap = (unsigned long long*)m.d_asnap[nai];
      T.words = m.vals_alloc / 8;
      T.stride_words = m.rep_stride / 8;
      T.nrep = m.nrep > 1 ? m.nrep : 0;
    } else {
      big.push_back(i);
    }
    if (!small || !staged) {
      src.push_back(m.d_vals);
      dst.push_back(m.d_asnap[ai]);
      words.push_back(m.vals_alloc / 8);
    }
  }
  if (jit && !P.results && !P.regs) jit = variant_kernel(vm, jit, kLeanVariant);
  const uint32_t grid = parallel_grid(vm, jit, general, n, P.nmaps);
  if (general && ensure_arena(vm, false, grid * 256, P.gen)) return fail(vm, XE_ERR_NOMEM, "device alloc (arena)");
  if (!src.empty() && launch_prologue(src.data(), dst.data(), words.data(), uint32_t(src.size()), nullptr, 0, s))
    return fail(vm, XE_ERR_DEVICE, "prologue");
  sl.t0.rec(s);
  if (launch_emulator(jit, &P, grid, 256, s)) return fail(vm, XE_ERR_DEVICE, "kernel launch");
  sl.t1.rec(s);
  for (size_t i : big) {
    HostMap& m = vm->maps[i];
    if (m.nrep > 1 && fold_map(m, s))
      return fail(vm, XE_ERR_DEVICE, "replica fold");
  }
  if (launch_tail(&A, s)) return fail(vm, XE_ERR_DEVICE, "epilogue");
  sl.done.rec(s);
  vm->staged_slot = int32_t(nai);
  sl.snap = ai;
  vm->next_snap = nai;
  sl.b = xe_vm::Batch{d_umem, umem_len, d_desc, n, d_results, d_verdicts, d_regs, s, stats};
  sl.aux_used = aux_used;
  sl.nmaps = P.nmaps;
  sl.grid = grid;
  sl.engine = jit ? XE_ENGINE_JIT : XE_ENGINE_INTERP;
  vm->last_grid = grid;
  vm->pending.push_back(si);
  vm->next_slot = (si + 1) % kAsyncDepth;
  vm->delta_base = false;
  for (size_t i = 1; i < vm->maps.size(); i++) vm->maps[i].dev_dirty = true;
  return XE_OK;
}

int xe_run_batch_host(xe_vm* vm, uint8_t* umem, uint64_t umem_len, const xe_desc* desc, uint32_t n,
                      xe_result* results, uint32_t* verdicts, xe_regs* regs, xe_batch_stats* stats) {
  if (!vm) return XE_ERR_INVAL;
  if (set_device(vm->settings.device)) return fail(vm, XE_ERR_DEVICE, "hipSetDevice failed");
  xe_stream_t s = vm->stream;
  if (ensure_buf(&vm->d_umem, &vm->d_umem_cap, umem_len) || ensure_buf(&vm->d_desc, &vm->d_desc_cap, size_t(n) * 16) ||
      ensure_buf(&vm->d_res, &vm->d_res_cap, size_t(n) * sizeof(xe_result)) ||
      ensure_buf(&vm->d_ver, &vm->d_ver_cap, size_t(n) * 4) ||
      (regs && ensure_buf(&vm->d_regs, &vm->d_regs_cap, size_t(n) * sizeof(xe_regs))))
    return fail(vm, XE_ERR_DEVICE, "device alloc (batch)");
  Timer a, b;
  a.rec(s);
  if ((umem_len && h2d(vm->d_umem, umem, umem_len, s)) || (n && h2d(vm->d_desc, desc, size_t(n) * 16, s)))
    return fail(vm, XE_ERR_DEVICE, "H2D");
  int rc = xe_run_batch_device(vm, vm->d_umem, umem_len, vm->d_desc, n, results ? vm->d_res : nullptr,
                               verdicts ? vm->d_ver : nullptr, regs ? vm->d_regs : nullptr, s, stats);
  if (rc) return rc;
  if ((results && d2h(results, vm->d_res, size_t(n) * sizeof(xe_result), s)) ||
      (verdicts && d2h(verdicts, vm->d_ver, size_t(n) * 4, s)) ||
      (regs && d2h(regs, vm->d_regs, size_t(n) * sizeof(xe_regs), s)) ||
      (umem_len && may_write_packet(vm->programs[vm->entry]) && d2h(umem, vm->d_umem, umem_len, s)))
    return fail(vm, XE_ERR_DEVICE, "D2H");
  b.rec(s);
  if (dsync(s)) return fail(vm, XE_ERR_DEVICE, "sync");
  if (stats) stats->total_ms = Timer::ms(a, b);
  a.fini(); b.fini();
  return XE_OK;
}

int xe_map_dump_list(xe_vm* vm, int32_t mi, void* data, uint64_t data_cap, uint32_t* lens, uint64_t cap, uint64_t* count,
                     uint64_t* bytes) {
  HostMap* m = get_map(vm, mi);
  if (!m || (m->dkind != XE_DM_LIST && m->dkind != XE_DM_PERF)) return XE_ERR_INVAL;
  set_device(vm->settings.device);
  if (map_download(vm, *m)) return fail(vm, XE_ERR_DEVICE, "map download");
  uint64_t total = 0;
  for (auto& r : m->items) total += r.val.size();
  if (count) *count = m->items.size();
  if (bytes) *bytes = total;
  if (!data && !lens) return XE_OK;
  if (cap < m->items.size() || (data && data_cap < total)) return fail(vm, XE_ERR_INVAL, "dump buffer too small");
  uint64_t off = 0;
  for (size_t i = 0; i < m->items.size(); i++) {
    if (lens) lens[i] = uint32_t(m->items[i].val.size());
    if (data && !m->items[i].val.empty()) memcpy((uint8_t*)data + off, m->items[i].val.data(), m->items[i].val.size());
    off += m->items[i].val.size();
  }
  return XE_OK;
}

int xe_map_lru_order(xe_vm* vm, int32_t mi, void* keys, uint64_t cap, uint64_t* count) {
  HostMap* m = get_map(vm, mi);
  if (!m || m->dkind != XE_DM_LRU) return XE_ERR_INVAL;
  set_device(vm->settings.device);
  if (map_download(vm, *m)) return fail(vm, XE_ERR_DEVICE, "map download");
  if (count) *count = m->items.size();
  if (!keys) return XE_OK;
  if (cap < m->items.size()) return fail(vm, XE_ERR_INVAL, "buffer too small");
  for (size_t i = 0; i < m->items.size(); i++) {
    uint8_t* kd = (uint8_t*)keys + i * m->def.key_size;
    memset(kd, 0, m->def.key_size);
    if (!m->items[i].nil_key) memcpy(kd, m->items[i].key.data(), m->def.key_size);
  }
  return XE_OK;
}

int xe_map_push(xe_vm* vm, int32_t mi, const void* value) {
// ... 455 lines not shown
  return XE_OK;
}

static int map_scan_run(xe_vm* vm, int32_t mi, const xe_map_filter* f, void* keys, void* values, uint64_t cap_entries,
                        uint64_t* matched, void* stream, bool expire, bool host) {
  HostMap* m = nullptr;
  XeMapOp o{};
  xe_stream_t s = nullptr;
  const int rc = mapop_begin(vm, mi, 1, expire, host ? nullptr : stream, &m, &o, &s);
  if (rc < 0) return rc;
  if (expire && m->dkind != XE_DM_HASH) return fail(vm, XE_ERR_INVAL, "delete not available on this map type");
  if (!matched) return fail(vm, XE_ERR_INVAL, "null matched");
  const xe_map_filter all{};
  if (!f) f = &all;
  if (f->op >= kMfOps) return fail(vm, XE_ERR_INVAL, "map filter: unknown op");
  if (f->pad) return fail(vm, XE_ERR_INVAL, "map filter: pad must be 0");
  if (f->op != XE_MF_ALL) {
    if (f->width != 1 && f->width != 2 && f->width != 4 && f->width != 8) return fail(vm, XE_ERR_INVAL, "map filter: width must be 1, 2, 4 or 8");
    if (uint64_t(f->offset) + f->width > m->def.value_size) return fail(vm, XE_ERR_INVAL, "map filter: the field lies outside the value");
    o.f_off = f->offset;
    o.f_width = f->width;
    o.f_operand = f->operand;
  }
  o.f_op = f->op;
  if (m->dkind == XE_DM_ARRAY) o.nslots = m->def.max_entries;
  else if (m->def.key_size == 0) o.sbase = m->cap, o.nslots = 1;
  else o.nslots = m->cap;
  *matched = 0;
  const size_t tiles = xe_ms_tiles(o.nslots);
  if (!tiles) return XE_OK;
  if (ensure_buf(&vm->d_ms, &vm->d_ms_cap, tiles * (kMsRounds * 8 + 4))) return fail(vm, XE_ERR_DEVICE, "device alloc (map scan scratch)");
  o.bitmap = (uint64_t*)vm->d_ms;
  o.tile = (uint32_t*)(o.bitmap + tiles * kMsRounds);
  if (int r = mapop_steps(vm, o, {XE_MO_SCAN_SELECT, XE_MO_SCAN_SCAN}, s)) return r;
  uint32_t total = 0;
  if (d2h(&total, o.ctr + kMoMatched, 4, s) || dsync(s)) return fail(vm, XE_ERR_DEVICE, "map scan");
  *matched = total;
  const uint32_t r = uint32_t(std::min<uint64_t>(total, cap_entries));
  const bool out = keys || values;
  if (!r || (!expire && !out)) return XE_OK;
  const size_t kb = size_t(r) * o.key_size, vb = size_t(r) * o.value_size;
  if (ensure_buf(&vm->d_mo, &vm->d_mo_cap, kMoCounters * 4 + size_t(r) * 4)) return fail(vm, XE_ERR_DEVICE, "device alloc (map operation scratch)");
  o.ctr = (uint32_t*)vm->d_mo;
  o.slot = o.ctr + kMoCounters;
  o.n = r;
  if (host && ((keys && ensure_buf(&vm->d_mo_keys, &vm->d_mo_keys_cap, kb)) || (values && ensure_buf(&vm->d_mo_vals, &vm->d_mo_vals_cap, vb))))
    return fail(vm, XE_ERR_DEVICE, "map operation staging");
  o.keys_out = (uint8_t*)(!keys ? nullptr : host ? vm->d_mo_keys : keys);
  o.values_out = (uint8_t*)(!values ? nullptr : host ? vm->d_mo_vals : values);
  if (int e = mapop_steps(vm, o, {XE_MO_SCAN_SCATTER}, s)) return e;
  if (out)
    if (int e = mapop_steps(vm, o, {XE_MO_SCAN_COPY}, s)) return e;
  uint32_t cnt = 0;
  if (expire) {
    if (int e = mapop_steps(vm, o, {XE_MO_SCAN_EXPIRE}, s)) return e;
    if (d2h(&cnt, m->d_count, 4, s)) return fail(vm, XE_ERR_DEVICE, "map expire");
  }
  if (host && ((keys && kb && d2h(keys, vm->d_mo_keys, kb, s)) || (values && vb && d2h(values, vm->d_mo_vals, vb, s))))
    return fail(vm, XE_ERR_DEVICE, "map operation staging");
  if (dsync(s)) return fail(vm, XE_ERR_DEVICE, expire ? "map expire" : "map scan");
  if (expire) {
    m->live = cnt;
    m->dev_dirty = true;
    vm->staged_slot = -1;
  }
  return XE_OK;
}

int xe_map_scan_device(xe_vm* vm, int32_t mi, const xe_map_filter* f, void* d_keys, void* d_values, uint64_t cap_entries,
                       uint64_t* matched, void* stream) {
  return map_scan_run(vm, mi, f, d_keys, d_values, cap_entries, matched, stream, false, false);
}
int xe_map_expire_device(xe_vm* vm, int32_t mi, const xe_map_filter* f, void* d_keys, void* d_values, uint64_t cap_entries,
                         uint64_t* matched, void* stream) {
  return map_scan_run(vm, mi, f, d_keys, d_values, cap_entries, matched, stream, true, false);
}
int xe_map_scan(xe_vm* vm, int32_t mi, const xe_map_filter* f, void* keys, void* values, uint64_t cap_entries, uint64_t* matched) {
  return map_scan_run(vm, mi, f, keys, values, cap_entries, matched, nullptr, false, true);
}
int xe_map_expire(xe_vm* vm, int32_t mi, const xe_map_filter* f, void* keys, void* values, uint64_t cap_entries, uint64_t* matched) {
  return map_scan_run(vm, mi, f, keys, values, cap_entries, matched, nullptr, true, true);
}

int xe_debug_map_traffic(xe_vm* vm, int32_t mi, uint64_t* uploads, uint64_t* downloads) {
  HostMap* m = get_map(vm, mi);
  if (!m) return XE_ERR_INVAL;
  if (uploads) *uploads = m->uploads;
  if (downloads) *downloads = m->downloads;
  return XE_OK;
}

}

extern "C" {
int xe_debug_set_schedule(xe_vm* vm, uint32_t sched) {
  if (!vm) return XE_ERR_INVAL;
  if (int rc = xe_sync(vm)) return rc;
  vm->sched = sched;
  return XE_OK;
}

int xe_debug_set_lru_epoch(xe_vm* vm, uint64_t epoch) {
  if (!vm || epoch > kLruEpochMax) return XE_ERR_INVAL;
  if (int rc = xe_sync(vm)) return rc;
  vm->lru_epoch = epoch;
  return XE_OK;
}

int xe_debug_map_pool(xe_vm* vm, int32_t mi, uint64_t* room, uint64_t* next_id) {
  HostMap* m = get_map(vm, mi);
  if (!m || !m->ordered()) return XE_ERR_INVAL;
  if (int rc = xe_sync(vm)) return rc;
  set_device(vm->settings.device);
  if (int rc = prepare_run(vm, vm->stream)) return rc;
  uint64_t hdr[8];
  if (d2h(hdr, m->d_hdr, 64, vm->stream) || dsync(vm->stream)) return fail(vm, XE_ERR_DEVICE, "map header");
  if (room) *room = m->pool_cap;
  if (next_id) *next_id = m->dkind == XE_DM_PERF ? hdr[0] : hdr[m->dkind == XE_DM_LRU ? 3 : 2];
  return XE_OK;
}

int xe_translate_uops(const uint64_t* insns, uint32_t n, void* out, uint32_t cap) {
  std::vector<XeUop> prog;
  std::string err;
  int rc = translate(insns, n, prog, err);
  if (rc) return rc;
  lift_rmw(prog);
  if (out && cap >= prog.size()) memcpy(out, prog.data(), prog.size() * sizeof(XeUop));
  return int(prog.size());
}

int xe_debug_may_write_packet(const uint64_t* insns, uint32_t n) {
  std::vector<XeUop> prog;
  std::string err;
  int rc = translate(insns, n, prog, err);
  if (rc) return rc;
  return may_write_packet(prog) ? 1 : 0;
}

int xe_internal_vm_device(const xe_vm* vm) { return vm ? vm->settings.device : -1; }
void* xe_internal_vm_stream(xe_vm* vm) { return vm ? (void*)vm->stream : nullptr; }
int xe_internal_nmaps(const xe_vm* vm) { return vm ? int(vm->maps.size()) - 1 : -1; }
int xe_internal_may_write_packet(const xe_vm* vm) {
  if (!vm || vm->entry < 1 || vm->entry >= int32_t(vm->programs.size())) return 1;
  return may_write_packet(vm->programs[vm->entry]) ? 1 : 0;
}
int xe_internal_delta_sum(xe_vm* vm, void* acc, const void* in, uint64_t bytes, uint32_t lane) {
  set_device(vm->settings.device);
  return launch_delta_sum(acc, in, bytes, lane, vm->stream) || dsync(vm->stream) ? XE_ERR_DEVICE : XE_OK;
}
int xe_internal_alloc(xe_vm* vm, void** p, uint64_t bytes) {
  set_device(vm->settings.device);
  return dev_alloc(p, size_t(bytes)) ? XE_ERR_NOMEM : XE_OK;
}
void xe_internal_free(xe_vm* vm, void* p) {
  set_device(vm->settings.device);
  dev_free(p);
}
int xe_internal_copy(xe_vm* vm, void* dst, const void* src, uint64_t bytes) {
  set_device(vm->settings.device);
  return d2d(dst, src, size_t(bytes), vm->stream) || dsync(vm->stream) ? XE_ERR_DEVICE : XE_OK;
}

const char* xe_version(void) {
#ifdef XE_HOSTSIM
  return "xdpemu-hostsim 0.1 (CPU test build of the device logic; not the product)";
// ... 17 lines not shown
```

### gobpfld_amd/emulator.py

```python
from __future__ import annotations

import ctypes as C
from dataclasses import dataclass

import numpy as np

from . import _native as N

STATUS = {0: "OK", 1: "VMERR", 2: "PANIC", 3: "BUDGET", 4: "UNSUPPORTED"}
MAP_HASH, MAP_ARRAY, MAP_PROG_ARRAY, MAP_PERF_EVENT_ARRAY, MAP_PERCPU_HASH, MAP_PERCPU_ARRAY = 1, 2, 3, 4, 5, 6
MAP_LRU_HASH, MAP_LRU_PERCPU_HASH, MAP_ARRAY_OF_MAPS, MAP_HASH_OF_MAPS, MAP_QUEUE, MAP_STACK = 9, 10, 12, 13, 22, 23
ARRAY_TYPES = (MAP_ARRAY, MAP_PERCPU_ARRAY, MAP_PROG_ARRAY, MAP_ARRAY_OF_MAPS)
HASH_TYPES = (MAP_HASH, MAP_PERCPU_HASH, MAP_HASH_OF_MAPS, MAP_LRU_HASH, MAP_LRU_PERCPU_HASH)
LIST_TYPES = (MAP_QUEUE, MAP_STACK, MAP_PERF_EVENT_ARRAY)
MODE_AUTO, MODE_PARALLEL, MODE_SEQUENTIAL, MODE_KEYED = 0, 1, 2, 3
MODE_CANCELLED = 4
MODE_SEGMENTS = 5
E_HOST_HELPER, E_IN_HELPER = 17, 0x80
ENGINE_AUTO, ENGINE_INTERP, ENGINE_JIT = 0, 1, 2


class EmulatorError(RuntimeError):
    def __init__(self, rc: int, msg: str):
        super().__init__(f"{msg} (rc={rc})")
# ... 229 lines not shown
    def map_lookup_batch(self, m: int, keys):
        d = self.map_defs[m]
        k, n = self._mo_keys(m, keys)
        if self._is_dev(k):
            import torch
            vals = torch.empty((n, d.value_size), dtype=torch.uint8, device=k.device)
            found = torch.empty(n, dtype=torch.uint8, device=k.device)
            rc = self.lib.map_lookup_batch_device(self.h, m, k.data_ptr() or None, n, vals.data_ptr() or None,
                                                  found.data_ptr() or None, None)
        else:
            vals = np.zeros((n, d.value_size), dtype=np.uint8)
            found = np.zeros(n, dtype=np.uint8)
            rc = self.lib.map_lookup_batch(self.h, m, k.ctypes.data, n, vals.ctypes.data, found.ctypes.data)
        self._check(rc, "map lookup batch")
        return vals, found

    def map_update_batch_device(self, m: int, keys, values) -> None:
        d = self.map_defs[m]
        k, n = self._mo_keys(m, keys)
        if self._is_dev(k):
            import torch
            assert self._is_dev(values), "keys and values: both on the device, or both on the host"
            v = values.contiguous().view(torch.uint8).reshape(-1)
            assert len(v) == n * d.value_size
            torch.cuda.current_stream(v.device).synchronize()
            rc = self.lib.map_update_batch_device(self.h, m, k.data_ptr() or None, v.data_ptr() or None, n, None)
        else:
            v = np.ascontiguousarray(values).view(np.uint8).reshape(-1)
            assert len(v) == n * d.value_size
            rc = self.lib.map_update_batch_staged(self.h, m, k.ctypes.data, v.ctypes.data, n)
        self._check(rc, "map update batch (device)")

    def map_delete_batch(self, m: int, keys):
        k, n = self._mo_keys(m, keys)
        if self._is_dev(k):
            import torch
            found = torch.empty(n, dtype=torch.uint8, device=k.device)
            rc = self.lib.map_delete_batch_device(self.h, m, k.data_ptr() or None, n, found.data_ptr() or None, None)
        else:
            found = np.zeros(n, dtype=np.uint8)
            rc = self.lib.map_delete_batch(self.h, m, k.ctypes.data, n, found.ctypes.data)
        self._check(rc, "map delete batch")
        return found

    def _map_scan(self, m: int, flt, cap, on_device: bool, expire: bool):
        d = self.map_defs[m]
        ks = 4 if d.type in ARRAY_TYPES else d.key_size
        what = "map expire" if expire else "map scan"
        dev_fn = self.lib.map_expire_device if expire else self.lib.map_scan_device
        host_fn = self.lib.map_expire if expire else self.lib.map_scan
        cf = None if flt is None else N.MapFilter(flt.op, flt.offset, flt.width, 0, flt.operand)
        fp = None if cf is None else C.byref(cf)
        n = C.c_uint64(0)
        if on_device:
            import torch
            dev = torch.device("cuda", self.settings.device)
            torch.cuda.current_stream(dev).synchronize()
        if cap is None:
            self._check(self.lib.map_scan_device(self.h, m, fp, None, None, 0, C.byref(n), None), what)
            cap = n.value
        if on_device:
            keys = torch.empty((cap, ks), dtype=torch.uint8, device=dev)
            vals = torch.empty((cap, d.value_size), dtype=torch.uint8, device=dev)
            rc = dev_fn(self.h, m, fp, keys.data_ptr() or None, vals.data_ptr() or None, cap, C.byref(n), None)
        else:
            keys = np.zeros((cap, ks), dtype=np.uint8)
            vals = np.zeros((cap, d.value_size), dtype=np.uint8)
            rc = host_fn(self.h, m, fp, keys.ctypes.data if cap else None, vals.ctypes.data if cap else None, cap, C.byref(n))
        self._check(rc, what)
        r = min(int(n.value), cap)
        return keys[:r], vals[:r], int(n.value)

    def map_scan(self, m: int, flt: "MapFilter | None" = None, cap: int | None = None, on_device: bool = False):
        return self._map_scan(m, flt, cap, on_device, False)

    def map_expire(self, m: int, flt: "MapFilter | None" = None, cap: int | None = None, on_device: bool = False):
        return self._map_scan(m, flt, cap, on_device, True)

    def map_traffic(self, m: int) -> tuple[int, int]:
        up, down = C.c_uint64(), C.c_uint64()
        self._check(self.lib.debug_map_traffic(self.h, m, C.byref(up), C.byref(down)), "map traffic")
        return up.value, down.value

    def map_values_bytes(self, m: int) -> int:
        b = C.c_uint64()
        self._check(self.lib.map_values_bytes(self.h, m, C.byref(b)), "map values bytes")
        return b.value

    def run_batch(self, umem: np.ndarray, descs: np.ndarray, want_regs: bool = False) -> BatchResult:
        d_desc, d_res, d_regs = N.np_dtypes()
        assert umem.dtype == np.uint8 and umem.flags.c_contiguous
        descs = np.ascontiguousarray(descs, dtype=d_desc)
        n = len(descs)
        res = np.zeros(n, dtype=d_res)
        ver = np.zeros(n, dtype=np.uint32)
        regs = np.zeros(n, dtype=d_regs) if want_regs else None
        st = N.BatchStats()
        fn = self.lib.run_batch_host if self.lib.has("run_batch_host") else self.lib.run_batch
        rc = fn(self.h, umem.ctypes.data if umem.size else None, umem.size, descs.ctypes.data if n else None, n,
                res.ctypes.data if n else None, ver.ctypes.data if n else None,
                regs.ctypes.data if (regs is not None and n) else None, C.byref(st))
        self._check(rc, "run batch")
        return BatchResult(res, ver, regs, _stats_dict(st))

    def run_batch_host_ptrs(self, umem: int, umem_len: int, desc: int, n: int, verdicts: int = 0,
                            results: int = 0) -> dict:
        st = N.BatchStats()
        rc = self.lib.run_batch_host(self.h, umem or None, umem_len, desc or None, n, results or None,
                                     verdicts or None, None, C.byref(st))
        self._check(rc, "run batch (host pointers)")
        return _stats_dict(st)

    def run_batch_device(self, d_umem: int, umem_len: int, d_desc: int, n: int, d_results: int = 0,
                         d_verdicts: int = 0, d_regs: int = 0, stream: int = 0) -> dict:
        st = N.BatchStats()
        rc = self.lib.run_batch_device(self.h, d_umem or None, umem_len, d_desc or None, n, d_results or None,
                                       d_verdicts or None, d_regs or None, stream or None, C.byref(st))
        self._check(rc, "run batch (device)")
        return _stats_dict(st)

    def run_batch_device_async(self, d_umem: int, umem_len: int, d_desc: int, n: int, d_results: int = 0,
                               d_verdicts: int = 0, d_regs: int = 0, stream: int = 0) -> "PendingBatch":
        st = N.BatchStats()
        rc = self.lib.run_batch_device_async(self.h, d_umem or None, umem_len, d_desc or None, n, d_results or None,
                                             d_verdicts or None, d_regs or None, stream or None, C.byref(st))
        self._check(rc, "run batch (device, pipelined)")
        pb = PendingBatch(self, st)
        self._pending.append(pb)
        return pb

    def prepare(self) -> None:
        if self.lib.has("prepare"):
            self._check(self.lib.prepare(self.h), "prepare")

    def kernel_sources(self, variants=(0, 1, 2)) -> list[str]:
        out = []
        for variant in variants:
            n = C.c_size_t()
            rc = self.lib.kernel_source(self.h, variant, None, 0, C.byref(n))
            if rc == -95:
                continue
            self._check(rc, "kernel source")
            buf = C.create_string_buffer(n.value + 1)
            self._check(self.lib.kernel_source(self.h, variant, buf, n.value + 1, C.byref(n)), "kernel source")
            out.append(buf.value.decode())
        return out

    def set_schedule(self, sched: int) -> None:
        self._check(self.lib.debug_set_schedule(self.h, sched), "set schedule")

    def set_lru_epoch(self, epoch: int) -> None:
        self._check(self.lib.debug_set_lru_epoch(self.h, epoch), "set LRU epoch")

    def map_pool(self, m: int) -> tuple[int, int]:
        room, nxt = C.c_uint64(), C.c_uint64()
        self._check(self.lib.debug_map_pool(self.h, m, C.byref(room), C.byref(nxt)), "map pool")
        return room.value, nxt.value

    def sync(self) -> None:
        rc = self.lib.sync(self.h)
        self._pending.clear()
        self._check(rc, "sync")

    def cancel(self) -> int:
        k = C.c_uint32()
        rc = self.lib.cancel(self.h, C.byref(k))
# ... 113 lines not shown
```

### include/xdpemu.h

```cpp
#ifndef XDPEMU_H
#define XDPEMU_H

#if !defined(__HIPCC_RTC__)
#include <stddef.h>
#include <stdint.h>
#else
typedef unsigned char uint8_t;
typedef unsigned short uint16_t;
typedef unsigned int uint32_t;
typedef unsigned long long uint64_t;
typedef signed char int8_t;
typedef short int16_t;
typedef int int32_t;
typedef long long int64_t;
typedef unsigned long uintptr_t;
typedef __SIZE_TYPE__ size_t;
#endif

#ifdef __cplusplus
extern "C" {
#endif

#define XE_OK 0
#define XE_ERR_INVAL (-22)
// ... 171 lines not shown
#define XE_FPF_SEQUENTIAL 2
#define XE_FPF_UNALIGNED 4
#define XE_FPF_EPOCH 8
int xe_footprint(xe_vm* vm, uint64_t* out, uint32_t cap_words, uint32_t* nwords);
int xe_shard_check(const uint64_t* fps, uint32_t ngpus, uint32_t nwords, uint32_t* lanes);
int xe_epoch_begin(xe_vm* vm, void* stream);
int xe_epoch_end(xe_vm* vm);
int xe_map_state_bytes(xe_vm* vm, int32_t map_idx, uint64_t* bytes);
int xe_map_state_export(xe_vm* vm, int32_t map_idx, void* d_out, void* stream);
int xe_map_state_import(xe_vm* vm, int32_t map_idx, const void* d_in, void* stream);

int xe_map_lookup_batch_device(xe_vm* vm, int32_t map_idx, const void* d_keys, uint64_t count, void* d_values,
                               void* d_found, void* stream);
int xe_map_update_batch_device(xe_vm* vm, int32_t map_idx, const void* d_keys, const void* d_values, uint64_t count,
                               void* stream);
int xe_map_delete_batch_device(xe_vm* vm, int32_t map_idx, const void* d_keys, uint64_t count, void* d_found,
                               void* stream);
int xe_map_lookup_batch(xe_vm* vm, int32_t map_idx, const void* keys, uint64_t count, void* values, uint8_t* found);
int xe_map_update_batch_staged(xe_vm* vm, int32_t map_idx, const void* keys, const void* values, uint64_t count);
int xe_map_delete_batch(xe_vm* vm, int32_t map_idx, const void* keys, uint64_t count, uint8_t* found);

#define XE_MF_ALL 0
#define XE_MF_EQ 1
#define XE_MF_NE 2
#define XE_MF_LT 3
#define XE_MF_LE 4
#define XE_MF_GT 5
#define XE_MF_GE 6
#define XE_MF_ANYBITS 7
#define XE_MF_NOBITS 8
typedef struct xe_map_filter {
  uint32_t op;
  uint32_t offset;
  uint32_t width;
  uint32_t pad;
  uint64_t operand;
} xe_map_filter;
int xe_map_scan_device(xe_vm* vm, int32_t map_idx, const xe_map_filter* f, void* d_keys, void* d_values,
                       uint64_t cap_entries, uint64_t* matched, void* stream);
int xe_map_expire_device(xe_vm* vm, int32_t map_idx, const xe_map_filter* f, void* d_keys, void* d_values,
                         uint64_t cap_entries, uint64_t* matched, void* stream);
int xe_map_scan(xe_vm* vm, int32_t map_idx, const xe_map_filter* f, void* keys, void* values, uint64_t cap_entries,
                uint64_t* matched);
int xe_map_expire(xe_vm* vm, int32_t map_idx, const xe_map_filter* f, void* keys, void* values, uint64_t cap_entries,
                  uint64_t* matched);

typedef struct xe_multi xe_multi;
int xe_multi_create(xe_vm* const* vms, uint32_t ngpus, xe_multi** out);
void xe_multi_destroy(xe_multi* m);
int xe_run_batch_multi(xe_multi* m, void* const* d_umem, const uint64_t* umem_len, const void* const* d_desc,
                       const uint32_t* n, void* const* d_results, void* const* d_verdicts, xe_batch_stats* stats,
                       uint32_t* replayed);
const char* xe_multi_last_error(const xe_multi* m);

int xe_set_kernel_cache(const char* dir);
int xe_kernel_source(xe_vm* vm, int variant, char* buf, size_t cap, size_t* len);
int xe_compile_kernel_source(const char* src, const char* arch, const char* dir, char* err, size_t errlen);
int xe_kernel_object_name(const char* src, const char* arch, char* buf, size_t cap);
int xe_kernel_cache_stats(uint64_t* hits, uint64_t* compiles, double* compile_s);

#define XE_TRACE_MAX_PACKETS 4096
#define XE_TRACE_MAX_STEPS 65536
typedef struct xe_trace_rec {
    uint32_t packet;
    uint32_t step;
    int32_t pc;
    int32_t pi;
    uint32_t sf;
    uint8_t kind[11];
    uint8_t pad;
    int64_t val[11];
} xe_trace_rec;
int xe_trace_config(xe_vm* vm, const uint32_t* packets, uint32_t npk, uint32_t max_steps);
int xe_trace_read(xe_vm* vm, uint32_t packet, xe_trace_rec* out, uint32_t cap, uint32_t* nsteps);

typedef int (*xe_helper_fn)(void* user, uint32_t packet, const int64_t args[5], const uint8_t kinds[5], int64_t* r0);
int xe_set_helper(xe_vm* vm, uint32_t id, xe_helper_fn fn, void* user);
int xe_reset_helper(xe_vm* vm, uint32_t id);

int xe_debug_set_schedule(xe_vm* vm, uint32_t sched);
int xe_debug_set_lru_epoch(xe_vm* vm, uint64_t epoch);
int xe_debug_map_pool(xe_vm* vm, int32_t map, uint64_t* room, uint64_t* next_id);
int xe_debug_map_traffic(xe_vm* vm, int32_t map_idx, uint64_t* uploads, uint64_t* downloads);

const char* xe_version(void);
int xe_device_count(int* n);

#ifdef __cplusplus
}
#endif
#endif
```

Measured before the change: 56560.

## Fuse pipelined batch epilogue into emulator kernel via last-workgroup arrival counter

Removes the separate single-block tail kernel launch after each pipelined batch. The epilogue (aux harvest, replay decision, replica-to-values reduction) now runs inside the main emulator kernel, in whichever workgroup increments a device-side arrival counter last, using agent-scope atomics for coherence. This saves one kernel launch and its dependency gap per batch, but serialises the epilogue onto one workgroup at the tail of the main kernel and adds atomic traffic. The change also adds debug counters for launches and arrivals.

```diff
diff --git a/gobpfld_amd/_native.py b/gobpfld_amd/_native.py
--- a/gobpfld_amd/_native.py
+++ b/gobpfld_amd/_native.py
@@ -151,6 +151,8 @@
     "map_scan": (C.c_int, [P, C.c_int32, P, P, P, C.c_uint64, C.POINTER(C.c_uint64)]),
     "map_expire": (C.c_int, [P, C.c_int32, P, P, P, C.c_uint64, C.POINTER(C.c_uint64)]),
     "debug_map_traffic": (C.c_int, [P, C.c_int32, C.POINTER(C.c_uint64), C.POINTER(C.c_uint64)]),
+    "debug_launches": (C.c_int, [P, C.POINTER(C.c_uint64)]),
+    "debug_arrivals": (C.c_int, [P, C.POINTER(C.c_uint32)]),
     "multi_create": (C.c_int, [P, C.c_uint32, C.POINTER(P)]),
     "multi_destroy": (None, [P]),
     "multi_last_error": (C.c_char_p, [P]),
@@ -180,6 +182,7 @@
     "xe_debug_set_lru_epoch", "xe_debug_map_pool",
     "xe_map_lookup_batch_device", "xe_map_update_batch_device", "xe_map_delete_batch_device",
     "xe_map_lookup_batch", "xe_map_update_batch_staged", "xe_map_delete_batch", "xe_debug_map_traffic",
+    "xe_debug_launches", "xe_debug_arrivals",
     "xe_map_scan_device", "xe_map_expire_device", "xe_map_scan", "xe_map_expire",
     "xe_set_kernel_cache", "xe_kernel_source", "xe_compile_kernel_source", "xe_kernel_object_name",
     "xe_kernel_cache_stats",
diff --git a/gobpfld_amd/csrc/xe_internal.h b/gobpfld_amd/csrc/xe_internal.h
--- a/gobpfld_amd/csrc/xe_internal.h
+++ b/gobpfld_amd/csrc/xe_internal.h
@@ -257,6 +257,7 @@
 
 #define XE_TAIL_MAPS 4
 #define XE_TAIL_MAP_WORDS 2048
+#define XE_TAIL_REP_WORDS 256
 struct XeTailMap {
   unsigned long long* vals;
   unsigned long long* rep;
@@ -316,6 +317,8 @@
   int32_t entry;
   XeGen gen;
   const uint32_t* poison;
+  uint32_t* arrive;
+  XeTailArgs tail;
   uint32_t seq_prefetch;
   XeKeyed K;
   uint32_t sched;
diff --git a/gobpfld_amd/csrc/xe_interp.h b/gobpfld_amd/csrc/xe_interp.h
--- a/gobpfld_amd/csrc/xe_interp.h
+++ b/gobpfld_amd/csrc/xe_interp.h
@@ -3596,3 +3596,71 @@
     }
   }
 }
+
+#if defined(__HIPCC__)
+XE_DEV unsigned long long xe_coh_take64(unsigned long long* p) {
+  return __hip_atomic_exchange((XE_GP(unsigned long long))p, 0ull, __ATOMIC_RELAXED, __HIP_MEMORY_SCOPE_AGENT);
+}
+XE_DEV unsigned long long xe_coh_add64(unsigned long long* p, unsigned long long v) {
+  return __hip_atomic_fetch_add((XE_GP(unsigned long long))p, v, __ATOMIC_RELAXED, __HIP_MEMORY_SCOPE_AGENT);
+}
+XE_DEV unsigned int xe_coh_read32(unsigned int* p) {
+  return __hip_atomic_fetch_or((XE_GP(unsigned int))p, 0u, __ATOMIC_RELAXED, __HIP_MEMORY_SCOPE_AGENT);
+}
+XE_DEV void xe_lds_or64(XE_LP(unsigned long long) p, unsigned long long v) {
+  __hip_atomic_fetch_or(p, v, __ATOMIC_RELAXED, __HIP_MEMORY_SCOPE_WORKGROUP);
+}
+#else
+XE_DEV unsigned long long xe_coh_take64(unsigned long long* p) { return __atomic_exchange_n(p, 0ull, __ATOMIC_RELAXED); }
+XE_DEV unsigned long long xe_coh_add64(unsigned long long* p, unsigned long long v) { return __atomic_fetch_add(p, v, __ATOMIC_RELAXED); }
+XE_DEV unsigned int xe_coh_read32(unsigned int* p) { return __atomic_fetch_or(p, 0u, __ATOMIC_RELAXED); }
+XE_DEV void xe_lds_or64(unsigned long long* p, unsigned long long v) { *p |= v; }
+#endif
+
+template <class Sync>
+XE_DEV void batch_epilogue(const XeTailArgs& A, uint32_t t, uint32_t nt, XE_LP(unsigned long long) orw, Sync sync) {
+  for (uint32_t w = t; w < XE_TAIL_REP_WORDS + 2; w += nt) orw[w] = 0;
+  sync();
+  if (t == 0) orw[XE_TAIL_REP_WORDS + 1] = xe_coh_read32(A.poison);
+  for (uint32_t i = t; i < A.aux_words; i += nt) {
+    const unsigned long long v = xe_coh_take64(&A.aux[i]);
+    A.host_aux[i] = v;
+    if (i == 0) orw[XE_TAIL_REP_WORDS] = v;
+    else if (i >= 16 && v) xe_lds_or64(&orw[(i - 16) % A.rep_words], v);
+  }
+  sync();
+  const bool poisoned = orw[XE_TAIL_REP_WORDS + 1] != 0;
+  if (t == 0) {
+    const bool replay = !poisoned && xe_replay_decision(uint32_t(orw[XE_TAIL_REP_WORDS]), orw, A.rep_words, A.nmaps, A.mode);
+    A.host_aux[XE_AUX_DECISION] = replay ? 1ull : 0ull;
+    if (replay) *A.poison = 1u;
+  }
+  if (poisoned) return;
+  for (uint32_t f = 0; f < A.ntail; f++) {
+    const XeTailMap& T = A.tail[f];
+    for (uint64_t i = t; i < T.words; i += nt) {
+      unsigned long long r[16];
+#pragma unroll
+      for (uint32_t k = 0; k < 16; k++) r[k] = k < T.nrep ? xe_coh_take64(&T.rep[k * T.stride_words + i]) : 0ull;
+      unsigned long long s = 0;
+#pragma unroll
+      for (uint32_t k = 0; k < 16; k++) s += r[k];
+      T.snap[i] = xe_coh_add64(&T.vals[i], s) + s;
+    }
+  }
+}
+
+#if defined(__HIPCC__) && !XE_UNIFORM
+XE_DEV void batch_arrive(const XeParams& P) {
+  __shared__ __attribute__((aligned(16))) unsigned long long xe_tail_lds[XE_TAIL_REP_WORDS + 4];
+  asm volatile("s_waitcnt vmcnt(0)" ::: "memory");
+  __syncthreads();
+  if (threadIdx.x == 0)
+    xe_tail_lds[XE_TAIL_REP_WORDS + 2] =
+        __hip_atomic_fetch_add((XE_GP(unsigned int))P.arrive, 1u, __ATOMIC_RELAXED, __HIP_MEMORY_SCOPE_AGENT) == gridDim.x - 1;
+  __syncthreads();
+  if (!xe_tail_lds[XE_TAIL_REP_WORDS + 2]) return;
+  batch_epilogue(P.tail, threadIdx.x, blockDim.x, (XE_LP(unsigned long long))xe_tail_lds, [] { __syncthreads(); });
+  if (threadIdx.x == 0) __hip_atomic_store((XE_GP(unsigned int))P.arrive, 0u, __ATOMIC_RELAXED, __HIP_MEMORY_SCOPE_AGENT);
+}
+#endif
diff --git a/gobpfld_amd/csrc/xe_jit.cpp b/gobpfld_amd/csrc/xe_jit.cpp
--- a/gobpfld_amd/csrc/xe_jit.cpp
+++ b/gobpfld_amd/csrc/xe_jit.cpp
@@ -986,23 +986,34 @@
   } else {
     uint32_t wave = (blockIdx.x * blockDim.x + threadIdx.x) >> 6;
     uint32_t nwaves = (gridDim.x * blockDim.x) >> 6;
+    bool committer = false;  // this wave only issues the other waves' adds: no packets, no records
 #if XE_COMMITTER
     if (P.mode == XE_MODE_PARALLEL && blockDim.x == 256) {
       const uint32_t wib = threadIdx.x >> 6;
-      if (wib == 3) { committer_loop(L, P, (XE_LP(XeRing))xe_rings, 3); return; }
-      L.ring = (XE_LP(XeRing))&xe_rings[wib];
+      committer = wib == 3;
+      if (committer) committer_loop(L, P, (XE_LP(XeRing))xe_rings, 3);
+      else L.ring = (XE_LP(XeRing))&xe_rings[wib];
       wave = blockIdx.x * 3 + wib;
       nwaves = gridDim.x * 3;
     }
 #endif
-    parallel_packets(L, P, wave, nwaves, [&](uint32_t i, bool valid) __attribute__((always_inline)) {
-      int status = XE_ST_OK, code = 0; int32_t res_pc = 0; uint64_t steps = 0;
-      if (valid) xe_jit_body(L, P, status, code, res_pc, steps);
-      lane_finish(L, P, i, valid, status, code, res_pc, steps);
-    });
+    if (!committer)
+      parallel_packets(L, P, wave, nwaves, [&](uint32_t i, bool valid) __attribute__((always_inline)) {
+        int status = XE_ST_OK, code = 0; int32_t res_pc = 0; uint64_t steps = 0;
+        if (valid) xe_jit_body(L, P, status, code, res_pc, steps);
+        lane_finish(L, P, i, valid, status, code, res_pc, steps);
+      });
 #if XE_COMMITTER
     if (L.ring) ring_done(L.ring);
 #endif
+#if !XE_KEYED
+    if (P.arrive) {  // a pipelined batch: its epilogue runs in the workgroup that retires last
+      if (!committer) flush_wave_state(L, P);
+      batch_arrive(P);
+      return;
+    }
+#endif
+    if (committer) return;
   }
 #endif  // !XE_UNIFORM
   flush_wave_state(L, P);
diff --git a/gobpfld_amd/csrc/xe_kernel.hip b/gobpfld_amd/csrc/xe_kernel.hip
--- a/gobpfld_amd/csrc/xe_kernel.hip
+++ b/gobpfld_amd/csrc/xe_kernel.hip
@@ -23,6 +23,11 @@
     const uint32_t wave = (blockIdx.x * blockDim.x + threadIdx.x) >> 6;
     const uint32_t nwaves = (gridDim.x * blockDim.x) >> 6;
     parallel_packets(L, P, wave, nwaves, [&](uint32_t i, bool valid) { run_staged(L, P, i, valid); });
+    if (P.arrive) {
+      flush_wave_state(L, P);
+      batch_arrive(P);
+      return;
+    }
   }
   flush_wave_state(L, P);
 }
@@ -83,50 +88,6 @@
     for (uint64_t i = tid; i < A.words[g]; i += nth) A.dst[g][i] = A.src[g][i];
 }
 
-extern "C" __global__ void __launch_bounds__(1024) xe_tail_kernel(XeTailArgs A) {
-  __shared__ unsigned long long orw[257];
-  const uint32_t t = threadIdx.x, nt = blockDim.x;
-  for (uint32_t w = t; w <= 256; w += nt) orw[w] = 0;
-  const bool poisoned = *(volatile uint32_t*)A.poison != 0;
-  __syncthreads();
-  for (uint32_t i = t; i < A.aux_words; i += nt) {
-    const unsigned long long v = A.aux[i];
-    if (v) A.aux[i] = 0;
-    A.host_aux[i] = v;
-    if (i == 0) orw[256] = v;
-    else if (i >= 16 && v) atomicOr(&orw[(i - 16) % A.rep_words], v);
-  }
-  __syncthreads();
-  if (t == 0) {
-    const bool replay = !poisoned && xe_replay_decision(uint32_t(orw[256]), orw, A.rep_words, A.nmaps, A.mode);
-    A.host_aux[XE_AUX_DECISION] = replay ? 1ull : 0ull;
-    if (replay) *A.poison = 1u;
-  }
-  if (poisoned) return;
-  for (uint32_t f = 0; f < A.ntail; f++) {
-    const XeTailMap& T = A.tail[f];
-    for (uint64_t i = t; i < T.words; i += nt) {
-      unsigned long long r[16];
-#pragma unroll
-      for (uint32_t k = 0; k < 16; k++) r[k] = k < T.nrep ? T.rep[k * T.stride_words + i] : 0ull;
-      unsigned long long s = 0;
-#pragma unroll
-      for (uint32_t k = 0; k < 16; k++) {
-        s += r[k];
-        if (r[k]) T.rep[k * T.stride_words + i] = 0;
-      }
-      const unsigned long long v = T.vals[i] + s;
-      if (s) T.vals[i] = v;
-      T.snap[i] = v;
-    }
-  }
-}
-extern "C" int xe_launch_tail(const XeTailArgs* A, hipStream_t s) {
-  if (A->rep_words > 256) return -1;
-  hipLaunchKernelGGL(xe_tail_kernel, dim3(1), dim3(1024), 0, s, *A);
-  return hipGetLastError() == hipSuccess ? 0 : -1;
-}
-
 __global__ void xe_desc_split_kernel(const xe_desc* d, uint32_t n, uint64_t umem_len, unsigned long long* key,
                                      uint32_t* len) {
   for (uint64_t i = blockIdx.x * uint64_t(blockDim.x) + threadIdx.x; i < n; i += uint64_t(gridDim.x) * blockDim.x) {
diff --git a/gobpfld_amd/csrc/xe_kernels.h b/gobpfld_amd/csrc/xe_kernels.h
--- a/gobpfld_amd/csrc/xe_kernels.h
+++ b/gobpfld_amd/csrc/xe_kernels.h
@@ -29,7 +29,6 @@
                        uint32_t rwords, uint32_t vsize, uint32_t cap, const void* lim, hipStream_t s);
 int xe_launch_prologue(const void* const* src, void* const* dst, const uint64_t* words, uint32_t nseg, void* zero,
                        uint64_t zero_words, hipStream_t s);
-int xe_launch_tail(const XeTailArgs* A, hipStream_t s);
 int xe_launch_desc_overlap(const void* desc, uint32_t n, uint64_t umem_len, void* scratch, size_t* scratch_bytes,
                            uint32_t* flag, hipStream_t s);
 int xe_launch_keyed(const XeKeyed* K, const XeDevMap* maps, uint8_t* skip, uint32_t step, uint32_t items, hipStream_t s);
diff --git a/gobpfld_amd/csrc/xe_runtime.cpp b/gobpfld_amd/csrc/xe_runtime.cpp
--- a/gobpfld_amd/csrc/xe_runtime.cpp
+++ b/gobpfld_amd/csrc/xe_runtime.cpp
@@ -62,6 +62,12 @@
                 [&](bool valid) { run_staged(L, *P, 0, valid, false); });
   }
   flush_wave_state(L, *P);
+  if (P->arrive) {
+    if (xe_atomic_add32(P->arrive, 1u) != 0) return -1;
+    unsigned long long orw[XE_TAIL_REP_WORDS + 2];
+    batch_epilogue(P->tail, 0, 1, orw, [] {});
+    *P->arrive = 0;
+  }
   return 0;
 }
 int launch_jit(void*, const XeParams* P, uint32_t b, uint32_t t, xe_stream_t s) { return launch_interp(P, b, t, s); }
@@ -121,31 +127,6 @@
       if (!((s0 <= cap && rc[s0 * rwords]) || (s1 != s0 && s1 <= cap && rc[s1 * rwords]))) continue;
     }
     for (uint32_t k = 0; k < nrep; k++) { v[i] += r[k * sw + i]; r[k * sw + i] = 0; }
-  }
-  return 0;
-}
-int launch_tail(const XeTailArgs* A, xe_stream_t) {
-  unsigned long long orw[257] = {};
-  const bool poisoned = *A->poison != 0;
-  for (uint32_t i = 0; i < A->aux_words; i++) {
-    const unsigned long long v = A->aux[i];
-    A->aux[i] = 0;
-    A->host_aux[i] = v;
-    if (i == 0) orw[256] = v;
-    else if (i >= 16) orw[(i - 16) % A->rep_words] |= v;
-  }
-  const bool replay = !poisoned && xe_replay_decision(uint32_t(orw[256]), orw, A->rep_words, A->nmaps, A->mode);
-  A->host_aux[XE_AUX_DECISION] = replay ? 1ull : 0ull;
-  if (replay) *A->poison = 1u;
-  if (poisoned) return 0;
-  for (uint32_t f = 0; f < A->ntail; f++) {
-    const XeTailMap& T = A->tail[f];
-    for (uint64_t i = 0; i < T.words; i++) {
-      unsigned long long s = 0;
-      for (uint32_t k = 0; k < T.nrep; k++) { s += T.rep[k * T.stride_words + i]; T.rep[k * T.stride_words + i] = 0; }
-      T.vals[i] += s;
-      T.snap[i] = T.vals[i];
-    }
   }
   return 0;
 }
@@ -348,7 +329,6 @@
 int launch_lru_log(const uint64_t* tag, uint32_t pool, const uint32_t* order, const uint64_t* hdr, uint64_t* log, xe_stream_t s) {
   return xe_launch_lru_log(tag, pool, order, hdr, log, s);
 }
-int launch_tail(const XeTailArgs* A, xe_stream_t s) { return xe_launch_tail(A, s); }
 int launch_desc_overlap(const void* desc, uint32_t n, uint64_t umem_len, void* scratch, size_t* bytes, uint32_t* flag,
                         xe_stream_t s) {
   return xe_launch_desc_overlap(desc, n, umem_len, scratch, bytes, flag, s);
@@ -402,7 +382,9 @@
   return n;
 }
 #endif
-int launch_emulator(void* fn, const XeParams* P, uint32_t blocks, uint32_t threads, xe_stream_t s) {
+void count_launch(xe_vm* vm, int kind);
+int launch_emulator(xe_vm* vm, void* fn, const XeParams* P, uint32_t blocks, uint32_t threads, xe_stream_t s) {
+  count_launch(vm, 0);
   return fn ? launch_jit(fn, P, blocks, threads, s) : launch_interp(P, blocks, threads, s);
 }
 
@@ -826,6 +808,7 @@
     unsigned long long* h_aux = nullptr;
     unsigned long long* h_aux_dev = nullptr;
     Timer t0, t1, done;
+    bool folded = false;
     Batch b;
     size_t aux_used = 0;
     uint32_t nmaps = 0, grid = 0, engine = 0;
@@ -836,6 +819,8 @@
   uint32_t next_slot = 0;
   uint32_t next_snap = 0;
   uint32_t* d_poison = nullptr;
+  uint32_t* d_arrive = nullptr;
+  uint64_t launches[4] = {0, 0, 0, 0};
   xe_stream_t cancel_stream = nullptr;
   int32_t staged_slot = -1;
   bool draining = false;
@@ -958,6 +943,8 @@
   return rc;
 }
 
+void count_launch(xe_vm* vm, int kind) { vm->launches[kind]++; }
+
 int ensure_buf(void** p, size_t* cap, size_t need) {
   if (*cap >= need && *p) return 0;
   dev_free(*p);
@@ -979,7 +966,8 @@
   return want;
 }
 
-int fold_map(HostMap& m, xe_stream_t s) {
+int fold_map(xe_vm* vm, HostMap& m, xe_stream_t s) {
+  count_launch(vm, 2);
   const bool hash = m.dkind == XE_DM_HASH && m.def.value_size > 0;
   const bool lru = m.dkind == XE_DM_LRU;
   const uint64_t words = lru ? (uint64_t(m.pool_cap) * m.def.value_size + 7) / 8 : m.vals_alloc / 8;
@@ -1545,13 +1533,14 @@
 void xe_destroy(xe_vm* vm) {
   if (!vm) return;
   set_device(vm->settings.device);
-  for (uint32_t si : vm->pending) (void)vm->slots[si].done.wait();
+  for (uint32_t si : vm->pending) (void)(vm->slots[si].folded ? vm->slots[si].done : vm->slots[si].t1).wait();
   vm->pending.clear();
   for (auto& sl : vm->slots) {
     dev_free(sl.d_aux); host_free(sl.h_aux);
     sl.t0.fini(); sl.t1.fini(); sl.done.fini();
   }
   dev_free(vm->d_poison);
+  dev_free(vm->d_arrive);
   stream_destroy(vm->cancel_stream);
   dev_free(vm->d_trace_pk); dev_free(vm->d_trace); dev_free(vm->d_trace_cnt);
   dev_free(vm->d_listrun); dev_free(vm->d_popflag); dev_free(vm->d_popbase); dev_free(vm->d_popused);
@@ -2529,6 +2518,7 @@
       dst.push_back(m.d_snap);
       words.push_back(m.vals_alloc / 8);
     }
+    count_launch(vm, 3);
     if (launch_prologue(src.data(), dst.data(), words.data(), uint32_t(src.size()), vm->d_aux, aux_used, s))
       return fail(vm, XE_ERR_DEVICE, "prologue");
   }
@@ -2618,7 +2608,7 @@
 int BatchRun::fold() {
   for (size_t i = 1; i < vm->maps.size(); i++) {
     HostMap& m = vm->maps[i];
-    if (m.nrep > 1 && fold_map(m, s)) return -1;
+    if (m.nrep > 1 && fold_map(vm, m, s)) return -1;
     if (m.dkind == XE_DM_LRU && m.trep_r > 1 && launch_lru_tag_fold(m.d_tag, m.d_trep, m.pool_cap, m.trep_r, m.d_hdr, s)) return -1;
   }
   return 0;
@@ -2648,7 +2638,7 @@
     }
     vm->t1.rec(s);
     void* sj = (jit && !jit_general && n >= kSeqScalarMin) ? variant_kernel(vm, jit, kSeqVariant) : nullptr;
-    if (launch_emulator(sj ? sj : jit, &P, 1, 64, s)) return fail(vm, XE_ERR_DEVICE, "kernel launch");
+    if (launch_emulator(vm, sj ? sj : jit, &P, 1, 64, s)) return fail(vm, XE_ERR_DEVICE, "kernel launch");
     vm->t2.rec(s);
     if (hostcalls && serve_hostcalls(vm->h_hostcall, s)) return fail(vm, XE_ERR_DEVICE, "kernel failed (host helpers)");
     if (read_aux()) return fail(vm, XE_ERR_DEVICE, "kernel failed");
@@ -2718,7 +2708,7 @@
   tmark("arena");
   X.mode = XE_MODE_SPEC;
   X.K = K;
-  if (launch_emulator(kjit, &X, kgrid, 256, s) || fold()) return kfail(XE_ERR_DEVICE, "kernel launch (keyed spec)");
+  if (launch_emulator(vm, kjit, &X, kgrid, 256, s) || fold()) return kfail(XE_ERR_DEVICE, "kernel launch (keyed spec)");
   if (read_aux()) return kfail(XE_ERR_DEVICE, "kernel failed (keyed spec)");
   const uint32_t sflags = uint32_t(red[0]);
   if (ordmaps && (sflags & XE_FLAG_CAPACITY) && !(sflags & XE_FLAG_ORDERED)) {
@@ -2872,7 +2862,7 @@
     XeParams Y = X;
     const uint32_t pgrid = parallel_grid(vm, jit, general, n, P.nmaps);
     if (general && ensure_arena(vm, false, pgrid * 256, Y.gen)) return kfail(XE_ERR_NOMEM, "device alloc (arena)");
-    if (launch_emulator(jit, &Y, pgrid, 256, s) || fold()) return kfail(XE_ERR_DEVICE, "kernel launch (keyed parallel)");
+    if (launch_emulator(vm, jit, &Y, pgrid, 256, s) || fold()) return kfail(XE_ERR_DEVICE, "kernel launch (keyed parallel)");
   }
   return KeyedResult::Done;
 }
@@ -2889,7 +2879,7 @@
   X.K.skip = nullptr;
   const uint32_t cgrid = std::max<uint32_t>(1, std::min<uint32_t>(kgrid, (K.nO + 255) / 256));
   if (general && ensure_arena(vm, false, cgrid * 256, X.gen)) return kfail(XE_ERR_NOMEM, "device alloc (arena)");
-  if (launch_emulator(kjit, &X, cgrid, 256, s) || kstep(XE_KS_UNNEW, K.dcap)) return kfail(XE_ERR_DEVICE, "kernel launch (keyed chains)");
+  if (launch_emulator(vm, kjit, &X, cgrid, 256, s) || kstep(XE_KS_UNNEW, K.dcap)) return kfail(XE_ERR_DEVICE, "kernel launch (keyed chains)");
   if (read_aux() || read_small()) return kfail(XE_ERR_DEVICE, "kernel failed (keyed chains)");
   if (run_conflict(red, P.nmaps)) return kreplay("chain conflict", true);
   auto inserts = [&](size_t i) {
@@ -2984,7 +2974,7 @@
 }
 
 int BatchRun::pass() {
-  if (launch_emulator(pj, &P, vm->last_grid, 256, s)) return fail(vm, XE_ERR_DEVICE, "kernel launch");
+  if (launch_emulator(vm, pj, &P, vm->last_grid, 256, s)) return fail(vm, XE_ERR_DEVICE, "kernel launch");
   vm->t1.rec(s);
   if (fold()) return fail(vm, XE_ERR_DEVICE, "replica fold");
   if (read_aux()) return fail(vm, XE_ERR_DEVICE, "kernel failed");
@@ -3227,7 +3217,7 @@
 int complete_oldest(xe_vm* vm) {
   const uint32_t si = vm->pending.front();
   xe_vm::Slot& sl = vm->slots[si];
-  if (sl.done.wait()) {
+  if ((sl.folded ? sl.done : sl.t1).wait()) {
     vm->pending.clear();
     return fail(vm, XE_ERR_DEVICE, "kernel failed (pipelined batch)");
   }
@@ -3458,12 +3448,17 @@
   if (!vm->d_poison) {
     if (dev_alloc((void**)&vm->d_poison, 8) || dmemset(vm->d_poison, 0, 8, s)) return fail(vm, XE_ERR_DEVICE, "alloc (poison)");
   }
+  if (!vm->d_arrive) {
+    if (dev_alloc((void**)&vm->d_arrive, 16) || dmemset(vm->d_arrive, 0, 16, s)) return fail(vm, XE_ERR_DEVICE, "alloc (arrival counter)");
+  }
   XeParams P = batch_params(vm, d_umem, umem_len, d_desc, n, d_results, d_verdicts, d_regs, sl.d_aux);
   P.mode = XE_MODE_PARALLEL;
   P.poison = vm->d_poison;
   const size_t aux_used = 16 + size_t(kRep) * P.rep_words;
   const bool staged = vm->staged_slot == int32_t(ai) && !vm->pending.empty() && vm->slots[vm->pending.back()].b.s == s;
-  XeTailArgs A{};
+  if (P.rep_words > XE_TAIL_REP_WORDS) return fail(vm, XE_ERR_UNSUPPORTED, "wave records too long for the batch epilogue");
+  XeTailArgs& A = P.tail;
+  P.arrive = vm->d_arrive;
   A.aux = sl.d_aux;
   A.host_aux = sl.h_aux_dev;
   A.poison = vm->d_poison;
@@ -3502,18 +3497,22 @@
   if (jit && !P.results && !P.regs) jit = variant_kernel(vm, jit, kLeanVariant);
   const uint32_t grid = parallel_grid(vm, jit, general, n, P.nmaps);
   if (general && ensure_arena(vm, false, grid * 256, P.gen)) return fail(vm, XE_ERR_NOMEM, "device alloc (arena)");
-  if (!src.empty() && launch_prologue(src.data(), dst.data(), words.data(), uint32_t(src.size()), nullptr, 0, s))
-    return fail(vm, XE_ERR_DEVICE, "prologue");
+  if (!src.empty()) {
+    count_launch(vm, 3);
+    if (launch_prologue(src.data(), dst.data(), words.data(), uint32_t(src.size()), nullptr, 0, s))
+      return fail(vm, XE_ERR_DEVICE, "prologue");
+  }
   sl.t0.rec(s);
-  if (launch_emulator(jit, &P, grid, 256, s)) return fail(vm, XE_ERR_DEVICE, "kernel launch");
+  if (launch_emulator(vm, jit, &P, grid, 256, s)) return fail(vm, XE_ERR_DEVICE, "kernel launch");
   sl.t1.rec(s);
+  sl.folded = false;
   for (size_t i : big) {
     HostMap& m = vm->maps[i];
-    if (m.nrep > 1 && fold_map(m, s))
-      return fail(vm, XE_ERR_DEVICE, "replica fold");
-  }
-  if (launch_tail(&A, s)) return fail(vm, XE_ERR_DEVICE, "epilogue");
-  sl.done.rec(s);
+    if (m.nrep <= 1) continue;
+    if (fold_map(vm, m, s)) return fail(vm, XE_ERR_DEVICE, "replica fold");
+    sl.folded = true;
+  }
+  if (sl.folded) sl.done.rec(s);
   vm->staged_slot = int32_t(nai);
   sl.snap = ai;
   vm->next_snap = nai;
@@ -4135,6 +4134,22 @@
   return map_scan_run(vm, mi, f, keys, values, cap_entries, matched, nullptr, true, true);
 }
 
+int xe_debug_launches(xe_vm* vm, uint64_t out[4]) {
+  if (!vm || !out) return XE_ERR_INVAL;
+  for (int k = 0; k < 4; k++) out[k] = vm->launches[k];
+  return XE_OK;
+}
+
+int xe_debug_arrivals(xe_vm* vm, uint32_t* count) {
+  if (!vm || !count) return XE_ERR_INVAL;
+  if (int rc = xe_sync(vm)) return rc;
+  *count = 0;
+  if (!vm->d_arrive) return XE_OK;
+  set_device(vm->settings.device);
+  if (d2h(count, vm->d_arrive, 4, vm->stream) || dsync(vm->stream)) return fail(vm, XE_ERR_DEVICE, "arrival counter read");
+  return XE_OK;
+}
+
 int xe_debug_map_traffic(xe_vm* vm, int32_t mi, uint64_t* uploads, uint64_t* downloads) {
   HostMap* m = get_map(vm, mi);
   if (!m) return XE_ERR_INVAL;
diff --git a/gobpfld_amd/emulator.py b/gobpfld_amd/emulator.py
--- a/gobpfld_amd/emulator.py
+++ b/gobpfld_amd/emulator.py
@@ -335,6 +335,16 @@
         self._check(self.lib.debug_map_traffic(self.h, m, C.byref(up), C.byref(down)), "map traffic")
         return up.value, down.value
 
+    def debug_launches(self) -> tuple[int, int, int, int]:
+        out = (C.c_uint64 * 4)()
+        self._check(self.lib.debug_launches(self.h, out), "debug launches")
+        return tuple(int(x) for x in out)
+
+    def debug_arrivals(self) -> int:
+        n = C.c_uint32()
+        self._check(self.lib.debug_arrivals(self.h, C.byref(n)), "debug arrivals")
+        return n.value
+
     def map_values_bytes(self, m: int) -> int:
         b = C.c_uint64()
         self._check(self.lib.map_values_bytes(self.h, m, C.byref(b)), "map values bytes")
diff --git a/include/xdpemu.h b/include/xdpemu.h
--- a/include/xdpemu.h
+++ b/include/xdpemu.h
@@ -277,6 +277,8 @@
 int xe_debug_set_lru_epoch(xe_vm* vm, uint64_t epoch);
 int xe_debug_map_pool(xe_vm* vm, int32_t map, uint64_t* room, uint64_t* next_id);
 int xe_debug_map_traffic(xe_vm* vm, int32_t map_idx, uint64_t* uploads, uint64_t* downloads);
+int xe_debug_launches(xe_vm* vm, uint64_t out[4]);
+int xe_debug_arrivals(xe_vm* vm, uint32_t* count);
 
 const char* xe_version(void);
 int xe_device_count(int* n);
```

Result: faster. 57180 (median of 6 runs) (+1.1%).
